# rcanut/nhwcodec

Measured on AMD Instinct MI355X. Metric: encode Mpixels/s (512x512 RGB batch), higher is better.
Workload: dtype int16

## Files before the change

include/nhw_hip_debug.h:

```cpp
#ifndef NHW_HIP_DEBUG_H
#define NHW_HIP_DEBUG_H

#include "nhw_hip.h"

#ifdef __cplusplus
extern "C" {
#endif

int nhw_debug_stop_after(nhw_enc *e, int stage);
int nhw_debug_front_fallback(nhw_enc *e, int on);
int nhw_debug_read(nhw_enc *e, int buf, int img, void *dst, size_t bytes);
int nhw_debug_hash(nhw_enc *e, int buf, size_t bytes, int n, void *d_out, void *stream);

int nhw_debug_fill(nhw_enc *e, int buf, int byte, size_t bytes, int n);

int nhw_debug_slice_order(nhw_enc *e, int mode);
int nhw_dec_debug_slice_order(nhw_dec *d, int mode);

int nhw_stage_chroma_loops(nhw_enc *e, int n, int comp, int form, void *stream);
int nhw_debug_write(nhw_enc *e, int buf, int img, const void *src, size_t bytes);
int nhw_stage_luma_loop(nhw_enc *e, int n, int form, void *stream);
int nhw_stage_ll2_walk(nhw_enc *e, int n, int form, void *stream);
int nhw_stage_quant(nhw_enc *e, int n, int form, void *stream);
int nhw_stage_residuals(nhw_enc *e, int n, int form, void *stream);
int nhw_stage_stream(nhw_enc *e, int n, int form, int32_t *status, uint32_t *sizes, void *stream);

void nhw_dec_debug_stop_after(nhw_dec *d, int stage);
int  nhw_dec_debug_read(nhw_dec *d, int what, int img, void *dst, size_t bytes);
int  nhw_dec_debug_colour(int quality, const void *d_yuv, void *d_rgb, int n);
void nhw_debug_warp_row_limit(int limit);

#ifdef __cplusplus
}
#endif
#endif
```

nhwcodec_amd/__init__.py:

```python
import ctypes
import math
import numbers
import os

HERE = os.path.dirname(os.path.abspath(__file__))
LIB_PATH = os.path.join(HERE, "libnhwhip.so")
IMG_BYTES = 786432
OUT_STRIDE = 512 << 10
QUALITY_DEFAULT = 20
NHW_OK, NHW_E_QUALITY, NHW_E_CODEBOOK, NHW_E_SPACE, NHW_E_ARG, NHW_E_HIP, NHW_E_FORMAT = 0, -1, -2, -3, -4, -5, -6
NHW_E_BUDGET = -7
PEAK_SSE_NUMERATOR = 65025 * IMG_BYTES

P = ctypes.c_void_p


class Timing(ctypes.Structure):
    _fields_ = [(n, ctypes.c_float) for n in ("total_ms", "front_ms", "color_dwt_ms", "luma_ms", "chroma_ms", "entropy_ms")] + [("parts", ctypes.c_int), ("front_images", ctypes.c_int), ("prefilter_ms", ctypes.c_float)]


class FitStats(ctypes.Structure):
    _fields_ = [("rungs", ctypes.c_int), ("quality", ctypes.c_int * 23), ("images", ctypes.c_int * 23), ("total_ms", ctypes.c_float)]


class NhwError(RuntimeError):
    pass


class CTensorFormat(ctypes.Structure):
    _fields_ = [(n, ctypes.c_int32) for n in ("dtype", "layout", "channels", "rows")] + [("scale", ctypes.c_float * 3), ("bias", ctypes.c_float * 3), ("reserved", ctypes.c_uint32)]


def load_library(path: str = LIB_PATH) -> ctypes.CDLL:
    if not os.path.exists(path):
        raise NhwError(f"{path} not built: run `python -c 'import __graft_entry__ as g; g.build()'` (needs hipcc); there is no CPU fallback")
    import torch
    L = ctypes.CDLL(path)
    L.nhw_last_error.restype = ctypes.c_char_p
    L.nhw_enc_create.argtypes = [ctypes.c_int, ctypes.c_int, ctypes.POINTER(P)]
    L.nhw_enc_create_ex.argtypes = [ctypes.c_int, ctypes.c_int, ctypes.c_uint, ctypes.POINTER(P)]
    L.nhw_enc_destroy.argtypes = [P]
    L.nhw_quality_supported.argtypes = [ctypes.c_int]
    L.nhw_enc_set_compat.argtypes = [P, ctypes.c_int]
    L.nhw_enc_batch_device.argtypes = [P, P, ctypes.c_int, ctypes.c_int, P, P, P, P]
    L.nhw_enc_batch.argtypes = [P, P, ctypes.c_int, ctypes.c_int, P, ctypes.c_size_t, P, P]
    L.nhw_synth_batch_device.argtypes = [P, P, ctypes.c_int, ctypes.c_uint32, P]
    L.nhw_enc_last_timing.argtypes = [P, ctypes.POINTER(Timing)]
    L.nhw_enc_synth_batch.argtypes = [P, ctypes.c_int, ctypes.c_uint32, ctypes.c_int, P, ctypes.c_size_t, P, P]
    L.nhw_host_alloc.restype = P
    L.nhw_host_alloc.argtypes = [ctypes.c_size_t]
    L.nhw_host_free.argtypes = [P]
    L.nhw_device_count.restype = ctypes.c_int
    L.nhw_enc_fit_batch_device.argtypes = [P, P, ctypes.c_int, P, P, ctypes.c_int, P, P, P, P, P]
    L.nhw_enc_fit_batch.argtypes = [P, P, ctypes.c_int, P, P, ctypes.c_int, P, ctypes.c_size_t, P, P, P]
    L.nhw_enc_last_fit_stats.argtypes = [P, ctypes.POINTER(FitStats)]
    L.nhw_sse_batch_device.argtypes = [P, P, ctypes.c_int, P, P]
    L.nhw_enc_fit_sse_batch_device.argtypes = [P, P, P, ctypes.c_int, P, P, ctypes.c_int, P, P, P, P, P, P]
    L.nhw_enc_fit_sse_batch.argtypes = [P, P, P, ctypes.c_int, P, P, ctypes.c_int, P, ctypes.c_size_t, P, P, P, P]
    L.nhw_stage_color.argtypes = [P, P, ctypes.c_int, ctypes.c_int, P, P, P, P]
    L.nhw_stage_prefilter.argtypes = [P, P, ctypes.c_int, ctypes.c_int, P]
    L.nhw_stage_chroma_l1.argtypes = [P, ctypes.c_int, P]
    L.nhw_stage_chroma_loops.argtypes = [P, ctypes.c_int, ctypes.c_int, ctypes.c_int, P]
    L.nhw_stage_luma_loop.argtypes = [P, ctypes.c_int, ctypes.c_int, P]
    L.nhw_stage_ll2_walk.argtypes = [P, ctypes.c_int, ctypes.c_int, P]
    L.nhw_stage_quant.argtypes = [P, ctypes.c_int, ctypes.c_int, P]
    L.nhw_stage_residuals.argtypes = [P, ctypes.c_int, ctypes.c_int, P]
    L.nhw_stage_stream.argtypes = [P, ctypes.c_int, ctypes.c_int, P, P, P]
    L.nhw_debug_write.argtypes = [P, ctypes.c_int, ctypes.c_int, P, ctypes.c_size_t]
    L.nhw_stage_analysis.argtypes = [P, P, P, ctypes.c_int, ctypes.c_size_t, ctypes.c_int, ctypes.c_int, ctypes.c_int, P]
    L.nhw_stage_synthesis.argtypes = [P, P, P, ctypes.c_int, ctypes.c_size_t, ctypes.c_int, ctypes.c_int, P]
    L.nhw_debug_slice_order.argtypes = [P, ctypes.c_int]
    L.nhw_dec_debug_slice_order.argtypes = [P, ctypes.c_int]
    L.nhw_picture_tiles.argtypes = [ctypes.c_uint32, ctypes.c_uint32]
    L.nhw_tile_pictures_device.argtypes = [P, ctypes.c_int, ctypes.c_int, ctypes.c_int, P, P]
    L.nhw_untile_pictures_device.argtypes = [P, P, ctypes.c_int, ctypes.c_int, ctypes.c_int, P]
    L.nhw_picture_info.argtypes = [P, ctypes.c_size_t, ctypes.POINTER(ctypes.c_uint32), ctypes.POINTER(ctypes.c_uint32)]
    L.nhw_enc_pictures.argtypes = [P, P, P, P, P, ctypes.c_int, ctypes.c_int, P, ctypes.c_size_t, P, P]
    L.nhw_dec_pictures.argtypes = [P, P, P, ctypes.c_int, P, P, P]
    L.nhw_sse_pictures_device.argtypes = [P, P, ctypes.c_int, ctypes.c_int, ctypes.c_int, P, P]
    L.nhw_enc_fit_pictures.argtypes = [P, P, P, P, P, ctypes.c_int, P, P, ctypes.c_int, P, ctypes.c_size_t, P, P, P]
    L.nhw_enc_fit_sse_pictures.argtypes = [P, P, P, P, P, P, ctypes.c_int, P, P, ctypes.c_int, P, ctypes.c_size_t, P, P, P, P]
    L.nhw_region_tiles.argtypes = [ctypes.c_uint32] * 6
    L.nhw_untile_regions_device.argtypes = [P, P, ctypes.c_int, ctypes.c_int, ctypes.c_int, P]
    L.nhw_dec_regions.argtypes = [P, P, P, ctypes.c_int, P, ctypes.c_int, P, P, P]
    L.nhw_dec_regions_to_device.argtypes = [P, P, P, ctypes.c_int, P, ctypes.c_int, P, P, P]
    L.nhw_dec_last_region_stats.argtypes = [P, ctypes.POINTER(ctypes.c_uint64), ctypes.POINTER(ctypes.c_uint64)]
    L.nhw_dec_batch_device_scaled.argtypes = [P, P, P, P, ctypes.c_int, ctypes.c_int, P, P, P, P]
    L.nhw_dec_batch_scaled.argtypes = [P, P, P, ctypes.c_int, ctypes.c_int, P, P, P]
    L.nhw_picture_scaled_size.argtypes = [ctypes.c_uint32, ctypes.c_uint32, ctypes.c_int, ctypes.POINTER(ctypes.c_uint32), ctypes.POINTER(ctypes.c_uint32)]
    L.nhw_untile_pictures_scaled_device.argtypes = [P, P, ctypes.c_int, ctypes.c_int, ctypes.c_int, ctypes.c_int, P]
    L.nhw_dec_pictures_scaled.argtypes = [P, P, P, ctypes.c_int, ctypes.c_int, P, P, P]
    L.nhw_window_tiles.argtypes = [ctypes.c_uint32, ctypes.c_uint32, ctypes.c_int] + [ctypes.c_uint32] * 4
    L.nhw_untile_windows_device.argtypes = [P, P, ctypes.c_int, P, ctypes.c_int, ctypes.c_int, ctypes.c_int, ctypes.c_int, P]
    L.nhw_dec_windows.argtypes = [P, P, P, ctypes.c_int, P, ctypes.c_int, ctypes.c_int, P, P, P]
    L.nhw_dec_windows_to_device.argtypes = [P, P, P, ctypes.c_int, P, ctypes.c_int, ctypes.c_int, P, P, P]
    L.nhw_dec_batch_device_tensor.argtypes = [P, P, P, P, ctypes.c_int, ctypes.c_int, ctypes.POINTER(CTensorFormat), P, P, P, P]
    L.nhw_bytes_to_tensor_device.argtypes = [P, ctypes.c_int, ctypes.POINTER(CTensorFormat), P, P]
    L.nhw_tensor_to_bytes_device.argtypes = [P, ctypes.c_int, ctypes.POINTER(CTensorFormat), P, P]
    L.nhw_crop_scale.argtypes = [ctypes.c_uint32] * 4
    L.nhw_resize_to_tensor_device.argtypes = [P, ctypes.c_int, ctypes.c_uint32, ctypes.c_uint32, ctypes.POINTER(CTensorFormat), P, P, P]
    L.nhw_dec_crops_to_device.argtypes = [P, P, P, ctypes.c_int, P, ctypes.c_int, ctypes.c_int, ctypes.c_uint32, ctypes.c_uint32, ctypes.POINTER(CTensorFormat), P, P, P]
    L.nhw_enc_batch_device_tensor.argtypes = [P, P, ctypes.c_int, ctypes.POINTER(CTensorFormat), ctypes.c_int, P, P, P, P]
    L.nhw_tile_tensors_device.argtypes = [P, ctypes.c_int, ctypes.c_int, ctypes.c_int, ctypes.POINTER(CTensorFormat), P, P]
    L.nhw_area_to_tensor_device.argtypes = L.nhw_resize_to_tensor_device.argtypes
    L.nhw_dec_crops_to_device_filter.argtypes = L.nhw_dec_crops_to_device.argtypes + [ctypes.c_int]
    a = L.nhw_resize_to_tensor_device.argtypes
    L.nhw_resample_to_tensor_device.argtypes = a[:4] + [ctypes.c_int] + a[4:]
    L.nhw_dec_crops_to_device_resample.argtypes = L.nhw_dec_crops_to_device_filter.argtypes
    L.nhw_enc_pictures_resized.argtypes = [P, P, P, P, P, ctypes.c_int, ctypes.c_uint32, ctypes.c_uint32, ctypes.c_int, P, ctypes.c_size_t, P, P]
    L.nhw_warp_to_tensor_device.argtypes = L.nhw_resize_to_tensor_device.argtypes
    L.nhw_dec_warps_to_device.argtypes = L.nhw_dec_crops_to_device.argtypes
    L.nhw_debug_warp_row_limit.argtypes, L.nhw_debug_warp_row_limit.restype = [ctypes.c_int], None
    L.nhw_grey_table.argtypes = [ctypes.c_int, P]
    L.nhw_dec_batch_device_grey.argtypes = L.nhw_dec_batch_device_tensor.argtypes
    L.nhw_dec_batch_grey.argtypes = L.nhw_dec_batch_scaled.argtypes
    L.nhw_untile_windows_grey_device.argtypes = L.nhw_untile_windows_device.argtypes
    L.nhw_resample_grey_to_tensor_device.argtypes = L.nhw_resample_to_tensor_device.argtypes
    L.nhw_warp_grey_to_tensor_device.argtypes = L.nhw_warp_to_tensor_device.argtypes
    L.nhw_dec_windows_grey.argtypes = L.nhw_dec_windows.argtypes
    L.nhw_dec_windows_grey_to_device.argtypes = L.nhw_dec_windows_to_device.argtypes
    L.nhw_dec_crops_grey_to_device.argtypes = L.nhw_dec_crops_to_device_resample.argtypes
    L.nhw_dec_warps_grey_to_device.argtypes = L.nhw_dec_warps_to_device.argtypes
    a = L.nhw_resample_to_tensor_device.argtypes
    L.nhw_resample_mapped_to_tensor_device.argtypes = a[:7] + [P] + a[7:]
    a = L.nhw_warp_to_tensor_device.argtypes
    L.nhw_warp_mapped_to_tensor_device.argtypes = a[:6] + [P] + a[6:]
    a = L.nhw_dec_crops_to_device_resample.argtypes
    L.nhw_dec_crops_mapped_to_device.argtypes = a[:11] + [P] + a[11:]
    a = L.nhw_dec_warps_to_device.argtypes
    L.nhw_dec_warps_mapped_to_device.argtypes = a[:11] + [P] + a[11:]
    a = L.nhw_resample_mapped_to_tensor_device.argtypes
    L.nhw_resample_toned_to_tensor_device.argtypes = a[:8] + [P] + a[8:]
    a = L.nhw_warp_mapped_to_tensor_device.argtypes
    L.nhw_warp_toned_to_tensor_device.argtypes = a[:7] + [P] + a[7:]
    a = L.nhw_dec_crops_mapped_to_device.argtypes
    L.nhw_dec_crops_toned_to_device.argtypes = a[:12] + [P] + a[12:]
    a = L.nhw_dec_warps_mapped_to_device.argtypes
    L.nhw_dec_warps_toned_to_device.argtypes = a[:12] + [P] + a[12:]
    L.nhw_hist_device.argtypes = [P, ctypes.c_int, ctypes.c_int, P, P]
    L.nhw_tone_from_hist_device.argtypes = [P, ctypes.c_int, ctypes.c_int, P, P, P]
    return L


_LIB = None


def _library():
    global _LIB
    if _LIB is None:
        _LIB = load_library()
    return _LIB


def psnr_to_max_sse(db):
    import numpy as np
    try:
        a = np.asarray(db, dtype=np.float64)
    except (TypeError, ValueError):
        raise NhwError(f"a PSNR target must be a finite number of dB above 0, got {db!r}") from None
    if a.size == 0 or not np.all(np.isfinite(a)) or not np.all(a > 0):
        raise NhwError(f"a PSNR target must be a finite number of dB above 0, got {db!r}")
    m = np.floor(float(PEAK_SSE_NUMERATOR) * np.power(10.0, -a / 10.0)).astype(np.int64)
    return int(m) if m.ndim == 0 else m


def sse_device(a, b):
    import torch
    for name, x in (("a", a), ("b", b)):
        if not (isinstance(x, torch.Tensor) and x.is_cuda and x.dtype == torch.uint8 and x.is_contiguous() and x.numel() > 0 and x.numel() % IMG_BYTES == 0):
            raise NhwError(f"sse_device: `{name}` must be a contiguous uint8 CUDA tensor of n * {IMG_BYTES} bytes")
    if a.numel() != b.numel() or a.device != b.device:
        raise NhwError("sse_device: `a` and `b` must hold as many pictures, on one device")
    n = a.numel() // IMG_BYTES
    L = _library()
    out = torch.empty(n, dtype=torch.int64, device=a.device)
    with torch.cuda.device(a.device):
        rc = L.nhw_sse_batch_device(a.data_ptr(), b.data_ptr(), n, out.data_ptr(), torch.cuda.current_stream(a.device).cuda_stream)
    if rc != 0:
        raise NhwError(f"libnhwhip rc={rc}: {L.nhw_last_error().decode()}")
    return out


PICTURE_DTYPE = [("addr", "<u8"), ("pitch", "<u8"), ("width", "<u4"), ("height", "<u4"), ("first_tile", "<u4"), ("reserved", "<u4")]


def picture_tiles(width: int, height: int) -> int:
    if not (1 <= width <= 65535 and 1 <= height <= 65535):
        raise NhwError(f"a picture side must be 1..65535, got {width} x {height}")
    return ((width + 511) // 512) * ((height + 511) // 512)


SCALES = (1, 2, 4)


def _scale(scale, what):
    if isinstance(scale, bool) or not isinstance(scale, numbers.Integral) or scale not in SCALES:
        raise NhwError(f"{what}: the scale must be 1, 2 or 4, got {scale!r}")
    return int(scale)


def scaled_size(width: int, height: int, scale: int) -> tuple:
    scale = _scale(scale, "scaled_size")
    if not (isinstance(width, numbers.Integral) and isinstance(height, numbers.Integral)):
        raise NhwError(f"a picture's sides must be integers, got {width!r} x {height!r}")
    picture_tiles(int(width), int(height))
    return -(-int(width) // scale), -(-int(height) // scale)


REGION_DTYPE = [("addr", "<u8"), ("pitch", "<u8"), ("x", "<u4"), ("y", "<u4"), ("width", "<u4"), ("height", "<u4"), ("pic_width", "<u4"),
                ("pic_height", "<u4"), ("first_tile", "<u4"), ("reserved", "<u4")]
RECT_DTYPE = [("container", "<u4"), ("x", "<u4"), ("y", "<u4"), ("width", "<u4"), ("height", "<u4")]


def region_tiles(pic_width: int, pic_height: int, x: int, y: int, width: int, height: int) -> int:
    picture_tiles(pic_width, pic_height)
# ... 1639 lines not shown
```

nhwcodec_amd/csrc/nhw_enc.h:

```cpp
#ifndef NHW_ENC_H
#define NHW_ENC_H

#include <stdio.h>
#include <stdlib.h>
#include <string.h>
#include <climits>

#include "nhw_host.h"
#include "nhw_ws.h"

extern thread_local std::string nhw_enc_err;
#define NHW_ERR nhw_enc_err

enum { EV_START, EV_FRONT, EV_LUMA, EV_CHROMA, EV_END, EV_COLOR, EV_PREFILTER, EV_COUNT };
enum { PE_LUMA_LIST, PE_CHROMA, PE_LISTS_FORK, PE_LISTS, PE_FRONT, PE_COUNT };
enum { LL_EV_FORK, LL_EV_DONE, LL_EV_Y5_FORK, LL_EV_Y5_DONE, LL_EV_PACK_FORK, LL_EV_PACK_DONE, LL_EV_COUNT };

struct nhw_enc {
	int device, max_batch;
	NhwWs ws;
	hipStream_t own_stream;
	hipStream_t part_stream[4];
	hipEvent_t part_ev[PE_COUNT];
	hipStream_t low_stream[4];
	hipEvent_t low_ev[LOW_EV_COUNT];
	int low_parts;
	int low_parts_used;
	int low_chroma;
	hipStream_t ll_stream;
	hipEvent_t ll_ev[LL_EV_COUNT];
	int ll_fork;
	int quant_join;
	int y5_fork;
	int ll2_once;
	int quant_marks;
	int pack_fork;
	int parts;
	hipEvent_t ev[EV_COUNT];
	bool timed;
	int timed_parts, timed_front_images;
	uint8_t *d_in, *d_out, *d_compact;
	uint32_t *d_sizes; int32_t *d_status; uint64_t *d_offs;
	int conv_cap;
	uint8_t *d_tensor_bytes;
	int chroma_fork;
	int lists_fork;
	int front_fallback;
	int stop_after;
	int slice_order;
	int last_n, last_q;
	struct {
		uint8_t *in, *out;
		uint32_t *sizes, *budget;
		int32_t *status, *quality;
		int *idx[2], *count;
		uint8_t *open;
	} fit;
	struct {
		uint8_t *px;
		uint64_t *doff;
		uint64_t *sse, *maxsse;
		uint64_t *sse_out;
		int32_t *dstatus;
	} fit_sse;
	int *h_fit_count;
	hipEvent_t fit_ev[2];
	nhw_fit_stats fit_stats;
	bool fit_done;
	GrowBuf pic_px, pic_desc, pfit_px, pfit_aux, pic_resized;
};

inline DevSet host_set(nhw_enc *e, size_t n)
{
	return { dev_buf(e->d_in, n * NHW_IMG_BYTES), dev_buf(e->d_out, n * NHW_OUT_STRIDE), dev_buf(e->d_compact, n * NHW_OUT_STRIDE), dev_buf(e->d_sizes, n),
	         dev_buf(e->d_status, n), dev_buf(e->d_offs, n + 1) };
}
inline DevSet fit_set(nhw_enc *e)
{
	const size_t mb = (size_t)e->max_batch;
	return { dev_buf(e->fit.in, mb * NHW_IMG_BYTES), dev_buf(e->fit.out, mb * NHW_OUT_STRIDE), dev_buf(e->fit.sizes, mb), dev_buf(e->fit.budget, mb),
	         dev_buf(e->fit.status, mb), dev_buf(e->fit.quality, mb), dev_buf(e->fit.idx[0], mb), dev_buf(e->fit.idx[1], mb), dev_buf(e->fit.count, 1),
	         dev_buf(e->fit.open, mb) };
}
inline DevSet fit_sse_set(nhw_enc *e)
{
	const size_t mb = (size_t)e->max_batch;
	return { dev_buf(e->fit_sse.px, mb * NHW_IMG_BYTES), dev_buf(e->fit_sse.doff, mb), dev_buf(e->fit_sse.sse, mb), dev_buf(e->fit_sse.maxsse, mb),
	         dev_buf(e->fit_sse.sse_out, mb), dev_buf(e->fit_sse.dstatus, mb) };
}

int host_buffers(nhw_enc *e, int n);
int host_download(nhw_enc *e, int n, uint8_t *out_arena, size_t arena_cap, uint64_t *out_off, int32_t *status);
int ladder_check(const int *ladder, int ladder_len, bool ascending, int *q, int *len);
int dec_check(const nhw_enc *e, nhw_dec *d, int need, const std::string &who, const char *need_name);
void fit_doff(uint64_t *d_off, int n, hipStream_t s);

#endif
```

nhwcodec_amd/csrc/nhw_enc.hip:

```cpp
#include "nhw_enc.h"

thread_local std::string nhw_enc_err;
extern "C" const char *nhw_last_error(void) { return nhw_enc_err.c_str(); }

static const size_t k_buf_bytes[B_COUNT] = {
	 8 * Q,  8 * Q,  Q,  Q,  2 * Q,  2 * Q,
	 2 * Q,  2 * Q,  Q / 2,  Q / 2,  4 * Q,  2 * Q,
	 2 * Q,  4 * Q + 256,  8 * Q,  16,  512,  6 * Q,
	 24832,  16384,  16384 + 256,  32768,  16384,  32768,
	 8192,  2 * Q + 1024,  2 * Q + 256,  2 * Q + 1024,  2 * Q + 1024,  Q / 2,
	 Q + 64, 8192 + 64, 16384 + 64,  Q + 64, 8192 + 64, 16384 + 64,  Q + 64, 8192 + 64, 16384 + 64,
	 2 * Q + 1024, 16384 + 64, 16384 + 64,  2048 + 64,  8 * Q + 64,
	 512,  512,  320000,  768,  768,  16384 + 64,  16384 + 64,
	 131072,  131072,  5632,  256,  512,  16,  16,  (8 + 9 * 512) * 2,
	 Q / 2 + 256,  Q / 2,  Q / 4,  4 * Q,
	 Q / 4 + 256,  2 * Q,
	 2 * Q,  2 * Q,  Q / 2,  Q / 2,  Q,
	 320 * 512,
	 sizeof(NhwChromaPack),  320000
};

static size_t round_up(size_t v, size_t a) { return (v + a - 1) / a * a; }

extern "C" int nhw_quality_supported(int quality) { return quality >= 1 && quality <= 23; }

extern "C" int nhw_enc_set_compat(nhw_enc *e, int mode)
{
	if (!e || (mode != NHW_COMPAT_CANONICAL && mode != NHW_COMPAT_GLIBC_ONESHOT)) return NHW_E_ARG;
	if (e->ws.compat != mode && mode == NHW_COMPAT_CANONICAL) {
		HIPCHK(hipSetDevice(e->device));
		HIPCHK(hipDeviceSynchronize());
		HIPCHK(hipMemset2D(e->ws.plane<uint8_t>(B_LL1).p + 2 * Q, e->ws.plane<uint8_t>(B_LL1).bytes(), 0, 1024, (size_t)e->max_batch));
		HIPCHK(hipMemset2D(e->ws.plane<uint8_t>(B_L2SAVE).p + 2 * Q, e->ws.plane<uint8_t>(B_L2SAVE).bytes(), 0, 256, (size_t)e->max_batch));
	}
	e->ws.compat = mode;
	return NHW_OK;
}

#define HOST_PATH_BYTES ((size_t)NHW_IMG_BYTES + 2 * (size_t)NHW_OUT_STRIDE + 24)
extern "C" int nhw_enc_create_ex(int device, int max_batch, unsigned flags, nhw_enc **out)
{
	if (!out || max_batch < 1 || max_batch > 65535 || (flags & ~(unsigned)NHW_CREATE_DEVICE_ONLY)) { nhw_enc_err = "bad argument"; return NHW_E_ARG; }
	const bool host_staging = !(flags & NHW_CREATE_DEVICE_ONLY);
	HIPCHK(hipSetDevice(device));
	nhw_enc *e = new nhw_enc();
	memset(e, 0, sizeof *e);
	e->device = device; e->max_batch = max_batch;
	size_t total = 0;
	for (int b = 0; b < B_COUNT; b++) {
		e->ws.stride[b] = round_up(k_buf_bytes[b] + GUARD, 256);
		e->ws.off[b] = total + GUARD;
		total += GUARD + e->ws.stride[b] * (size_t)max_batch;
	}
	const int rc = [&]() -> int {
		size_t free_b = 0, total_b = 0;
		HIPCHK(hipMemGetInfo(&free_b, &total_b));
		const size_t need = total + (host_staging ? HOST_PATH_BYTES * (size_t)max_batch : 0);
		if (need > free_b) {
			char b[200];
			snprintf(b, sizeof b, "encoder workspace for max_batch %d needs %zu MiB (%.1f MiB per image), %zu MiB of HBM are free", max_batch, need >> 20, (double)need / max_batch / 1048576.0, free_b >> 20);
			nhw_enc_err = b;
			return NHW_E_ARG;
		}
		{ const char *where = ""; int rc_ = nhw_front_set_attrs(&where); if (!rc_) rc_ = nhw_tail_set_attrs(&where);
		  if (rc_) { nhw_enc_err = std::string(where) + " -> " + hipGetErrorString((hipError_t)rc_); return NHW_E_HIP; } }
		HIPCHK(hipMalloc((void **)&e->ws.base, total));
		HIPCHK(hipMemset(e->ws.base, 0, total));
		HIPCHK(hipStreamCreate(&e->own_stream));
		for (int i = 0; i < EV_COUNT; i++) HIPCHK(hipEventCreate(&e->ev[i]));
		for (int i = 0; i < 4; i++) HIPCHK(hipStreamCreateWithFlags(&e->part_stream[i], hipStreamNonBlocking));
		for (int i = 0; i < PE_COUNT; i++) HIPCHK(hipEventCreateWithFlags(&e->part_ev[i], hipEventDisableTiming));
		for (int i = 0; i < 4; i++) HIPCHK(hipStreamCreateWithFlags(&e->low_stream[i], hipStreamNonBlocking));
		for (int i = 0; i < LOW_EV_COUNT; i++) HIPCHK(hipEventCreateWithFlags(&e->low_ev[i], hipEventDisableTiming));
		HIPCHK(hipStreamCreateWithFlags(&e->ll_stream, hipStreamNonBlocking));
		for (int i = 0; i < LL_EV_COUNT; i++) HIPCHK(hipEventCreateWithFlags(&e->ll_ev[i], hipEventDisableTiming));
		for (int i = 0; i < 2; i++) HIPCHK(hipEventCreate(&e->fit_ev[i]));
		HIPCHK(hipHostMalloc((void **)&e->h_fit_count, sizeof(int), hipHostMallocDefault));
		return host_staging ? host_buffers(e, max_batch) : NHW_OK;
	}();
	if (rc != NHW_OK) { nhw_enc_destroy(e); return rc; }
	auto env = [](const char *name, int dflt) { const char *p = getenv(name); return p ? atoi(p) : dflt; };
	auto within = [](int v, int lo, int hi, int other) { return v < lo || v > hi ? other : v; };
	e->parts = within(env("NHW_PARTS", 1), 1, 4, 1);
	e->low_parts = within(env("NHW_LOW_PARTS", 2), 1, 4, 1);
	e->low_chroma = within(env("NHW_LOW_CHROMA", 2), 0, 2, 2);
	e->chroma_fork = env("NHW_CHROMA_FORK", 1) != 0;
	e->lists_fork = env("NHW_LISTS_FORK", 1) != 0;
	e->ll_fork = env("NHW_LL_FORK", 1) != 0;
	e->quant_join = env("NHW_QUANT_JOIN", 1) != 0;
	e->y5_fork = env("NHW_Y5_FORK", 1) != 0;
	e->ll2_once = env("NHW_LL2_ONCE", 1) != 0;
	e->quant_marks = env("NHW_QUANT_MARKS", 1) != 0;
	e->pack_fork = within(env("NHW_PACK_FORK", 2), 0, 2, 2);
	*out = e;
	return NHW_OK;
}

extern "C" int nhw_enc_create(int device, int max_batch, nhw_enc **out) { return nhw_enc_create_ex(device, max_batch, 0u, out); }

extern "C" void nhw_enc_destroy(nhw_enc *e)
{
	if (!e) return;
	(void)hipSetDevice(e->device);
	(void)hipDeviceSynchronize();
	if (e->ws.base) (void)hipFree(e->ws.base);
	dev_free(host_set(e, 0));
	dev_free({ dev_buf(e->d_tensor_bytes, 0) });
	dev_free(fit_set(e));
	dev_free(fit_sse_set(e));
	for (GrowBuf *g : { &e->pic_px, &e->pic_desc, &e->pfit_px, &e->pfit_aux, &e->pic_resized }) nhw_grow_free(*g);
	if (e->h_fit_count) (void)hipHostFree(e->h_fit_count);
	for (int i = 0; i < 2; i++) if (e->fit_ev[i]) (void)hipEventDestroy(e->fit_ev[i]);
	for (int i = 0; i < EV_COUNT; i++) if (e->ev[i]) (void)hipEventDestroy(e->ev[i]);
	if (e->own_stream) (void)hipStreamDestroy(e->own_stream);
	for (int i = 0; i < 4; i++) if (e->part_stream[i]) (void)hipStreamDestroy(e->part_stream[i]);
	for (int i = 0; i < PE_COUNT; i++) if (e->part_ev[i]) (void)hipEventDestroy(e->part_ev[i]);
	for (int i = 0; i < 4; i++) if (e->low_stream[i]) (void)hipStreamDestroy(e->low_stream[i]);
	for (int i = 0; i < LOW_EV_COUNT; i++) if (e->low_ev[i]) (void)hipEventDestroy(e->low_ev[i]);
	if (e->ll_stream) (void)hipStreamDestroy(e->ll_stream);
	for (int i = 0; i < LL_EV_COUNT; i++) if (e->ll_ev[i]) (void)hipEventDestroy(e->ll_ev[i]);
	delete e;
}

int host_buffers(nhw_enc *e, int n)
{
	if (e->conv_cap >= n) return NHW_OK;
	dev_free(host_set(e, 0));
	e->conv_cap = 0;
	const int rc = dev_alloc(host_set(e, (size_t)n), nullptr, n, nhw_enc_err);
	if (rc == NHW_OK) e->conv_cap = n;
	return rc;
}

#define STAGE_DONE() do { if (e->stop_after && ++stage == e->stop_after) { HIPCHK(hipGetLastError()); return NHW_OK; } } while (0)
static int chroma_head_launches(nhw_enc *e, const NhwWs &ws, int comp, int n, hipStream_t cs, int &stage)
{
	const int q = ws.q;
	const bool low = q <= 16;
	const bool vp = comp && ws.split_chroma;
	const Plane<int16_t> cjpeg = ws.plane<int16_t>(vp ? B_CJPEG_V : B_CJPEG), cproc = ws.plane<int16_t>(vp ? B_CPROC_V : B_CPROC);
	const Plane<int16_t> cll1 = ws.plane<int16_t>(vp ? B_CLL1_V : B_CLL1), cl2save = ws.plane<int16_t>(vp ? B_CL2SAVE_V : B_CL2SAVE);
	const Plane<const uint8_t> bytes = ws.plane<const uint8_t>(comp ? B_PV : B_PU);
	const bool widen_in_analysis = q > 14 && !ws.dbg;
	if (q <= 14) nhw_launch_low_prefilter_chroma(bytes, cjpeg, q, n, cs);
	else if (!widen_in_analysis) nhw_launch_phase(PH_C0, ws, comp, cs);
	STAGE_DONE();
	NhwAnalysis l1 = NhwAnalysis{ cjpeg, cproc, n, H, H, 0 }.saving(cll1, H / 2, ANA_SAVE_LL);
	l1.store = ws.dbg ? ANA_STORE_ALL : ANA_STORE_NO_T_LL_SAVED;
	if (widen_in_analysis) l1.src8 = bytes;
	nhw_launch_analysis(l1, cs);
	if (low) nhw_launch_low_chroma_thin(cproc, n, cs);
	STAGE_DONE();
	STAGE_DONE();
	if (!ws.dbg) {
		nhw_launch_chroma_loops(cproc, cll1, cl2save, ws.plane<const uint8_t>(B_PU), q, comp, ws.compat, n, cs);
		return 1;
	}
	const NhwAnalysis l2{ cjpeg, cproc, n, H, H / 2, 1 };
	nhw_launch_analysis(l2, cs);
	STAGE_DONE();
	nhw_launch_phase(PH_C2, ws, comp, cs);
	STAGE_DONE();
	nhw_launch_synthesis(cjpeg, cproc, n, H, H / 2, 0, cs);
	STAGE_DONE();
	nhw_launch_phase(PH_C3, ws, comp, cs);
	STAGE_DONE();
	nhw_launch_analysis(l2.saving(cl2save, H / 2, ANA_SAVE_BLOCK), cs);
	STAGE_DONE();
	STAGE_DONE();
	nhw_launch_phase(PH_C4, ws, comp, cs);
	STAGE_DONE();
	nhw_launch_synthesis(cjpeg, cproc, n, H, H / 2, 0, cs);
	STAGE_DONE();
	return 1;
}

static int luma_loop_launches(nhw_enc *e, const NhwWs &ws, int n, hipStream_t s, int &stage, bool y5_beside = false ,
                              bool lean = false )
{
	const int q = ws.q;
	const Plane<int16_t> jpeg = ws.plane<int16_t>(B_JPEG), proc = ws.plane<int16_t>(B_PROC), ll1 = ws.plane<int16_t>(B_LL1), l2save = ws.plane<int16_t>(B_L2SAVE);
	const NhwAnalysis l2{ jpeg, proc, n, W, H, 1 };
	assert(!lean || (!ws.dbg && !ws.compat));
	NhwAnalysis first = l2.from(ll1, H);
	if (lean && q > 6) first.store = ANA_STORE_NO_T;
	nhw_launch_analysis(first, s);
	STAGE_DONE();
	if (q > 6) {
	if (y5_beside) {
		assert(!ws.dbg);
		HIPCHK(hipEventRecord(e->ll_ev[LL_EV_Y5_FORK], s));
		HIPCHK(hipStreamWaitEvent(e->ll_stream, e->ll_ev[LL_EV_Y5_FORK], 0));
		nhw_launch_phase(PH_L1, ws, 0, e->ll_stream);
		HIPCHK(hipEventRecord(e->ll_ev[LL_EV_Y5_DONE], e->ll_stream));
	} else
	nhw_launch_phase(PH_L1, ws, 0, s);
	nhw_launch_wave(WV_DQ1, ws, s);
	if (y5_beside) HIPCHK(hipStreamWaitEvent(s, e->ll_ev[LL_EV_Y5_DONE], 0));
	STAGE_DONE();
	if (ws.dbg) {
	nhw_launch_synthesis(jpeg, proc, n, W, H, 0, s);
	STAGE_DONE();
	nhw_launch_phase(PH_L2, ws, 0, s);
	STAGE_DONE();
	} else nhw_launch_l2_recon(jpeg, proc, ll1, q > 12 ? l2save : Plane<int16_t>{}, n, s, lean && q > 12);
	if (q <= 12) nhw_launch_analysis(l2, s);
	else if (ws.dbg) nhw_launch_analysis(l2.saving(l2save, H, ANA_SAVE_BLOCK), s);
	STAGE_DONE();
	}
	return 1;
}

static int run_batch(nhw_enc *e, const NhwWs &ws_in, const void *d_bgr, int n, int quality, void *d_out, uint32_t *d_sizes, int32_t *d_status, hipStream_t s,
                     int timed ,
                     int what = 3 )
{
	NhwWs ws = ws_in;
	const int q = quality;
	const bool low = q <= 16;
	const Plane<int16_t> jpeg = ws.plane<int16_t>(B_JPEG), proc = ws.plane<int16_t>(B_PROC);
	const Plane<uint8_t> pu = ws.plane<uint8_t>(B_PU), pv = ws.plane<uint8_t>(B_PV);

	e->low_parts_used = 1;
	int stage = 0;
	if (what & 1) {
	if (timed == 1) HIPCHK(hipEventRecord(e->ev[EV_START], s));
	const Plane<int16_t> yin = ws.plane<int16_t>(B_KMAP);
	NhwFront f;
	f.q = q; f.n = n; f.y = yin ; f.st = ws.plane<uint8_t>(B_ROWSTATE);
	f.proc = proc; f.jpeg = jpeg; f.ll1 = ws.plane<int16_t>(B_LL1); f.switches = ws.dbg ? 2 : 0;
	if (low) {
		nhw_launch_color((const uint8_t *)d_bgr, n, q, jpeg, pu, pv, s);
		HIPCHK(hipEventRecord(e->ev[EV_COLOR], s));
		STAGE_DONE();
		{ const int lparts = (timed == 1 && what == 3 && !e->stop_after && n >= 1024) ? e->low_parts : 1;
		  e->low_parts_used = lparts;
		  HIPCHK((hipError_t)nhw_launch_low_prefilter(jpeg, yin, proc, ws.plane<uint8_t>(B_SCAN), ws.plane<uint8_t>(B_KEEP), ws.plane<uint8_t>(B_LOWTAB), q, n, s, (e->front_fallback & 1) ? 32 : 0,
		                                              lparts, e->low_stream, e->low_ev)); }
		HIPCHK(hipEventRecord(e->ev[EV_PREFILTER], s));
		STAGE_DONE();
		if (ws.compat) nhw_launch_low_stale(proc, ws.plane<uint8_t>(B_STALE), n, s);
	} else {
		HIPCHK(hipEventRecord(e->ev[EV_COLOR], s)); HIPCHK(hipEventRecord(e->ev[EV_PREFILTER], s));
		STAGE_DONE();
		if (q < 22) STAGE_DONE();
		f.bgr = (const uint8_t *)d_bgr; f.pu = pu; f.pv = pv; f.with_prefilter = q < 22; f.switches |= e->front_fallback & 1;
		if (q > 21) f.keep = ws.plane<int16_t>(B_KEEP);
	}
	nhw_launch_front_fused(f, s);
	if (!low && ws.compat && q < 22) {
		nhw_launch_color((const uint8_t *)d_bgr, n, q, yin, pu, pv, s);
		nhw_launch_front_stale(yin, f.st, ws.plane<uint8_t>(B_STALE), n, s);
	}
	STAGE_DONE();
	STAGE_DONE();
	if (timed == 1) HIPCHK(hipEventRecord(e->ev[EV_FRONT], s));
	if (!(what & 2)) { HIPCHK(hipGetLastError()); return NHW_OK; }
	}
	const bool fork = timed == 1 && what == 3 && !e->stop_after && e->chroma_fork;
	const bool fork_ll = fork && q > 13 && !ws.compat && e->ll_fork;
	ws.defer_verbatim = fork_ll;
	hipStream_t cs = fork ? e->part_stream[0] : s;
	ws.split_chroma = fork;
	auto chroma_head = [&](int comp) -> int { return chroma_head_launches(e, ws, comp, n, cs, stage); };
	auto chroma_tail = [&](int comp) -> int {
		nhw_launch_phase(PH_C5, ws, comp, cs);
		STAGE_DONE();
		return 1;
	};
#define CHROMA(call) do { const int rc_ = (call); if (rc_ != 1) return rc_; } while (0)
	if (fork) {
		HIPCHK(hipStreamWaitEvent(cs, !low || e->low_chroma == 0 ? e->ev[EV_FRONT] : (e->low_chroma == 2 && e->low_parts_used > 1) ? e->low_ev[low_ev_pass_a(e->low_parts_used - 1)] : e->ev[EV_COLOR], 0));
		CHROMA(chroma_head(0));
		CHROMA(chroma_head(1));
	}
	{ const int rc_ = luma_loop_launches(e, ws, n, s, stage, fork && e->y5_fork, !ws.dbg && !ws.compat); if (rc_ != 1) return rc_; }
	if (q <= 12) {
		nhw_launch_low_ll2(proc, q, n, s);
		nhw_launch_copy_block(proc, W, ws.plane<int16_t>(B_L2SAVE), H, H, H, n, s);
	}
	STAGE_DONE();
	const bool one_walk = fork && q > 12 && e->ll2_once;
	const bool marks = q > 16 && !e->stop_after && !ws.dbg && e->quant_marks;
	nhw_launch_wave(WV_EMIT, ws, s, one_walk);
	if (fork_ll) {
		HIPCHK(hipEventRecord(e->ll_ev[LL_EV_FORK], s));
		HIPCHK(hipStreamWaitEvent(e->ll_stream, e->ll_ev[LL_EV_FORK], 0));
		nhw_launch_phase(PH_L3, ws, 0, e->ll_stream);
		HIPCHK(hipEventRecord(e->ll_ev[LL_EV_DONE], e->ll_stream));
		HIPCHK(hipEventRecord(e->part_ev[PE_LUMA_LIST], e->ll_stream));
	} else {
	nhw_launch_phase(PH_L3, ws, 0, s);
	if (fork) HIPCHK(hipEventRecord(e->part_ev[PE_LUMA_LIST], s));
	}
	if (q > 12) {
	nhw_launch_wave(WV_DQ0, ws, s, one_walk, marks);
	STAGE_DONE();
	if (fork_ll) {
		HIPCHK(hipStreamWaitEvent(s, e->ll_ev[LL_EV_DONE], 0));
		const Plane<const uint8_t> meta = ws.plane<const uint8_t>(B_META), len{ meta.p + offsetof(NhwMeta, ll_mem_len), meta.pitch };
		nhw_launch_synthesis(jpeg, proc, n, W, H, q <= 21 && !ws.dbg, ws.plane<const uint8_t>(B_LLMEM), len, s);
	} else
	nhw_launch_synthesis(jpeg, proc, n, W, H, q <= 21 && !ws.dbg, s);
	STAGE_DONE();
	}
	nhw_launch_phase(PH_L4A, ws, 0, s);
	const bool fork_lists = fork && q <= 20 && q > 12 && e->lists_fork;
	if (fork_lists) {
		HIPCHK(hipEventRecord(e->part_ev[PE_LISTS_FORK], s));
		HIPCHK(hipStreamWaitEvent(e->part_stream[1], e->part_ev[PE_LISTS_FORK], 0));
		nhw_launch_phase(PH_L4B, ws, 0, e->part_stream[1]);
		HIPCHK(hipEventRecord(e->part_ev[PE_LISTS], e->part_stream[1]));
	} else if (q > 12)
		nhw_launch_phase(PH_L4B, ws, 0, s);
	nhw_launch_phase(PH_L4C, ws, 0, s);
	const bool early_join = fork && e->quant_join;
	const int pack_fork = fork ? e->pack_fork : 0;
	auto chroma_rest = [&]() -> int {
		HIPCHK(hipStreamWaitEvent(cs, e->part_ev[PE_LUMA_LIST], 0));
		CHROMA(chroma_tail(0));
		CHROMA(chroma_tail(1));
		if (pack_fork == 2) {
			HIPCHK(hipEventRecord(e->ll_ev[LL_EV_PACK_FORK], cs));
			HIPCHK(hipStreamWaitEvent(e->ll_stream, e->ll_ev[LL_EV_PACK_FORK], 0));
			nhw_launch_pack_chroma(ws, e->ll_stream);
			HIPCHK(hipEventRecord(e->ll_ev[LL_EV_PACK_DONE], e->ll_stream));
		}
		nhw_launch_phase(PH_LLC, ws, 0, cs);
		if (pack_fork == 1) nhw_launch_pack_chroma(ws, cs);
		if (pack_fork == 2) HIPCHK(hipStreamWaitEvent(cs, e->ll_ev[LL_EV_PACK_DONE], 0));
		HIPCHK(hipEventRecord(e->part_ev[PE_CHROMA], cs));
		return 1;
	};
	if (early_join) {
		CHROMA(chroma_rest());
		if (fork_lists) HIPCHK(hipStreamWaitEvent(s, e->part_ev[PE_LISTS], 0));
		HIPCHK(hipStreamWaitEvent(s, e->part_ev[PE_CHROMA], 0));
	}
	nhw_launch_wave(WV_QUANT, ws, s, false, marks);
	if (q > 21) nhw_launch_phase(PH_L4C2, ws, 0, s);
	if (fork && !early_join) CHROMA(chroma_rest());
	nhw_launch_phase(PH_L4D, ws, 0, s);
	STAGE_DONE();
	if (timed) HIPCHK(hipEventRecord(e->ev[EV_LUMA], s));

	if (fork_lists && !early_join) HIPCHK(hipStreamWaitEvent(s, e->part_ev[PE_LISTS], 0));
	if (fork) { if (!early_join) HIPCHK(hipStreamWaitEvent(s, e->part_ev[PE_CHROMA], 0)); }
	else
		for (int comp = 0; comp < 2; comp++) {
			CHROMA(chroma_head(comp));
			CHROMA(chroma_tail(comp));
		}
#undef CHROMA
	if (timed) HIPCHK(hipEventRecord(e->ev[EV_CHROMA], s));
	if (!fork) nhw_launch_phase(PH_LLC, ws, 0, s);
	nhw_launch_final(ws, (uint8_t *)d_out, d_sizes, d_status, s, pack_fork != 0);
	if (timed == 1) HIPCHK(hipEventRecord(e->ev[EV_END], s));
	HIPCHK(hipGetLastError());
	return NHW_OK;
}

extern "C" int nhw_enc_batch_device(nhw_enc *e, const void *d_bgr, int n, int quality, void *d_out, uint32_t *d_sizes,
                                    int32_t *d_status, void *stream)
{
	if (!e || !d_bgr || !d_out || !d_sizes || !d_status || n < 1 || n > e->max_batch) { nhw_enc_err = "bad argument"; return NHW_E_ARG; }
	if (!nhw_quality_supported(quality)) { nhw_enc_err = "quality outside 1..23"; return NHW_E_QUALITY; }
	HIPCHK(hipSetDevice(e->device));
	hipStream_t s = stream ? (hipStream_t)stream : e->own_stream;
	const NhwSliceScope slices(e->slice_order);
	NhwWs ws = e->ws;
	ws.n = n; ws.q = quality; ws.dbg = e->stop_after != 0;
	e->timed = false;
	const int parts = (e->stop_after || n < 512) ? 1 : e->parts;
	if (parts == 1) {
		const int rc = run_batch(e, ws, d_bgr, n, quality, d_out, d_sizes, d_status, s, 1);
		if (rc == NHW_OK && !e->stop_after) { e->timed = true; e->timed_parts = 1; e->timed_front_images = n; e->last_n = n; e->last_q = quality; }
		return rc;
	}
	HIPCHK(hipEventRecord(e->ev[EV_START], s));
	{ const int rc = run_batch(e, ws, d_bgr, n, quality, d_out, d_sizes, d_status, s, 0, 1); if (rc != NHW_OK) return rc; }
	HIPCHK(hipEventRecord(e->ev[EV_FRONT], s));
	HIPCHK(hipEventRecord(e->part_ev[PE_FRONT], s));
	e->timed_front_images = n;
	for (int k = 0; k < parts; k++) {
		const int i0 = (int)((long long)n * k / parts), i1 = (int)((long long)n * (k + 1) / parts);
		NhwWs view = ws;
		view.n = i1 - i0;
		for (int b = 0; b < B_COUNT; b++) view.off[b] += (size_t)i0 * ws.stride[b];
		hipStream_t ps_ = e->part_stream[k];
		HIPCHK(hipStreamWaitEvent(ps_, e->part_ev[PE_FRONT], 0));
		const int rc = run_batch(e, view, (const uint8_t *)d_bgr + (size_t)i0 * (W * W * 3), i1 - i0, quality, (uint8_t *)d_out + (size_t)i0 * NHW_OUT_STRIDE,
		                         d_sizes + i0, d_status + i0, ps_, k == 0 ? 2 : 0, 2);
		if (rc != NHW_OK) return rc;
		HIPCHK(hipEventRecord(e->part_ev[k], ps_));
		HIPCHK(hipStreamWaitEvent(s, e->part_ev[k], 0));
	}
	HIPCHK(hipEventRecord(e->ev[EV_END], s));
	e->timed = true; e->timed_parts = parts; e->last_n = n; e->last_q = quality;
	return NHW_OK;
}

extern "C" int nhw_enc_last_timing(nhw_enc *e, nhw_timing *t)
{
	if (!e || !t || !e->timed) { nhw_enc_err = "no timed batch"; return NHW_E_ARG; }
	HIPCHK(hipEventSynchronize(e->ev[EV_END]));
	memset(t, 0, sizeof *t);
	HIPCHK(hipEventElapsedTime(&t->total_ms, e->ev[EV_START], e->ev[EV_END]));
	HIPCHK(hipEventElapsedTime(&t->front_ms, e->ev[EV_START], e->ev[EV_FRONT]));
	HIPCHK(hipEventElapsedTime(&t->luma_ms, e->ev[EV_FRONT], e->ev[EV_LUMA]));
	HIPCHK(hipEventElapsedTime(&t->chroma_ms, e->ev[EV_LUMA], e->ev[EV_CHROMA]));
	HIPCHK(hipEventElapsedTime(&t->entropy_ms, e->ev[EV_CHROMA], e->ev[EV_END]));
	HIPCHK(hipEventElapsedTime(&t->color_dwt_ms, e->ev[EV_START], e->ev[EV_COLOR]));
	HIPCHK(hipEventElapsedTime(&t->prefilter_ms, e->ev[EV_COLOR], e->ev[EV_PREFILTER]));
	t->parts = e->timed_parts; t->front_images = e->timed_front_images;
	return NHW_OK;
}

extern "C" int nhw_synth_batch_device(nhw_enc *e, void *d_bgr, int n, uint32_t seed_base, void *stream)
{
	if (!e || !d_bgr || n < 1) { nhw_enc_err = "bad argument"; return NHW_E_ARG; }
	HIPCHK(hipSetDevice(e->device));
	nhw_launch_synth((uint8_t *)d_bgr, n, seed_base, stream ? (hipStream_t)stream : e->own_stream);
	HIPCHK(hipGetLastError());
	return NHW_OK;
}

extern "C" int nhw_stage_color(nhw_enc *e, const void *d_bgr, int n, int quality, void *d_y, void *d_u, void *d_v, void *stream)
{
	if (!e || n < 1) return NHW_E_ARG;
	if (quality < 1 || quality > 23) return NHW_E_QUALITY;
	HIPCHK(hipSetDevice(e->device));
	nhw_launch_color((const uint8_t *)d_bgr, n, quality, Plane<int16_t>{ (int16_t *)d_y, 4 * Q }, Plane<uint8_t>{ (uint8_t *)d_u, Q }, Plane<uint8_t>{ (uint8_t *)d_v, Q }, stream ? (hipStream_t)stream : e->own_stream);
	HIPCHK(hipGetLastError());
	return NHW_OK;
}

extern "C" int nhw_stage_prefilter(nhw_enc *e, void *d_y, int n, int quality, void *stream)
{
	if (!e || !d_y || n < 1 || n > e->max_batch) { nhw_enc_err = "bad argument"; return NHW_E_ARG; }
	if (quality < 1 || quality > 16) { nhw_enc_err = "the pre-filter is a stage of its own only for quality 1..16"; return NHW_E_QUALITY; }
	HIPCHK(hipSetDevice(e->device));
	const NhwWs &ws = e->ws;
	hipStream_t s = stream ? (hipStream_t)stream : e->own_stream;
	const Plane<int16_t> filtered = ws.plane<int16_t>(B_KMAP);
	HIPCHK((hipError_t)nhw_launch_low_prefilter(Plane<const int16_t>{ (const int16_t *)d_y, 4 * Q }, filtered, ws.plane<int16_t>(B_PROC), ws.plane<uint8_t>(B_SCAN), ws.plane<uint8_t>(B_KEEP), ws.plane<uint8_t>(B_LOWTAB), quality, n, s, 0, 1 , e->low_stream, e->low_ev));
	HIPCHK(hipMemcpy2DAsync(d_y, 8 * Q, filtered.p, filtered.bytes(), 8 * Q, (size_t)n, hipMemcpyDeviceToDevice, s));
	HIPCHK(hipGetLastError());
	return NHW_OK;
}

__global__ __launch_bounds__(256) void k_plane_range(const int16_t *__restrict__ base, size_t plane_stride, int *__restrict__ mnmx)
{
	const uint4 *p = reinterpret_cast<const uint4 *>(base + (size_t)blockIdx.y * plane_stride);
	int mn = 32767, mx = -32768;
	for (int i = blockIdx.x * 256 + threadIdx.x; i < W * W / 8; i += gridDim.x * 256) {
		const uint4 v = p[i];
		const uint32_t w[4] = { v.x, v.y, v.z, v.w };
		for (int k = 0; k < 4; k++) {
			const int a = (int16_t)(w[k] & 0xFFFF), b = (int16_t)(w[k] >> 16);
			mn = a < mn ? a : mn; mn = b < mn ? b : mn; mx = a > mx ? a : mx; mx = b > mx ? b : mx;
		}
	}
	for (int o = 32; o; o >>= 1) { const int a = __shfl_xor(mn, o), b = __shfl_xor(mx, o); mn = a < mn ? a : mn; mx = b > mx ? b : mx; }
	if ((threadIdx.x & 63) == 0) { atomicMin(&mnmx[0], mn); atomicMax(&mnmx[1], mx); }
}

extern "C" int nhw_stage_analysis(nhw_enc *e, void *d_jpeg, void *d_proc, int n_img, size_t plane_stride, int stride, int size,
                                  int final_level, void *stream)
{
	if (!e || n_img < 1) { nhw_enc_err = "bad argument"; return NHW_E_ARG; }
	HIPCHK(hipSetDevice(e->device));
	hipStream_t s = stream ? (hipStream_t)stream : e->own_stream;
	if (size == 512) {
		if (stride != W || final_level || n_img > e->max_batch) { nhw_enc_err = "size 512: stride 512, not the final level, n <= max_batch"; return NHW_E_ARG; }
		if (((uintptr_t)d_jpeg & 15) || ((uintptr_t)d_proc & 15) || (plane_stride & 7) || plane_stride < (size_t)W * W) {
			nhw_enc_err = "size 512: planes must be 16-byte aligned and plane_stride (in samples) a multiple of 8, at least 512 x 512"; return NHW_E_ARG;
		}
		const NhwWs &ws = e->ws;
		{
			int *d_mm = reinterpret_cast<int *>(ws.plane<uint8_t>(B_ROWSTATE).p), mm[2] = { 32767, -32768 };
			HIPCHK(hipMemcpyAsync(d_mm, mm, sizeof mm, hipMemcpyHostToDevice, s));
			k_plane_range<<<dim3(32, n_img), 256, 0, s>>>((const int16_t *)d_jpeg, plane_stride, d_mm);
			HIPCHK(hipMemcpyAsync(mm, d_mm, sizeof mm, hipMemcpyDeviceToHost, s));
			HIPCHK(hipStreamSynchronize(s));
			const long U = mm[1] > 0 ? mm[1] : 0, L = mm[0] < 0 ? -(long)mm[0] : 0;
			if (104 * U + 40 * L > NHW_ANA512_BOUND || 104 * L + 40 * U > NHW_ANA512_BOUND) {
				nhw_enc_err = "size 512: samples outside the level-1 kernel's 16-bit domain (104 U + 40 L <= 32720, see nhw_hip.h)";
				return NHW_E_ARG;
			}
		}
		const Plane<int16_t> in = ws.plane<int16_t>(B_KMAP);
		HIPCHK(hipMemcpy2DAsync(in.p, in.bytes(), d_jpeg, plane_stride * 2, 8 * Q, (size_t)n_img, hipMemcpyDeviceToDevice, s));
		NhwFront f;
		f.q = 20; f.n = n_img; f.y = in; f.st = ws.plane<uint8_t>(B_ROWSTATE);
		f.proc = { (int16_t *)d_proc, plane_stride }; f.jpeg = { (int16_t *)d_jpeg, plane_stride }; f.ll1 = ws.plane<int16_t>(B_LL1); f.switches = 2;
		nhw_launch_front_fused(f, s);
	} else if (size == 256 || size == 128)
		nhw_launch_analysis(NhwAnalysis{ { (int16_t *)d_jpeg, plane_stride }, { (int16_t *)d_proc, plane_stride }, n_img, stride, size, final_level }, s);
	else { nhw_enc_err = "transform size must be 512, 256 or 128"; return NHW_E_ARG; }
	HIPCHK(hipGetLastError());
	return NHW_OK;
}

extern "C" int nhw_stage_chroma_l1(nhw_enc *e, int n, void *stream)
{
	if (!e || n < 1 || n > e->max_batch) { nhw_enc_err = "bad argument"; return NHW_E_ARG; }
	if (!e->timed || n > e->last_n || e->last_q < 15) {
		nhw_enc_err = "nhw_stage_chroma_l1: the handle's last batch does not cover the request (needs a completed batch of >= n images at quality >= 15)";
		return NHW_E_ARG;
	}
	HIPCHK(hipSetDevice(e->device));
	const NhwWs &ws = e->ws;
	hipStream_t s = stream ? (hipStream_t)stream : e->own_stream;
	HIPCHK(hipStreamWaitEvent(s, e->ev[EV_END], 0));
	NhwAnalysis l1 = NhwAnalysis{ ws.plane<int16_t>(B_CJPEG), ws.plane<int16_t>(B_CPROC), n, H, H, 0 }.saving(ws.plane<int16_t>(B_CLL1), H / 2, ANA_SAVE_LL);
	l1.store = ANA_STORE_NO_T_LL_SAVED;
	for (int comp = 0; comp < 2; comp++) { l1.src8 = ws.plane<const uint8_t>(comp ? B_PV : B_PU); nhw_launch_analysis(l1, s); }
	HIPCHK(hipGetLastError());
	return NHW_OK;
}

extern "C" int nhw_stage_chroma_loops(nhw_enc *e, int n, int comp, int form, void *stream)
{
	if (!e || n < 1 || n > e->max_batch || comp < 0 || comp > 1 || form < 0 || form > 8) { nhw_enc_err = "bad argument"; return NHW_E_ARG; }
	if (!e->timed || n > e->last_n || e->stop_after) {
		nhw_enc_err = "nhw_stage_chroma_loops: needs a completed whole batch of >= n images and no debug stop";
		return NHW_E_ARG;
	}
	HIPCHK(hipSetDevice(e->device));
	NhwWs ws = e->ws;
	ws.n = n; ws.q = e->last_q; ws.dbg = 0; ws.split_chroma = false;
	hipStream_t s = stream ? (hipStream_t)stream : e->own_stream;
	HIPCHK(hipStreamWaitEvent(s, e->ev[EV_END], 0));
	const Plane<int16_t> cjpeg = ws.plane<int16_t>(B_CJPEG), cproc = ws.plane<int16_t>(B_CPROC), cll1 = ws.plane<int16_t>(B_CLL1), cl2save = ws.plane<int16_t>(B_CL2SAVE);
	if (form == 0) {
		int stage = 0;
		const int rc = chroma_head_launches(e, ws, comp, n, s, stage);
		if (rc != 1) return rc;
	} else if (form == 1)
		nhw_launch_chroma_loops(cproc, cll1, cl2save, ws.plane<const uint8_t>(B_PU), ws.q, comp, ws.compat, n, s);
	else {
		const int k = form - 1;
		const NhwAnalysis l2{ cjpeg, cproc, n, H, H / 2, 1 };
		nhw_launch_analysis(l2.from(cll1, H / 2), s);
		if (k > 1) nhw_launch_phase(PH_C2, ws, comp, s);
		if (k > 2) nhw_launch_synthesis(cjpeg, cproc, n, H, H / 2, 0, s);
		if (k > 3) nhw_launch_phase(PH_C3, ws, comp, s);
		if (k > 4) nhw_launch_analysis(l2.saving(cl2save, H / 2, ANA_SAVE_BLOCK), s);
		if (k > 5) nhw_launch_phase(PH_C4, ws, comp, s);
		if (k > 6) nhw_launch_synthesis(cjpeg, cproc, n, H, H / 2, 0, s);
	}
	HIPCHK(hipGetLastError());
	return NHW_OK;
}

extern "C" int nhw_stage_luma_loop(nhw_enc *e, int n, int form, void *stream)
{
	if (!e || n < 1 || n > e->max_batch || form < 0 || form > 7) { nhw_enc_err = "bad argument"; return NHW_E_ARG; }
	if (!e->timed || n > e->last_n || e->stop_after || e->last_q < 7) {
		nhw_enc_err = "nhw_stage_luma_loop: needs a completed whole batch of >= n images at quality >= 7 and no debug stop";
		return NHW_E_ARG;
	}
	HIPCHK(hipSetDevice(e->device));
	NhwWs ws = e->ws;
	ws.n = n; ws.q = e->last_q; ws.dbg = 0;
	hipStream_t s = stream ? (hipStream_t)stream : e->own_stream;
	HIPCHK(hipStreamWaitEvent(s, e->ev[EV_END], 0));
	const Plane<int16_t> jpeg = ws.plane<int16_t>(B_JPEG), proc = ws.plane<int16_t>(B_PROC), ll1 = ws.plane<int16_t>(B_LL1), l2save = ws.plane<int16_t>(B_L2SAVE);
	const NhwAnalysis l2{ jpeg, proc, n, W, H, 1 };
	const bool save = ws.q > 12;
	const bool lean = form >= 6;
	if (lean && ws.compat) { nhw_enc_err = "nhw_stage_luma_loop: forms 6 and 7 are not launched in the compatibility mode"; return NHW_E_ARG; }
	if (form == 0 || form == 6) {
		int stage = 0;
		const int rc = luma_loop_launches(e, ws, n, s, stage, false, lean);
		if (rc != 1) return rc;
	} else if (form == 1 || form == 7) {
		nhw_launch_l2_recon(jpeg, proc, ll1, save ? l2save : Plane<int16_t>{}, n, s, lean && save);
		if (!save) nhw_launch_analysis(l2, s);
	} else {
		if (form == 3 || form == 4) {
			nhw_launch_analysis(l2.from(ll1, H), s);
			nhw_launch_phase(PH_L1, ws, 0, s);
			nhw_launch_wave(WV_DQ1, ws, s);
		}
		nhw_launch_synthesis(jpeg, proc, n, W, H, 0, s);
		if (form < 4) {
			nhw_launch_phase(PH_L2, ws, 0, s);
			nhw_launch_analysis(save ? l2.saving(l2save, H, ANA_SAVE_BLOCK) : l2, s);
		}
	}
	HIPCHK(hipGetLastError());
	return NHW_OK;
}

extern "C" int nhw_stage_ll2_walk(nhw_enc *e, int n, int form, void *stream)
{
	if (!e || n < 1 || n > e->max_batch || form < 0 || form > 3) { nhw_enc_err = "bad argument"; return NHW_E_ARG; }
	if (!e->timed || n > e->last_n || e->stop_after || e->last_q < 13) {
		nhw_enc_err = "nhw_stage_ll2_walk: needs a completed whole batch of >= n images at quality >= 13 and no debug stop";
		return NHW_E_ARG;
	}
	HIPCHK(hipSetDevice(e->device));
	NhwWs ws = e->ws;
	ws.n = n; ws.q = e->last_q; ws.dbg = 0; ws.defer_verbatim = form >= 2;
	hipStream_t s = stream ? (hipStream_t)stream : e->own_stream;
	HIPCHK(hipStreamWaitEvent(s, e->ev[EV_END], 0));
	const bool one_walk = !(form & 1);
	nhw_launch_wave(WV_EMIT, ws, s, one_walk);
	nhw_launch_phase(PH_L3, ws, 0, s);
	nhw_launch_wave(WV_DQ0, ws, s, one_walk);
	if (ws.defer_verbatim) {
		const Plane<const uint8_t> meta = ws.plane<const uint8_t>(B_META), len{ meta.p + offsetof(NhwMeta, ll_mem_len), meta.pitch };
		nhw_launch_synthesis(ws.plane<int16_t>(B_JPEG), ws.plane<int16_t>(B_PROC), n, W, H, ws.q <= 21, ws.plane<const uint8_t>(B_LLMEM), len, s);
	}
	HIPCHK(hipGetLastError());
	return NHW_OK;
}

extern "C" int nhw_stage_quant(nhw_enc *e, int n, int form, void *stream)
{
	if (!e || n < 1 || n > e->max_batch || form < 0 || form > 1) { nhw_enc_err = "bad argument"; return NHW_E_ARG; }
	if (!e->timed || n > e->last_n || e->stop_after || e->last_q < 17) {
		nhw_enc_err = "nhw_stage_quant: needs a completed whole batch of >= n images at quality >= 17 and no debug stop";
		return NHW_E_ARG;
	}
	HIPCHK(hipSetDevice(e->device));
	NhwWs ws = e->ws;
	ws.n = n; ws.q = e->last_q; ws.dbg = 0; ws.defer_verbatim = 1;
	hipStream_t s = stream ? (hipStream_t)stream : e->own_stream;
	HIPCHK(hipStreamWaitEvent(s, e->ev[EV_END], 0));
	if (form == 0) nhw_launch_wave(WV_DQ0, ws, s, true, true);
	nhw_launch_wave(WV_QUANT, ws, s, false, form == 0);
	HIPCHK(hipGetLastError());
	return NHW_OK;
}

extern "C" int nhw_stage_residuals(nhw_enc *e, int n, int form, void *stream)
{
	if (!e || n < 1 || n > e->max_batch || form < 0 || form > 3) { nhw_enc_err = "bad argument"; return NHW_E_ARG; }
	if (!e->timed || n > e->last_n || e->stop_after || (form == 2 && e->last_q <= 12)) {
		nhw_enc_err = "nhw_stage_residuals: needs a completed whole batch of >= n images (form 2: at quality >= 13) and no debug stop";
		return NHW_E_ARG;
	}
	HIPCHK(hipSetDevice(e->device));
	NhwWs ws = e->ws;
	ws.n = n; ws.q = e->last_q; ws.dbg = form == 1;
	hipStream_t s = stream ? (hipStream_t)stream : e->own_stream;
	HIPCHK(hipStreamWaitEvent(s, e->ev[EV_END], 0));
	if (form < 2) nhw_launch_phase(PH_L4A, ws, 0, s);
	if (form < 3 && ws.q > 12) nhw_launch_phase(PH_L4B, ws, 0, s);
	if (form != 2) nhw_launch_phase(PH_L4C, ws, 0, s);
	HIPCHK(hipGetLastError());
	return NHW_OK;
}

extern "C" int nhw_stage_stream(nhw_enc *e, int n, int form, int32_t *status, uint32_t *sizes, void *stream)
{
	if (!e || (!status && form != 2) || n < 1 || n > e->max_batch || form < 0 || form > 2) { nhw_enc_err = "bad argument"; return NHW_E_ARG; }
	if (!e->timed || n > e->last_n || e->stop_after) {
		nhw_enc_err = "nhw_stage_stream: needs a completed whole batch of >= n images and no debug stop";
		return NHW_E_ARG;
	}
	HIPCHK(hipSetDevice(e->device));
	{ const int rc = host_buffers(e, n); if (rc != NHW_OK) return rc; }
	NhwWs ws = e->ws;
	ws.n = n; ws.q = e->last_q; ws.dbg = 0;
	hipStream_t s = stream ? (hipStream_t)stream : e->own_stream;
	HIPCHK(hipStreamWaitEvent(s, e->ev[EV_END], 0));
	if (form != 1) nhw_launch_phase(PH_L4D, ws, 0, s);
	if (form == 2) { HIPCHK(hipGetLastError()); HIPCHK(hipStreamSynchronize(s)); return NHW_OK; }
	nhw_launch_final(ws, e->d_out, e->d_sizes, e->d_status, s);
	HIPCHK(hipGetLastError());
	HIPCHK(hipMemcpyAsync(status, e->d_status, sizeof(int32_t) * (size_t)n, hipMemcpyDeviceToHost, s));
	if (sizes) HIPCHK(hipMemcpyAsync(sizes, e->d_sizes, sizeof(uint32_t) * (size_t)n, hipMemcpyDeviceToHost, s));
	HIPCHK(hipStreamSynchronize(s));
	return NHW_OK;
}

extern "C" int nhw_stage_synthesis(nhw_enc *e, void *d_jpeg, void *d_proc, int n_img, size_t plane_stride, int stride, int size, void *stream)
{
	if (!e || n_img < 1) return NHW_E_ARG;
	if (size != 256 && size != 128) { nhw_enc_err = "synthesis: transform size must be 256 or 128 (the encoder has no synthesis of size 512)"; return NHW_E_ARG; }
	HIPCHK(hipSetDevice(e->device));
	nhw_launch_synthesis({ (int16_t *)d_jpeg, plane_stride }, { (int16_t *)d_proc, plane_stride }, n_img, stride, size, 0, stream ? (hipStream_t)stream : e->own_stream);
	HIPCHK(hipGetLastError());
	return NHW_OK;
}

extern "C" int nhw_debug_front_fallback(nhw_enc *e, int on) { if (!e) return NHW_E_ARG; e->front_fallback = on; return NHW_OK; }
extern "C" int nhw_debug_stop_after(nhw_enc *e, int stage) { if (!e) return NHW_E_ARG; e->stop_after = stage; return NHW_OK; }
extern "C" int nhw_debug_slice_order(nhw_enc *e, int mode) { if (!e || mode < 0 || mode > 2) return NHW_E_ARG; e->slice_order = mode; return NHW_OK; }
__global__ __launch_bounds__(256) void k_debug_hash(const uint8_t *base, size_t stride, size_t words, unsigned long long *out)
{
	const uint32_t *p = reinterpret_cast<const uint32_t *>(base + (size_t)blockIdx.x * stride);
	unsigned long long h = 0;
	for (size_t i = threadIdx.x; i < words; i += 256) {
		unsigned long long x = ((unsigned long long)p[i] + 0x9E3779B97F4A7C15ull) * (2 * i + 1);
		x ^= x >> 29; x *= 0xBF58476D1CE4E5B9ull; x ^= x >> 32;
		h += x;
	}
	if (threadIdx.x == 0) out[blockIdx.x] = 0;
	__syncthreads();
	atomicAdd(&out[blockIdx.x], h);
}
extern "C" int nhw_debug_hash(nhw_enc *e, int buf, size_t bytes, int n, void *d_out, void *stream)
{
	if (!e || buf < 0 || buf >= B_COUNT || n < 1 || n > e->max_batch || bytes > e->ws.stride[buf]) return NHW_E_ARG;
// ... 31 lines not shown
```

nhwcodec_amd/csrc/nhw_host.h:

```cpp
#ifndef NHW_HOST_H
#define NHW_HOST_H

#include <hip/hip_runtime.h>
#include <stdint.h>
#include <string>
#include <vector>

#include "../../include/nhw_hip.h"
#include "nhw_container.h"

struct NhwWs;

template <class T> struct Plane {
	T *p = nullptr; size_t pitch = 0;
	Plane at(size_t i) const { return { p + i * pitch, pitch }; }
	size_t bytes() const { return pitch * sizeof(T); }
	operator Plane<const T>() const { return { p, pitch }; }
};

extern thread_local int nhw_slice_mode;

struct NhwSliceScope {
	int saved;
	explicit NhwSliceScope(int mode) : saved(nhw_slice_mode) { nhw_slice_mode = mode; }
	~NhwSliceScope() { nhw_slice_mode = saved; }
};

template <typename F> inline void nhw_slices(int nslices, F &&launch)
{
	if (nhw_slice_mode == 1) for (int i = 0; i < nslices; i++) launch(i);
	else if (nhw_slice_mode == 2) for (int i = nslices - 1; i >= 0; i--) launch(i);
	else launch(-1);
}

void nhw_launch_color(const uint8_t *bgr, int n, int q, Plane<int16_t> y, Plane<uint8_t> u, Plane<uint8_t> v, hipStream_t s);
enum NhwAnaSave { ANA_SAVE_NONE, ANA_SAVE_BLOCK , ANA_SAVE_LL  };
enum NhwAnaStore { ANA_STORE_ALL, ANA_STORE_NO_T, ANA_STORE_NO_T_LL_SAVED };
struct NhwAnalysis {
	Plane<int16_t> jpeg, proc; int n, stride, size, final_level;
	Plane<int16_t> save = {}; int save_row = 0; NhwAnaSave save_kind = ANA_SAVE_NONE; NhwAnaStore store = ANA_STORE_ALL;
	Plane<const uint8_t> src8 = {}; Plane<const int16_t> alt = {}; int alt_stride = 0;
	NhwAnalysis from(Plane<const int16_t> p, int row) const { NhwAnalysis a = *this; a.alt = p; a.alt_stride = row; return a; }
	NhwAnalysis saving(Plane<int16_t> p, int row, NhwAnaSave kind) const { NhwAnalysis a = *this; a.save = p; a.save_row = row; a.save_kind = kind; return a; }
};
void nhw_launch_analysis(const NhwAnalysis &a, hipStream_t s);
void nhw_launch_synthesis(Plane<int16_t> jpeg, Plane<int16_t> proc, int n, int stride, int size, int drop_nat, Plane<const uint8_t> verb_list, Plane<const uint8_t> verb_len, hipStream_t s);
inline void nhw_launch_synthesis(Plane<int16_t> jpeg, Plane<int16_t> proc, int n, int stride, int size, int drop_nat, hipStream_t s) { nhw_launch_synthesis(jpeg, proc, n, stride, size, drop_nat, {}, {}, s); }
void nhw_launch_synth(uint8_t *bgr, int n, uint32_t seed_base, hipStream_t s);
struct NhwFront {
	const uint8_t *bgr = nullptr; Plane<uint8_t> pu = {}, pv = {}, st = {}; Plane<const int16_t> y = {};
	Plane<int16_t> proc = {}, jpeg = {}, ll1 = {}, keep = {}; int q = 0, with_prefilter = 0, n = 0, switches = 0;
};
void nhw_launch_front_fused(const NhwFront &f, hipStream_t s);
void nhw_launch_front_stale(Plane<const int16_t> y, Plane<const uint8_t> st, Plane<uint8_t> stale, int n, hipStream_t s);
int nhw_front_set_attrs(const char **where);
enum { PH_L1, PH_L2, PH_L3, PH_L4A, PH_C0, PH_C2, PH_C3, PH_C4, PH_C5, PH_L4B = 10, PH_L4C, PH_L4D, PH_LLC, PH_L4C2 };
enum { WV_DQ1, WV_DQ0, WV_EMIT, WV_QUANT };
void nhw_launch_phase(int ph, const NhwWs &ws, int comp, hipStream_t s);
void nhw_launch_pack_chroma(const NhwWs &ws, hipStream_t s);
void nhw_launch_final(const NhwWs &ws, uint8_t *out, uint32_t *sizes, int32_t *status, hipStream_t s, bool chroma_packed = false);
void nhw_launch_wave(int ph, const NhwWs &ws, hipStream_t s, bool one_walk = false ,
                     bool marks = false );
void nhw_launch_l2_recon(Plane<int16_t> jpeg, Plane<int16_t> proc, Plane<int16_t> ll1, Plane<int16_t> l2save , int n, hipStream_t s, bool lean = false );
void nhw_launch_chroma_loops(Plane<int16_t> cproc, Plane<int16_t> cll1, Plane<int16_t> cl2save, Plane<const uint8_t> pu, int q, int comp, int compat, int n, hipStream_t s);
void nhw_launch_copy_block(Plane<const int16_t> src, int src_row, Plane<int16_t> dst, int dst_row, int rows, int cols, int n, hipStream_t s);
int nhw_tail_set_attrs(const char **where);
enum { LOW_EV_START = 0, LOW_EV_COUNT = 13 };
inline int low_ev_pass_a(int p) { return 1 + p; }
inline int low_ev_done(int parts, int p) { return 1 + parts + p; }
int nhw_launch_low_prefilter(Plane<const int16_t> src, Plane<int16_t> y, Plane<int16_t> km, Plane<uint8_t> so, Plane<uint8_t> chain, Plane<uint8_t> tab,
                             int q, int n, hipStream_t s, int force, int parts, hipStream_t *aux, hipEvent_t *ev);
void nhw_launch_low_prefilter_chroma(Plane<const uint8_t> src, Plane<int16_t> dst, int q, int n, hipStream_t s);
void nhw_launch_low_chroma_thin(Plane<int16_t> plane, int n, hipStream_t s);
void nhw_launch_low_ll2(Plane<int16_t> proc, int q, int n, hipStream_t s);
void nhw_launch_low_stale(Plane<const int16_t> km, Plane<uint8_t> stale, int n, hipStream_t s);
void nhw_launch_fit_gather(const uint8_t *d_bgr, const int *idx, int m, uint8_t *staging, hipStream_t s);
void nhw_launch_fit_select(const int *idx, int m, const uint8_t *st_out, const uint32_t *st_sizes, const int32_t *st_status, const void *limit,
                           const int32_t *dec_status, const uint64_t *sse, int quality, int last, uint8_t *out, uint32_t *sizes, int32_t *status,
                           int32_t *qual, uint64_t *sse_out, uint8_t *open, hipStream_t s);
void nhw_launch_fit_compact(const uint8_t *open, const int *idx, int m, int *next, int *count, hipStream_t s);
hipError_t nhw_launch_sse(const uint8_t *a, const uint8_t *b, int n, uint64_t *sse, hipStream_t s);
hipError_t nhw_launch_tile_pad(const nhw_picture *d_pics, int n_pics, int tile0, int m, uint8_t *d_tiles, hipStream_t s);
hipError_t nhw_launch_untile_crop(const uint8_t *d_tiles, const nhw_picture *d_pics, int n_pics, int tile0, int m, int scale , hipStream_t s);
hipError_t nhw_launch_untile_region(const uint8_t *d_tiles, const nhw_region *d_regs, int n_regs, int tile0, int m, hipStream_t s);
hipError_t nhw_launch_untile_window(const uint8_t *d_tiles, const nhw_region *d_regs, int n_regs, const nhw_window_use *d_uses , int n_uses, int tile0, int m, int scale, hipStream_t s);
hipError_t nhw_launch_untile_window_grey(const uint8_t *d_tiles , const nhw_region *d_regs, int n_regs, const nhw_window_use *d_uses, int n_uses, int tile0, int m, int scale, hipStream_t s);
hipError_t nhw_launch_sse_crop(const uint8_t *d_tiles, const nhw_picture *d_pics, int n_pics, int tile0, int m, uint64_t *d_sse, hipStream_t s);
void nhw_dec_props(const nhw_dec *d, int *device, int *max_batch, int *stop_after);

int nhw_hip_error(std::string &err, hipError_t e, const char *file, int line, const char *call);
#define HIPCHK(x) do { hipError_t e_ = (x); if (e_ != hipSuccess) return nhw_hip_error(NHW_ERR, e_, __FILE__, __LINE__, #x); } while (0)

struct DevBuf { void **p; size_t bytes; };
using DevSet = std::vector<DevBuf>;
template <class T> inline DevBuf dev_buf(T *&p, size_t count) { return { (void **)&p, count * sizeof(T) }; }
void dev_free(const DevSet &set);
int dev_alloc(const DevSet &set, const char *what, int images, std::string &err);

struct GrowBuf {
	void *p; size_t cap;
	template <class T> T *as() const { return (T *)p; }
};
hipError_t nhw_grow(GrowBuf &b, size_t bytes);
void nhw_grow_free(GrowBuf &b);

#endif
```

nhwcodec_amd/csrc/nhw_tail.hip:

```cpp
#include "nhw_host.h"
#include "nhw_tail_par.h"
#include "nhw_dwt.h"

using namespace nhw;

#ifndef NHW_DENSE_STREAM
#define NHW_DENSE_STREAM 0
#endif

template <int PH>
__global__ __launch_bounds__(256) void k_phase(NhwWs ws, int comp)
{
	__shared__ int sh_counts[2];
	__shared__ int sh_pos[2 * NT + 2];
	__shared__ uint32_t sh_z[4 * Q / 16 / 32 + 4];
	extern __shared__ __attribute__((aligned(16))) int16_t dyn_lds[];
	const int img = blockIdx.x, tid = threadIdx.x;
	Ctx c;
	ctx_load(&c, ws, img, comp);
	if (PH == PH_L1) luma_p1_par(&c, tid, sh_pos);
	else if (PH == PH_L2) luma_p2_par(&c, tid, dyn_lds);
	else if (PH == PH_L3) luma_p3_par(&c, tid, sh_pos, sh_counts, dyn_lds, ws.q <= 12 || ws.dbg != 0);
	else if (PH == PH_L4A) luma_p4a_par(&c, tid, dyn_lds);
	else if (PH == PH_L4B) luma_p4b_par(&c, tid, sh_pos, dyn_lds);
	else if (PH == PH_L4C) luma_p4c_par(&c, tid, sh_pos, dyn_lds, ws.q > 21 || ws.dbg);
	else if (PH == PH_L4D) luma_p4d_par(&c, tid, sh_counts, sh_z, dyn_lds, NHW_DENSE_STREAM || ws.dbg);
	else if (PH == PH_L4C2) luma_p4c2_par(&c, tid, reinterpret_cast<unsigned *>(sh_z), sh_pos);
	else if (PH == PH_LLC) { PROF_BEGIN(); ll_code_chroma_par(&c, tid, reinterpret_cast<uint8_t *>(dyn_lds)); if (!tid) PROF(&c, 18); }
	else if (PH == PH_C0) chroma_p0_par(&c, comp, tid);
	else if (PH == PH_C2) { chroma_ll1_neighbour(&c, tid); dequant_sim_chroma_par(&c, 1, tid); }
	else if (PH == PH_C3) chroma_p3_par(&c, comp, tid);
	else if (PH == PH_C4) dequant_sim_chroma_par(&c, 0, tid);
	else if (PH == PH_C5) chroma_p5_par(&c, comp, tid, dyn_lds, sh_counts, ws.dbg != 0);
}

#ifndef NHW_FINAL_WAVES
#define NHW_FINAL_WAVES 6
#endif
__global__ __launch_bounds__(256) __attribute__((amdgpu_waves_per_eu(NHW_FINAL_WAVES, NHW_FINAL_WAVES))) void k_final(NhwWs ws, uint8_t *out, uint32_t *sizes, int32_t *status)
{
	extern __shared__ __attribute__((aligned(16))) int16_t dyn_lds[];
	__shared__ PackShared sh_pack;
	const int img = blockIdx.x, tid = threadIdx.x;
	Ctx c;
	ctx_load(&c, ws, img);
	final_phase_par(&c, ws.buf<NhwChromaPack>(B_CPACK, img), ws.buf<uint32_t>(B_CPACKET, img), out + (size_t)img * (512u << 10), 512u << 10, &sizes[img], &status[img], &sh_pack, tid,
	                reinterpret_cast<uint32_t *>(dyn_lds));
}

#ifndef NHW_PACKC_WAVES
#define NHW_PACKC_WAVES 6
#endif
__global__ __launch_bounds__(256) __attribute__((amdgpu_waves_per_eu(NHW_PACKC_WAVES, NHW_PACKC_WAVES))) void k_pack_chroma(NhwWs ws)
{
	extern __shared__ __attribute__((aligned(16))) int16_t dyn_lds[];
	__shared__ PackShared sh_pack;
	const int img = blockIdx.x;
	Ctx c;
	ctx_load(&c, ws, img);
	pack_chroma_par(&c, ws.buf<NhwChromaPack>(B_CPACK, img), ws.buf<uint32_t>(B_CPACKET, img), &sh_pack, threadIdx.x, reinterpret_cast<uint32_t *>(dyn_lds));
}

__global__ __launch_bounds__(512) void k_y31(NhwWs ws)
{
	extern __shared__ __attribute__((aligned(16))) int16_t dyn_lds[];
	__shared__ int sh_counts[2];
	Ctx c;
	ctx_load(&c, ws, blockIdx.x);
	PROF_BEGIN();
	scan_rewrite_list_par<512>(&c, threadIdx.x, reinterpret_cast<uint8_t *>(dyn_lds), sh_counts);
	if (!threadIdx.x) PROF(&c, 17);
}

#ifndef NHW_L4A_WAVES
#define NHW_L4A_WAVES 8
#endif
__global__ __launch_bounds__(256) __attribute__((amdgpu_waves_per_eu(NHW_L4A_WAVES, NHW_L4A_WAVES))) void k_l4a(NhwWs ws)
{
	extern __shared__ __attribute__((aligned(16))) int16_t dyn_lds[];
	Ctx c;
	ctx_load(&c, ws, blockIdx.x);
	luma_p4a_par(&c, threadIdx.x, dyn_lds);
}

template <int PH>
__global__ __launch_bounds__(256) void k_wave(NhwWs ws, int flags )
{
	const int one_walk = flags & 1, marks = flags & 2;
	const int img = blockIdx.x * 4 + (threadIdx.x >> 6), lane = threadIdx.x & 63;
	__shared__ uint32_t dq_lut[(PH == WV_DQ1 || PH == WV_DQ0) ? DQ_WORDS : 1];
	if (PH == WV_DQ1 || PH == WV_DQ0) {
		for (int i = threadIdx.x; i < DQ_WORDS; i += 256) dq_lut[i] = dq_entry(i);
		__syncthreads();
	}
	if (img >= ws.n) return;
	Ctx c;
	ctx_load(&c, ws, img);
	if (PH == WV_DQ1) wave_dequant_sim_luma(&c, 1, lane, dq_lut, false, ws.dbg != 0);
	else if (PH == WV_DQ0) wave_dequant_sim_luma(&c, 0, lane, dq_lut, !ws.dbg, ws.dbg != 0, one_walk != 0, marks ? ws.buf<int16_t>(B_KMAP, img) : nullptr);
	else if (PH == WV_QUANT) {
		__shared__ __attribute__((aligned(16))) uint8_t park[4][16 * QROW];
		__shared__ uint32_t lut[4][QLUT + 3];
		PROF_BEGIN(); wave_quantise_luma(&c, lane, park[threadIdx.x >> 6], lut[threadIdx.x >> 6], ws.q > 21 || ws.dbg, NHW_DENSE_STREAM || ws.dbg, !(ws.q > 21 || ws.dbg), marks ? ws.buf<int16_t>(B_KMAP, img) : nullptr); if (!lane) PROF(&c, 15);
	}
	else if (PH == WV_EMIT) { PROF_BEGIN(); wave_emit_ll2(&c, lane, one_walk != 0); if (!lane) PROF(&c, 4); }
}
void nhw_launch_wave(int ph, const NhwWs &ws, hipStream_t s, bool one_walk, bool marks)
{
	const dim3 g((ws.n + 3) / 4), b(256);
	assert(!one_walk || ((ph == WV_EMIT || ph == WV_DQ0) && ws.q > 12 && !ws.dbg));
	assert(!marks || ((ph == WV_DQ0 || ph == WV_QUANT) && ws.q > 16 && !ws.dbg));
	(ph == WV_DQ1 ? k_wave<WV_DQ1> : ph == WV_DQ0 ? k_wave<WV_DQ0> : ph == WV_EMIT ? k_wave<WV_EMIT> : k_wave<WV_QUANT>)<<<g, b, 0, s>>>(ws, (one_walk ? 1 : 0) | (marks ? 2 : 0));
}

template <bool ANA, bool LEAN = false>
__global__ __launch_bounds__(1024) void k_l2_recon(int16_t *__restrict__ jpegb, int16_t *__restrict__ procb, size_t plane_stride, int16_t *__restrict__ ll1b, size_t ll1_stride, int n,
                                                   int16_t *__restrict__ saveb, size_t save_stride)
{
	extern __shared__ __attribute__((aligned(16))) int16_t smem[];
	constexpr int S = H, LS = S + 2, HLF = S / 2, PPL = HLF / 64, NT_ = 1024, NPRE = S * (S / 8) / NT_;
	const int t = threadIdx.x, lane = t & 63, wv = t >> 6;
	int16_t *A = smem;
	int8_t *ytab = reinterpret_cast<int8_t *>(A + S * LS);
	if (t < PRECOMP_TAB) ytab[t] = (int8_t)precomp_pick(t / 11 - 12, t % 11 - 5);
	uint4 pre[NPRE];
	if ((int)blockIdx.x < n) {
		const int16_t *src = jpegb + (size_t)blockIdx.x * plane_stride;
#pragma unroll
		for (int u = 0; u < NPRE; u++) { const int v = t + u * NT_; pre[u] = *reinterpret_cast<const uint4 *>(src + (size_t)(v / (S / 8)) * W + 8 * (v % (S / 8))); }
	}
	for (int img = blockIdx.x; img < n; img += gridDim.x) {
		int16_t *jp = jpegb + (size_t)img * plane_stride, *o = ll1b + (size_t)img * ll1_stride;
		int16_t *p = procb + (size_t)img * plane_stride;
#pragma unroll
		for (int u = 0; u < NPRE; u++) {
			const int v = t + u * NT_, row = v / (S / 8), c8 = v % (S / 8);
			uint32_t *d = reinterpret_cast<uint32_t *>(A + row * LS + 8 * c8);
			d[0] = pre[u].x; d[1] = pre[u].y; d[2] = pre[u].z; d[3] = pre[u].w;
		}
		lds_barrier();
		if (img + (int)gridDim.x < n) {
			const int16_t *src = jpegb + (size_t)(img + gridDim.x) * plane_stride;
#pragma unroll
			for (int u = 0; u < NPRE; u++) { const int v = t + u * NT_; pre[u] = *reinterpret_cast<const uint4 *>(src + (size_t)(v / (S / 8)) * W + 8 * (v % (S / 8))); }
		}
		const int r0 = wv * 16, c0 = 4 * lane;
		int side = 0;
		if (lane < 16) side = p[(size_t)(r0 + lane) * W - 1];
		else if (lane < 32) side = p[(size_t)(r0 + lane - 16) * W + H];
		else if (lane == 32) { side = o[(size_t)r0 * H - 1]; if (wv > 0) side = side > 14000 ? side - 16000 : side > 10000 ? side - 12000 : side; }
		else if (lane == 33) { side = o[(size_t)(r0 + 16) * H]; if (wv < 15) side = side > 14000 ? side - 16000 : side > 10000 ? side - 12000 : side; }
		for (int i = 0; i < 16; i++) {
			int16_t *x = A + (wv * 16 + i) * LS;
			int e[PPL], od[PPL];
#pragma unroll
			for (int u = 0; u < PPL; u++) syn_pair<S>(x, 1, lane + 64 * u, false, &e[u], &od[u]);
#pragma unroll
			for (int u = 0; u < PPL; u++) reinterpret_cast<uint32_t *>(x)[lane + 64 * u] = (uint32_t)(uint16_t)e[u] | ((uint32_t)(uint16_t)od[u] << 16);
		}
		lds_barrier();
#pragma unroll 4
		for (int i = 0; i < 16; i++) {
			int16_t *x = A + wv * 16 + i;
			int e[PPL], od[PPL];
#pragma unroll
			for (int u = 0; u < PPL; u++) syn_pair<S>(x, LS, lane + 64 * u, true, &e[u], &od[u]);
#pragma unroll
			for (int u = 0; u < PPL; u++) { const int k = lane + 64 * u; x[(2 * k) * LS] = (int16_t)e[u]; x[(2 * k + 1) * LS] = (int16_t)od[u]; }
		}
		lds_barrier();
		auto ll1_row = [&](int i) { return *reinterpret_cast<const uint2 *>(o + (size_t)(r0 + (i < 16 ? i : 15)) * H + c0); };
		auto untag = [](int v) { return v > 14000 ? v - 16000 : v > 10000 ? v - 12000 : v; };
		uint2 w0 = ll1_row(0), w1 = ll1_row(1), w2 = ll1_row(2), w3 = ll1_row(3);
#pragma unroll 1
		for (int i = 0; i < 16; i++) {
			const int r = r0 + i;
			int v[4];
			unpack4(w0, v);
			w0 = w1; w1 = w2; w2 = w3; w3 = ll1_row(i + 4);
			bool any = false;
#pragma unroll
			for (int k = 0; k < 4; k++) {
				const int step = v[k] > 14000 ? 1 : v[k] > 10000 ? -1 : 0;
				if (!step) continue;
				v[k] = untag(v[k]);
				any = true;
				const int j = c0 + k;
				if (r < HLF && j >= HLF) A[(2 * r) * LS + 2 * (j - HLF) + 1] += (int16_t)step;
				else if (r >= HLF && j < HLF) A[(2 * (r - HLF) + 1) * LS + 2 * j] += (int16_t)step;
				else if (r >= HLF && j >= HLF) A[(2 * (r - HLF) + 1) * LS + 2 * (j - HLF) + 1] += (int16_t)step;
			}
			if (any) {
				uint2 w;
				w.x = (uint32_t)(uint16_t)v[0] | ((uint32_t)(uint16_t)v[1] << 16); w.y = (uint32_t)(uint16_t)v[2] | ((uint32_t)(uint16_t)v[3] << 16);
				*reinterpret_cast<uint2 *>(o + (size_t)r * H + c0) = w;
			}
		}
		w0 = ll1_row(0); w1 = ll1_row(1); w2 = ll1_row(2); w3 = ll1_row(3);
		lds_barrier();
		int o_left = __builtin_amdgcn_readlane(side, 32);
#pragma unroll 1
		for (int i = 0; i < 16; i++) {
			const int r = r0 + i;
			int pv[4], ov[4], d[4], st[4];
			unpack4(w0, ov);
			const int o_right = i == 15 ? __builtin_amdgcn_readlane(side, 33) : untag((int)(int16_t)(__builtin_amdgcn_readlane((int)w1.x, 0) & 0xFFFF));
			w0 = w1; w1 = w2; w2 = w3; w3 = ll1_row(i + 4);
#pragma unroll
			for (int k = 0; k < 4; k++) { ov[k] = untag(ov[k]); pv[k] = A[(c0 + k) * LS + r]; d[k] = (int16_t)(pv[k] - ov[k]); }
			const int p_left = __shfl(side, i), p_right = __shfl(side, 16 + i);
			const int my_edge = lane ? p_right - o_right : p_left - o_left;
			o_left = __builtin_amdgcn_readlane(ov[3], 63);
			const int sd = __shfl_down(d[0], 1), su = __shfl_up(d[3], 1);
			const int dn4 = lane < 63 ? sd : my_edge;
			const int first = lane ? su : my_edge;
			const int nb[4] = { precomp_right(d[1]), precomp_right(d[2]), precomp_right(d[3]), precomp_right(dn4) };
			int prev_in = first;
			for (;;) {
				int prev = prev_in;
#pragma unroll
				for (int k = 0; k < 4; k++) { st[k] = ytab[precomp_index(d[k], nb[k] + prev)]; prev = d[k] + st[k]; }
				int np = __shfl_up(prev, 1);
				if (!lane) np = first;
				if (!__any(np != prev_in)) break;
				prev_in = np;
			}
			uint2 w;
			w.x = (uint32_t)(uint16_t)(ov[0] + st[0]) | ((uint32_t)(uint16_t)(ov[1] + st[1]) << 16); w.y = (uint32_t)(uint16_t)(ov[2] + st[2]) | ((uint32_t)(uint16_t)(ov[3] + st[3]) << 16);
			if (!ANA) *reinterpret_cast<uint2 *>(jp + (size_t)r * W + c0) = w;
			else {
				int lo[2], hi[2];
				ana_row_quad(w.x, w.y, lane, lo, hi);
				int16_t *x = A + (2 * lane) * LS + r;
				x[0] = (int16_t)lo[0]; x[LS] = (int16_t)lo[1]; x[HLF * LS] = (int16_t)hi[0]; x[(HLF + 1) * LS] = (int16_t)hi[1];
			}
// ... 40 lines not shown

__global__ __launch_bounds__(512) __attribute__((amdgpu_waves_per_eu(8, 8))) void k_chroma_loops(int16_t *__restrict__ cprocb, size_t plane_stride, int16_t *__restrict__ cll1b, size_t ll1_stride,
                                                      int16_t *__restrict__ saveb, size_t save_stride, const uint8_t *__restrict__ pub, size_t pu_stride,
                                                      int q, int comp, int compat)
{
	constexpr int S = H / 2, LS = S + 2, HLF = S / 2;
	__shared__ __attribute__((aligned(16))) int16_t A[S * LS];
	const int t = threadIdx.x, lane = t & 63, wv = t >> 6, img = blockIdx.x, r0 = wv * 16;
	int16_t *p = cprocb + (size_t)img * plane_stride, *o = cll1b + (size_t)img * ll1_stride, *save = saveb + (size_t)img * save_stride;
	const uint8_t *pu = pub + (size_t)img * pu_stride;
	const int behind = compat ? (int16_t)(pu[32768] | (pu[32769] << 8)) : 0;
	auto ll1_row = [&](int i) { return reinterpret_cast<const uint32_t *>(o + (size_t)(r0 + (i < 16 ? i : 15)) * S)[lane]; };
	uint32_t w0 = ll1_row(0), w1 = ll1_row(1), w2 = ll1_row(2), w3 = ll1_row(3);
	int side = 0;
	if (lane < 16) side = p[(size_t)(r0 + lane) * H + S];
	else if (lane == 16) side = wv < 7 ? o[(size_t)(r0 + 16) * S] : behind;
	if (t == 0) o[Q >> 2] = (int16_t)behind;
	auto ana_row = [&](int16_t *x, uint32_t w) {
		const uint32_t Dw[1] = { w };
		int lo[1], hi[1];
		ana_row_pair<1>(Dw, lane, lo, hi);
		x[lane] = (int16_t)lo[0]; x[HLF + lane] = (int16_t)hi[0];
	};
	auto columns = [&](const int loop , int16_t *out) {
		for (int i = 0; i < 8; i++) {
			const int c = r0 + 2 * i;
			uint32_t Ew[1], Ow[1];
			int lo[1][2], hi[1][2];
			Ew[0] = *reinterpret_cast<const uint32_t *>(A + (2 * lane) * LS + c); Ow[0] = *reinterpret_cast<const uint32_t *>(A + (2 * lane + 1) * LS + c);
			ana_col_pair<1, HLF>(Ew, Ow, c < HLF, lane, lo, hi);
			*reinterpret_cast<uint32_t *>(A + lane * LS + c) = (uint32_t)(uint16_t)lo[0][0] | ((uint32_t)(uint16_t)lo[0][1] << 16);
			*reinterpret_cast<uint32_t *>(A + (HLF + lane) * LS + c) = (uint32_t)(uint16_t)hi[0][0] | ((uint32_t)(uint16_t)hi[0][1] << 16);
			if (out)
#pragma unroll
				for (int h = 0; h < 2; h++) { int16_t *d = out + (size_t)(c + h) * S; d[lane] = (int16_t)lo[0][h]; d[HLF + lane] = (int16_t)hi[0][h]; }
		}
		for (int i = 0; i < 16; i++) {
			const int r = r0 + i, col0 = r < HLF ? HLF : 0;
			int16_t *x = A + r;
			int v[3] = { x[lane * LS], x[(HLF + lane) * LS], __builtin_amdgcn_readlane(side, i) };
			int ll = v[0];
			if (loop) {
				if (q <= 15) ll = (int16_t)((ll & 0xFFFC) + 1);
				else if ((r == 0) == (bool)(lane & 1)) ll = clear_bit0(ll);
			} else if (ll > 0 && ll < 256) ll = clear_bit0(ll);
			if (col0) v[0] = 0;
			uint64_t pair[2] = { 0, 0 };
			if (!loop) {
				const uint64_t m0 = __ballot(v[0] == -7 || v[0] == -8), m1 = __ballot(v[1] == -7 || v[1] == -8);
				const M4 m = M4{ { col0 ? 0 : m0, m1, 0, 0 } };
				const M4 fired = alt_runs(m & dn1(m) & col_range(col0, S - 2));
				const M4 both = fired | up1(fired);
				pair[0] = both.w[0]; pair[1] = both.w[1];
			}
			int dv[2] = { ll, 0 };
			for (int k = col0 ? 1 : 0; k < 2; k++) {
				int a = v[k];
				const int nx = right_of(v, k, 3, 1, lane);
				if (a < 0) {
					a = -a;
					if (nx < 0 && nx > -8) { if ((a & 7) < 6) a &= 0xFFF8; }
					else { if ((a & 7) < 7) a &= 0xFFF8; }
					a = -a;
				}
				dv[k] = ((pair[k] >> lane) & 1) ? -11 : dequant_value(a);
			}
			x[lane * LS] = (int16_t)dv[0]; x[(HLF + lane) * LS] = (int16_t)dv[1];
			int e, od;
			syn_pair<S>(x, LS, lane, false, &e, &od);
			x[(2 * lane) * LS] = (int16_t)e; x[(2 * lane + 1) * LS] = (int16_t)od;
		}
	};
	auto p3_step = [&](int d, int nx) {
		int step = 0;
		if (d > 10) step = -6; else if (d > 7) step = -3; else if (d > 4) step = -2; else if (d > 3) step = -1;
		else if (d > 2 && (comp ? nx > 0 : nx >= 0)) step = -1;
		else if (d < -10) step = 6; else if (d < -7) step = 3; else if (d < -4) step = 2; else if (d < -3) step = 1;
		else if (d < -2 && (comp ? nx < 0 : nx <= 0)) step = 1;
		return step;
	};
#pragma unroll 1
	for (int i = 0; i < 16; i++) { ana_row(A + (r0 + i) * LS, w0); w0 = w1; w1 = w2; w2 = w3; w3 = ll1_row(i + 4); }
	lds_barrier();
	columns(1, nullptr);
	w0 = ll1_row(0); w1 = ll1_row(1); w2 = ll1_row(2); w3 = ll1_row(3);
	lds_barrier();
#pragma unroll 1
	for (int i = 0; i < 16; i++) {
		int16_t *x = A + (r0 + i) * LS;
		int e, od;
		syn_pair<S>(x, 1, lane, true, &e, &od);
		const uint32_t ow = w0, ow_next = w1;
		w0 = w1; w1 = w2; w2 = w3; w3 = ll1_row(i + 4);
		const int oc0 = (int16_t)(ow & 0xFFFF), oc1 = (int)ow >> 16;
		int pn = __builtin_amdgcn_update_dpp(0, e, 0x130 , 0xF, 0xF, false);
		int on = (int16_t)(__builtin_amdgcn_update_dpp(0, (int)ow, 0x130, 0xF, 0xF, false) & 0xFFFF);
		if (lane == 63) {
			pn = __builtin_amdgcn_readlane(side, i);
			on = i < 15 ? (int16_t)(__builtin_amdgcn_readlane((int)ow_next, 0) & 0xFFFF) : __builtin_amdgcn_readlane(side, 16);
		}
		const int d0 = e - oc0, d1 = od - oc1, d2 = pn - on;
		ana_row(x, (uint32_t)(uint16_t)(oc0 + p3_step(d0, d1)) | ((uint32_t)(uint16_t)(oc1 + p3_step(d1, d2)) << 16));
	}
	lds_barrier();
	columns(0, save);
	lds_barrier();
#pragma unroll 1
	for (int i = 0; i < 16; i++) {
		int e, od;
		syn_pair<S>(A + (r0 + i) * LS, 1, lane, true, &e, &od);
		reinterpret_cast<uint32_t *>(p + (size_t)(r0 + i) * H)[lane] = (uint32_t)(uint16_t)e | ((uint32_t)(uint16_t)od << 16);
	}
}
void nhw_launch_chroma_loops(Plane<int16_t> cproc, Plane<int16_t> cll1, Plane<int16_t> cl2save, Plane<const uint8_t> pu, int q, int comp, int compat, int n, hipStream_t s)
{
	k_chroma_loops<<<n, 512, 0, s>>>(cproc.p, cproc.pitch, cll1.p, cll1.pitch, cl2save.p, cl2save.pitch, pu.p, pu.pitch, q, comp, compat);
}

__global__ __launch_bounds__(256) void k_copy_block(const int16_t *__restrict__ src, size_t src_plane, int src_row,
                                                    int16_t *__restrict__ dst, size_t dst_plane, int dst_row, int rows, int cols)
{
	const int16_t *sp = src + (size_t)blockIdx.x * src_plane;
	int16_t *dp = dst + (size_t)blockIdx.x * dst_plane;
	const int per = cols >> 3, n = rows * per;
	for (int i0 = threadIdx.x; i0 < n; i0 += 4 * 256) {
		uint4 v[4];
#pragma unroll
		for (int u = 0; u < 4; u++) { const int i = i0 + u * 256; if (i < n) v[u] = reinterpret_cast<const uint4 *>(sp + (size_t)(i / per) * src_row)[i % per]; }
#pragma unroll
		for (int u = 0; u < 4; u++) { const int i = i0 + u * 256; if (i < n) reinterpret_cast<uint4 *>(dp + (size_t)(i / per) * dst_row)[i % per] = v[u]; }
	}
}

static size_t phase_lds(int ph)
{
	const size_t tile = (size_t)NT * TLS * sizeof(int16_t);
	switch (ph) {
	case PH_L2: return 3 * 32 * 33 + 32;
	case PH_L3: return LL_LDS_BYTES;
	case PH_LLC: return LLC_LDS_BYTES;
	case PH_L4A: return RF_LDS_BYTES > (NT + 2) * TLS * sizeof(int16_t) ? RF_LDS_BYTES : (size_t)(NT + 2) * TLS * sizeof(int16_t);
	case PH_L4B: return (size_t)(NT + 2) * TLS * sizeof(int16_t);
	case PH_L4C: return 0;
	case PH_L4D: return SL_LDS_BYTES;
	case PH_C5: return CQ_LDS_BYTES > 32 * 130 * 2 + (32 * 128 + 258) * 2 ? CQ_LDS_BYTES : 32 * 130 * 2 + (32 * 128 + 258) * 2;
	default: return 0;
	}
}

int nhw_tail_set_attrs(const char **where)
{
#define SETATTR(fn) do { const hipError_t e_ = hipFuncSetAttribute(reinterpret_cast<const void *>(&fn), hipFuncAttributeMaxDynamicSharedMemorySize, 100 << 10); \
                         if (e_ != hipSuccess) { *where = "hipFuncSetAttribute(" #fn ", MaxDynamicSharedMemorySize)"; return (int)e_; } } while (0)
	SETATTR(k_phase<PH_L1>); SETATTR(k_phase<PH_L2>); SETATTR(k_phase<PH_L3>); SETATTR(k_phase<PH_C5>);
	for (const void *fn : { reinterpret_cast<const void *>(&k_l2_recon<false>), reinterpret_cast<const void *>(&k_l2_recon<true>), reinterpret_cast<const void *>(&k_l2_recon<true, true>) }) {
		const hipError_t e_ = hipFuncSetAttribute(fn, hipFuncAttributeMaxDynamicSharedMemorySize, (int)(H * (H + 2) * sizeof(int16_t) + 288));
		if (e_ != hipSuccess) { *where = "hipFuncSetAttribute(k_l2_recon, MaxDynamicSharedMemorySize)"; return (int)e_; }
	}
#undef SETATTR
	return 0;
}

void nhw_launch_phase(int ph, const NhwWs &ws, int comp, hipStream_t s)
{
	const dim3 g(ws.n), b(256);
	const size_t lds = phase_lds(ph);
#define PHASE(P) case P: k_phase<P><<<g, b, lds, s>>>(ws, comp); break
	switch (ph) {
	PHASE(PH_L1); PHASE(PH_L2); PHASE(PH_L3);
	case PH_L4A: if (ws.q >= 17) k_l4a<<<g, b, lds, s>>>(ws); else k_phase<PH_L4A><<<g, b, lds, s>>>(ws, comp); break;
	PHASE(PH_L4B); PHASE(PH_L4C);
	case PH_L4D: if (NHW_DENSE_STREAM || ws.dbg) k_phase<PH_L4D><<<g, b, lds, s>>>(ws, comp); else k_y31<<<g, 512, lds, s>>>(ws); break;
	PHASE(PH_LLC); PHASE(PH_L4C2); PHASE(PH_C0); PHASE(PH_C2); PHASE(PH_C3); PHASE(PH_C4); PHASE(PH_C5);
	}
#undef PHASE
}
void nhw_launch_pack_chroma(const NhwWs &ws, hipStream_t s)
{
	k_pack_chroma<<<ws.n, 256, PK_LDS_BYTES, s>>>(ws);
}
void nhw_launch_final(const NhwWs &ws, uint8_t *out, uint32_t *sizes, int32_t *status, hipStream_t s, bool chroma_packed)
{
	if (!chroma_packed) nhw_launch_pack_chroma(ws, s);
	k_final<<<ws.n, 256, PK_LDS_BYTES, s>>>(ws, out, sizes, status);
}

void nhw_launch_copy_block(Plane<const int16_t> src, int src_row, Plane<int16_t> dst, int dst_row, int rows, int cols, int n, hipStream_t s)
{
	if ((cols | src_row | dst_row) & 7 || (src.pitch | dst.pitch) & 7 || ((uintptr_t)src.p | (uintptr_t)dst.p) & 15) { fprintf(stderr, "nhw_launch_copy_block: block not 16-byte aligned\n"); abort(); }
	k_copy_block<<<n, 256, 0, s>>>(src.p, src.pitch, src_row, dst.p, dst.pitch, dst_row, rows, cols);
}
```

nhwcodec_amd/csrc/nhw_tail_par.h:

```cpp
#ifndef NHW_TAIL_PAR_H
#define NHW_TAIL_PAR_H

#include "nhw_tail_dev.h"
#include "nhw_tail_wave.h"

namespace nhw {

#define NT 256
#define BARRIER() __syncthreads()
#include "nhw_residual_rules.h"


DEV void tag_l2_details_par(Ctx *c, int tid)
{
	const int16_t *p = c->proc;
	for (int g = tid; g < Q / 8; g += NT) {
		const int r = g >> 5, j0 = (g & 31) * 8;
		if (r < H / 2 && j0 < H / 2) continue;
		const int at0 = r * W + j0;
		const uint4 pv = *reinterpret_cast<const uint4 *>(p + at0);
		uint4 cv = *reinterpret_cast<const uint4 *>(c->ll1 + r * H + j0);
		uint4 uv = make_uint4(0, 0, 0, 0), dv = uv;
		int u0 = 0, d7 = 0;
		if (r > 0) { uv = *reinterpret_cast<const uint4 *>(p + at0 - W); u0 = p[at0 - W - 1]; }
// ... 529 lines not shown
		BARRIER();
		if (tid < 2) carry[tid] = T[63 * FO_TP + 2 + H - 2 + tid];
		for (int jl = wv; jl < 64; jl += NT / 64) {
			const uint32_t *w = reinterpret_cast<const uint32_t *>(T + jl * FO_TP + 4 * lane);
			const uint32_t w0 = w[0], w1 = w[1] & 0xFFFFu;
			if (!(w0 | w1)) continue;
			const unsigned by[6] = { w0 & 255u, (w0 >> 8) & 255u, (w0 >> 16) & 255u, w0 >> 24, w1 & 255u, w1 >> 8 };
			uint2 *cell = reinterpret_cast<uint2 *>(f + (size_t)(64 * b + jl) * H + 4 * lane);
			uint2 v = *cell;
			int x[4] = { (int16_t)(v.x & 0xFFFF), (int16_t)(v.x >> 16), (int16_t)(v.y & 0xFFFF), (int16_t)(v.y >> 16) };
#pragma unroll
			for (int k = 0; k < 4; k++) x[k] += add[by[k + 2]] + add[32 + by[k + 1]] + add[64 + by[k]];
			v.x = (uint32_t)(uint16_t)x[0] | ((uint32_t)(uint16_t)x[1] << 16); v.y = (uint32_t)(uint16_t)x[2] | ((uint32_t)(uint16_t)x[3] << 16);
			*cell = v;
		}
	}
	BARRIER();
}

struct CleanP { int thresh, lim, lim2, last_look; };
template <int MODE>
DEV int clean_cell(const CleanP &f, int x, int n, int v1, int v2, bool look2, int &dout)
{
	const int ax = iabs(x);
	const bool keep = ax >= f.thresh, small = keep && ax < f.lim2, in_lim = x < f.lim && x > -f.lim;
	bool to7;
	if (MODE == 0) to7 = small && n < 3 && in_lim && ax > 6;
	else if (MODE == 1) to7 = small && ((n < 3 && in_lim) || !n);
	else to7 = small && n < 3;
	int e = keep ? x : 0;
	e = to7 ? (x < 0 ? -7 : 7) : e;
	const int nv1 = -v1;
	const bool big_p = e >= 8 && (e & 7) < 2, big_n = e < -7 && ((-e) & 7) < 2;
	const bool up1 = big_n && v1 < -14 && ((nv1 & 7) == 7 || ((nv1 & 7) < 2 && look2 && v2 <= 0));
	dout = (big_p && v1 > 7 && v1 < 10000) ? -1 : up1 ? 1 : 0;
	e = (e == -7 && v1 == 8) ? -8 : e;
	return e;
}
template <int MODE>
DEV int clean_row(const CleanP &f, const int o[4], uint2 up, uint2 dn, int my_far, int upt, int c0, int jb, int je, int lane, int e[4])
{
	typedef short s16x2_ __attribute__((ext_vector_type(2)));
	typedef unsigned short u16x2_ __attribute__((ext_vector_type(2)));
	const int left = __shfl_up(o[3], 1), sd0 = __shfl_down(o[0], 1), r2 = __shfl_down(o[1], 1);
	const int r1 = lane < 63 ? sd0 : my_far;
	auto loud2 = [](uint32_t w, uint32_t bias) {
		const s16x2_ v = __builtin_bit_cast(s16x2_, w);
		const u16x2_ a = __builtin_bit_cast(u16x2_, __builtin_elementwise_max(v, -v));
		return __builtin_bit_cast(uint32_t, (u16x2_)((a + __builtin_bit_cast(u16x2_, bias)) >> (u16x2_)(15)));
	};
	const uint32_t bu = 0x80008000u - 0x00010001u * (uint32_t)upt, b6 = 0x7FFA7FFAu;
	const uint32_t s01 = loud2(up.x, bu) + loud2(dn.x, b6), s23 = loud2(up.y, bu) + loud2(dn.y, b6);
	int n[4]; bool proc[4];
#pragma unroll
	for (int k = 0; k < 4; k++) {
		const int j = c0 + k;
		proc[k] = j >= jb && j < je;
		const int lv = k ? o[k ? k - 1 : 0] : left, rv = k < 3 ? o[k < 3 ? k + 1 : k] : r1;
		const int lt = (MODE == 2 && j - 1 >= jb) ? 7 : 6;
		n[k] = (iabs(lv) >= lt) + (iabs(rv) >= 6) + (int)(((k < 2 ? s01 : s23) >> (16 * (k & 1))) & 3u);
	}
	int din = 0, dd = 0, d0out = 0;
#pragma unroll
	for (int k = 0; k < 4; k++) {
		const int x = o[k] + dd;
		if (proc[k]) {
			const int v1 = k < 3 ? o[k < 3 ? k + 1 : k] : r1, v2 = k < 2 ? o[k < 2 ? k + 2 : k] : (k == 2 ? r1 : r2);
			e[k] = clean_cell<MODE>(f, x, n[k], v1, v2, c0 + k < f.last_look, dd);
		} else { e[k] = x; dd = 0; }
		if (k == 0) d0out = dd;
	}
	int dout = dd;
	for (;;) {
		int nd = __shfl_up(dout, 1);
		if (!lane) nd = 0;
		if (!__any(nd != din)) break;
		din = nd;
		int d0 = 0;
		{
			const int x = o[0] + din;
			if (proc[0]) e[0] = clean_cell<MODE>(f, x, n[0], o[1], o[2], c0 < f.last_look, d0);
			else e[0] = x;
		}
		if (__any(d0 != d0out)) {
			d0out = d0; dd = d0;
#pragma unroll
			for (int k = 1; k < 4; k++) {
				const int x = o[k] + dd;
				if (proc[k]) {
					const int v1 = k < 3 ? o[k < 3 ? k + 1 : k] : r1, v2 = k < 2 ? o[k < 2 ? k + 2 : k] : (k == 2 ? r1 : r2);
					e[k] = clean_cell<MODE>(f, x, n[k], v1, v2, c0 + k < f.last_look, dd);
				} else { e[k] = x; dd = 0; }
			}
			dout = dd;
		}
	}
	return dout;
}
DEV void clean_details_seq(Ctx *c, int tid, bool ll_in_plane )
{
	int16_t *p = c->proc;
	const int q = c->q, lane = tid & 63, wv = tid >> 6;
	const CleanP fa = { DEADZONE - 2, q > 22 ? 8 : 9, q > 22 ? 4 : 9, W - 2 };
	const CleanP fb = { DEADZONE - 2, q > 17 ? 8 : 9, q > 22 ? 4 : 9, H - 2 };
	const int lim = q > 22 ? 8 : 11;
	const CleanP fc = { DEADZONE - 1, lim, lim, W - 2 };
	auto ld = [&](int r, int c0) { return *reinterpret_cast<const uint2 *>(p + (size_t)r * W + c0); };
	auto st = [&](int r, int c0, const int e[4]) {
		uint2 w;
		w.x = (uint32_t)(uint16_t)e[0] | ((uint32_t)(uint16_t)e[1] << 16); w.y = (uint32_t)(uint16_t)e[2] | ((uint32_t)(uint16_t)e[3] << 16);
		*reinterpret_cast<uint2 *>(p + (size_t)r * W + c0) = w;
	};
	const int cl = 4 * lane, ch = H + 4 * lane;
	const int lo0 = H + 64 * wv, lo1 = lo0 + 63 < W - 2 ? lo0 + 63 : W - 2;
	const uint2 hh_below = ld(lo1 + 1, ch);
	BARRIER();
	{
		const int r0 = 1 + 64 * wv, r1 = r0 + 63 < H - 2 ? r0 + 63 : H - 2;
		uint2 up = ld(r0 - 1, ch), cur = ld(r0, ch), dn = ld(r0 + 1, ch);
		for (int r = r0; r <= r1; r++) {
			const uint2 nx = ld(r + 2 < W ? r + 2 : r + 1, ch);
			int o[4], e[4];
			unpack4(cur, o);
			clean_row<0>(fa, o, up, dn, 0, 6, ch, H + 1, W - 1, lane, e);
			st(r, ch, e);
			up = cur; cur = dn; dn = nx;
		}
	}
	{
		uint2 upl = (wv == 0 && !ll_in_plane) ? *reinterpret_cast<const uint2 *>(c->l2save + (size_t)(H - 1) * H + cl) : ld(lo0 - 1, cl), curl = ld(lo0, cl), dnl = ld(lo0 + 1, cl);
		uint2 uph = ld(lo0 - 1, ch), curh = ld(lo0, ch), dnh = lo0 + 1 > lo1 ? hh_below : ld(lo0 + 1, ch);
		for (int r = lo0; r <= lo1; r++) {
			const int rn = r + 2 < W ? r + 2 : W - 1;
			const uint2 nxl = ld(rn, cl);
			const uint2 nxh = r + 2 > lo1 ? (r + 2 == lo1 + 1 ? hh_below : make_uint2(0, 0)) : ld(rn, ch);
			int o[4], e[4];
			unpack4(curl, o);
			const int my_far = (int16_t)((uint32_t)__builtin_amdgcn_readfirstlane((int)curh.x) & 0xFFFFu);
			const int dout = clean_row<1>(fb, o, upl, dnl, my_far, 6, cl, 1, H, lane, e);
			st(r, cl, e);
			const int moved = __builtin_amdgcn_readlane(dout, 63);
			unpack4(curh, o);
			if (lane == 0) o[0] += moved;
			clean_row<2>(fc, o, uph, dnh, 0, r > H ? 7 : 6, ch, H + 1, W - 1, lane, e);
			st(r, ch, e);
			upl = curl; curl = dnl; dnl = nxl;
			uph = curh; curh = dnh; dnh = nxh;
		}
	}
}

#define CQROW 264
#define CQ_LDS_BYTES (4 * 16 * CQROW + 2 * (H + 2))
DEV void quantise_chroma_par(Ctx *c, int comp, int tid, int16_t *lds, bool write_plane, bool dense )
{
	unsigned vtotal = 0;
	int16_t *p = c->cproc;
	uint8_t *ubytes = c->ubytes;
	uint8_t *scan = c->scan + 4 * Q;
	const int lane = tid & 63, wv = tid >> 6;
	uint8_t *park = reinterpret_cast<uint8_t *>(lds) + wv * 16 * CQROW;
	int16_t *nf = lds + 4 * 16 * CQROW / 2;
	nf[tid + 1] = p[(tid + 1) * H];
	BARRIER();
	int cur[4], nxt[4] = { 0, 0, 0, 0 };
	const int r0 = 64 * wv;
	for (int k = 0; k < 4; k++) cur[k] = p[r0 * H + lane + 64 * k];
	for (int i = 0; i < 64; i++) {
		const int r = r0 + i;
		if (i + 1 < 64) for (int k = 0; k < 4; k++) nxt[k] = p[(r + 1) * H + lane + 64 * k];
		const int first_next = nf[r + 1];
		unsigned P, S, T;
		BS_PRED(P, cur, 4, (unsigned)(x + 8) < 2u); BS_PRED(S, cur, 4, x > 6 && x <= 127 && (x & 7) >= 6); BS_PRED(T, cur, 4, x == 7);
		const unsigned inrow = lane == 63 ? 0x7u : 0xFu;
		const unsigned pc = P & bs_dn(P, lane) & inrow, bc = S & bs_dn(T, lane) & inrow;
		const unsigned pf = __any(pc != 0) ? bs_from4(alt_runs(bs_ballot4(pc))) : 0u;
		const unsigned bf = __any(bc != 0) ? bs_from4(alt_runs(bs_ballot4(bc))) : 0u;
		const unsigned pair = pf | bs_up<4>(pf, lane), raised = bs_up<4>(bf, lane);
		for (int k = 0; k < 4; k++) {
			const int x = cur[k], nx = right_of_dpp(cur, k, 4, lane, first_next);
			int a = (raised >> k) & 1 ? 8 : x;
			const bool neg = a < 0;
			int m = neg ? -a : a;
			const bool keep = (nx < 0 && nx > -8) ? (m & 7) >= 6 : (m & 7) == 7;
			m = (neg && !keep) ? (m & 504) : m;
			a = neg ? -m : m;
			int sym = (unsigned)(a + DEADZONE - 1) < (unsigned)(2 * DEADZONE - 1) ? 128 : ((a + 128) & 248);
			sym = (pair >> k) & 1 ? 120 : sym;
			if (__ballot(x > 127 || x < -127)) {
				if (x == 12400) sym = 124; else if (x == 12600) sym = 126; else if (x == 12900) sym = 122; else if (x == 13000) sym = 130;
				else if (x > 127) sym = big_code(x, k_big_pos);
				else if (x < -127) sym = big_code(-x, k_big_neg);
			}
			if (write_plane) p[r * H + lane + 64 * k] = (int16_t)sym;
			park[(i & 15) * CQROW + lane + 64 * k] = (uint8_t)sym;
		}
		if ((i & 15) == 15) {
			__threadfence_block();
			const int strip = lane >> 1, rb = r - 15 + 8 * (lane & 1);
			uint32_t w[16];
			for (int j = 0; j < 8; j++) {
				const uint2 x = *reinterpret_cast<const uint2 *>(park + (8 * (lane & 1) + j) * CQROW + 8 * strip);
				if ((rb + j) & 1) { w[2 * j] = __builtin_bswap32(x.y); w[2 * j + 1] = __builtin_bswap32(x.x); } else { w[2 * j] = x.x; w[2 * j + 1] = x.y; }
			}
			const int pos = strip * (8 * H) + 8 * rb;
			if (!comp) { for (int j = 0; j < 4; j++) reinterpret_cast<uint4 *>(ubytes + pos)[j] = make_uint4(w[4 * j], w[4 * j + 1], w[4 * j + 2], w[4 * j + 3]); }
			else {
				uint32_t o[32];
				for (int j = 0; j < 4; j++) {
					const uint4 u4 = reinterpret_cast<const uint4 *>(ubytes + pos)[j];
					const uint32_t uu[4] = { u4.x, u4.y, u4.z, u4.w };
					for (int e = 0; e < 4; e++) {
						const uint32_t u = uu[e], v = w[4 * j + e];
						o[8 * j + 2 * e] = (u & 0xFF) | ((v & 0xFF) << 8) | ((u & 0xFF00) << 8) | ((v & 0xFF00) << 16);
						o[8 * j + 2 * e + 1] = ((u >> 16) & 0xFF) | (((v >> 16) & 0xFF) << 8) | ((u >> 24) << 16) | ((v >> 24) << 24);
					}
				}
				if (dense) for (int j = 0; j < 8; j++) reinterpret_cast<uint4 *>(scan + 2 * pos)[j] = make_uint4(o[4 * j], o[4 * j + 1], o[4 * j + 2], o[4 * j + 3]);
				const int F = 4 * wv + (i >> 4);
				const uint64_t M0 = (uint64_t)ne_mask32(o, 0x80808080u) | (uint64_t)ne_mask32(o + 8, 0x80808080u) << 32;
				const uint64_t M1 = (uint64_t)ne_mask32(o + 16, 0x80808080u) | (uint64_t)ne_mask32(o + 24, 0x80808080u) << 32;
				*reinterpret_cast<uint4 *>(c->cnzq + (F * 64 + lane) * 2) = make_uint4((uint32_t)M0, (uint32_t)(M0 >> 32), (uint32_t)M1, (uint32_t)(M1 >> 32));
				const unsigned cnt = (unsigned)(__builtin_popcountll(M0) + __builtin_popcountll(M1));
				unsigned incl = cnt;
				for (int o_ = 1; o_ < 64; o_ <<= 1) { const unsigned t_ = (unsigned)__shfl_up((int)incl, o_); if (lane >= o_) incl += t_; }
				if (lane == 0) { c->cfbase[F] = 32768u * wv + vtotal; c->cfbase[16 + wv] = vtotal + (unsigned)__builtin_amdgcn_readlane((int)incl, 63); }
				uint8_t *vp = c->cvals + 32768u * wv + vtotal + incl - cnt;
				vtotal += (unsigned)__builtin_amdgcn_readlane((int)incl, 63);
				uint32_t *sw = reinterpret_cast<uint32_t *>(park);
				static_assert(16 * CQROW >= 16 * 64 * 4, "a slice of every lane fits the parked rows");
#pragma unroll
				for (int hs = 0; hs < 2; hs++) {
					__builtin_amdgcn_fence(__ATOMIC_SEQ_CST, "wavefront"); __builtin_amdgcn_wave_barrier();
#pragma unroll
					for (int k = 0; k < 16; k++) sw[64 * k + lane] = o[16 * hs + k];
					__builtin_amdgcn_fence(__ATOMIC_SEQ_CST, "wavefront"); __builtin_amdgcn_wave_barrier();
					const uint8_t *sb = reinterpret_cast<const uint8_t *>(sw) + 4 * lane;
					for (uint64_t m = hs ? M1 : M0; m; m &= m - 1) {
						const int bit = __builtin_ctzll(m);
						*vp++ = sb[256 * (bit >> 2) + (bit & 3)];
					}
				}
			}
			__threadfence_block();
		}
		for (int k = 0; k < 4; k++) cur[k] = nxt[k];
	}
}

DEV bool is_pm8(int v) { return v == 136 || v == 120; }
DEV bool pair_cand(const uint8_t *s, int c, int n)
{
	return c >= 0 && c <= n - 5 && is_pm8(s[c]) && s[c + 1] == 128 && s[c + 2] == 128 && s[c + 3] == 128 && is_pm8(s[c + 4]);
}
DEV void fix_sign_code(uint8_t *s, int at) { if (s[at] == 153) s[at] = 124; else if (s[at] == 155) s[at] = 123; }

DEV void scan_and_rewrite_par(Ctx *c, int tid, int *sh_counts, uint32_t *sh_z , int16_t *lds )
{
	const int16_t *p = c->proc;
	uint8_t *s = c->scan;
	const int n = 4 * Q;
	PROF_BEGIN();
	uint32_t *bits = reinterpret_cast<uint32_t *>(c->half);

	if (tid == 0) { sh_counts[0] = 0; sh_counts[1] = 0; }
	BARRIER();

#define WIN_LOAD(dst_, base) do { const uint4 a_ = *reinterpret_cast<const uint4 *>(s + (base) - 16), b_ = *reinterpret_cast<const uint4 *>(s + (base)), \
		c_ = (base) + 16 < n ? *reinterpret_cast<const uint4 *>(s + (base) + 16) : make_uint4(0, 0, 0, 0);    \
		dst_[0] = a_.x; dst_[1] = a_.y; dst_[2] = a_.z; dst_[3] = a_.w; dst_[4] = b_.x; dst_[5] = b_.y; dst_[6] = b_.z; dst_[7] = b_.w; dst_[8] = c_.x; dst_[9] = c_.y; dst_[10] = c_.z; dst_[11] = c_.w; } while (0)
#define WB(w, k) ((int)(((w)[((k) + 16) >> 2] >> (8 * (((k) + 16) & 3))) & 0xFF))
#define PM8(v) ((v) == 136 || (v) == 120)
#define WIN_MASK(w, pat) ((unsigned long long)(~ne_mask32((w) + 2, pat)) << 8)
#define Z4(x) ((((~((((x) ^ 0x80808080u) & 0x7F7F7F7Fu) + 0x7F7F7F7Fu | ((x) ^ 0x80808080u) | 0x7F7F7F7Fu)) >> 7) * 0x00204081u) >> 21 & 15u)
#define HASZ(x) ((((x) - 0x01010101u) & ~(x)) & 0x80808080u)
#define ANY_PM8(w) ((HASZ((w)[4] ^ 0x88888888u) | HASZ((w)[5] ^ 0x88888888u) | HASZ((w)[6] ^ 0x88888888u) | HASZ((w)[7] ^ 0x88888888u) | \
                     HASZ((w)[4] ^ 0x78787878u) | HASZ((w)[5] ^ 0x78787878u) | HASZ((w)[6] ^ 0x78787878u) | HASZ((w)[7] ^ 0x78787878u)) != 0)
	for (int w = tid; w < n / 32; w += NT) bits[w] = 0;
	if (tid < 4) sh_z[n / 16 / 32 + tid] = 0;
	BARRIER();
	if (!tid) PROF(c, 40);
	for (int base = 16 * tid; base < n; base += 16 * NT) {
		uint32_t w[12];
		WIN_LOAD(w, base);
		{
			const unsigned long long mask = __ballot(w[4] == 0x80808080u && w[5] == 0x80808080u && w[6] == 0x80808080u && w[7] == 0x80808080u);
			if ((tid & 63) == 0) { sh_z[base >> 9] = (uint32_t)mask; sh_z[(base >> 9) + 1] = (uint32_t)(mask >> 32); }
		}
		if (!ANY_PM8(w)) continue;
		const unsigned long long Zm = WIN_MASK(w, 0x80808080u), P = WIN_MASK(w, 0x88888888u) | WIN_MASK(w, 0x78787878u);
		unsigned long long hit = P & (Zm >> 1) & (Zm >> 2) & (Zm >> 3) & (P >> 4) & 0xFFFF0000ull;
		if (base > n - 5 - 15) hit &= (1ull << (n - 4 - base + 16)) - 1;
		const unsigned long long prev = (P << 4) & (Zm << 3) & (Zm << 2) & (Zm << 1);
		while (hit) {
			const int j = __ffsll((long long)hit) - 1, cpos = base + j - 16;
			hit &= hit - 1;
			int m = 1, back = cpos - 4;
			if (back >= 0 && ((prev >> j) & 1)) {
				m++; back -= 4;
				while (pair_cand(s, back, n)) { m++; back -= 4; }
			}
			if (m & 1) atomicOr(&bits[cpos >> 5], 1u << (cpos & 31));
		}
	}
	BARRIER();
	if (!tid) PROF(c, 41);
	for (int w = tid; w < n / 32; w += NT) {
		uint32_t word = bits[w];
		while (word) {
			const int cpos = (w << 5) + __ffs((int)word) - 1;
			word &= word - 1;
			const int x = s[cpos], y = s[cpos + 4];
			s[cpos] = (uint8_t)(x == 136 ? (y == 136 ? 132 : 133) : (y == 136 ? 134 : 135));
			s[cpos + 4] = 201;
		}
	}
	BARRIER();
	if (tid < 4) { s[tid] = 128; s[n - 4 + tid] = 128; }
	BARRIER();

	if (!tid) PROF(c, 42);
	{
		int n1 = 0, n2 = 0;
		for (int base = 16 * tid; base < n; base += 16 * NT) {
			uint32_t w[12];
			WIN_LOAD(w, base);
			if (!ANY_PM8(w)) continue;
			const unsigned long long Zm = WIN_MASK(w, 0x80808080u), P6 = WIN_MASK(w, 0x88888888u), P0 = WIN_MASK(w, 0x78787878u), P = P6 | P0;
			unsigned long long act = P & 0xFFFF0000ull;
			unsigned long long left = P << 1;
			if (base == 0) { act &= ~0xFull << 16; left &= ~0x1Full << 16; }
			if (base == n - 16) act &= (1ull << 28) - 1;
			const unsigned long long before4 = (Zm << 1) & (Zm << 2) & (Zm << 3) & (Zm << 4);
			const unsigned long long after3 = (Zm >> 2) & (Zm >> 3) & (Zm >> 4);
			const unsigned long long taken = left & (Zm >> 1) & (((Zm << 2) & (Zm << 3) & (Zm << 4) & (Zm << 5)) | ((Zm << 2) & after3));
			act &= ~taken;
			const unsigned long long pairA = act & (P >> 1) & (Zm >> 2) & (before4 | ((Zm << 1) & (Zm >> 3) & (Zm >> 4) & (Zm >> 5)));
			const unsigned long long lone = act & ~pairA & (Zm >> 1) & (before4 | ((Zm << 1) & after3));
			for (unsigned long long h = pairA; h; h &= h - 1) {
				const int j = __ffsll((long long)h) - 1;
				s[base + j - 15] = (uint8_t)(((P0 >> (j + 1)) & 1) ? 157 : 159);
			}
			for (unsigned long long h = lone; h; h &= h - 1) {
				const int j = __ffsll((long long)h) - 1;
				s[base + j - 16] = (uint8_t)(((P6 >> j) & 1) ? 153 : 155);
			}
			n2 += __popcll(pairA); n1 += __popcll(lone);
		}
		if (n1) atomicAdd(&sh_counts[0], n1);
		if (n2) atomicAdd(&sh_counts[1], n2);
	}
	BARRIER();
	if (tid == 0) { c->m->select1 = sh_counts[0]; c->m->select2 = sh_counts[1]; }

	if (!tid) PROF(c, 43);
	int *cand = reinterpret_cast<int *>(lds);
	if (!tid) cand[0] = 0;
	BARRIER();
	for (int base = 16 * tid; base < n; base += 16 * NT) {
		const int gi = base >> 4;
		unsigned long long zz;
		if (gi) { const int g = gi - 1; zz = ((unsigned long long)sh_z[(g >> 5) + 1] << 32 | sh_z[g >> 5]) >> (g & 31); }
		else zz = ((unsigned long long)sh_z[1] << 32 | sh_z[0]) << 1;
		if (((zz >> 2) & 0x3FFF) != 0x3FFF) continue;
		int i;
		if ((zz >> 1) & 1) {
			if (zz & 1) continue;
			if (base > 0 && s[base - 1] == 128) continue;
			i = base;
		} else {
			const uint4 o = *reinterpret_cast<const uint4 *>(s + base);
			const unsigned own = Z4(o.x) | (Z4(o.y) << 4) | (Z4(o.z) << 8) | (Z4(o.w) << 12);
			const int tz = __clz((int)~(own << 16));
			if (tz == 0) continue;
			i = base + 16 - tz;
		}
		cand[1 + atomicAdd(&cand[0], 1)] = i;
	}
	BARRIER();
	const int ncand = cand[0];
	for (int ci = tid; ci < ncand; ci += NT) {
		const int i = cand[1 + ci];
		{
			int b;
			{
				int g2 = (i >> 4) + 1;
				for (;;) {
					const uint32_t inv = ~(sh_z[g2 >> 5] >> (g2 & 31));
					const int room = 32 - (g2 & 31);
					const int z = inv ? __ffs((int)inv) - 1 : 32;
					if (z >= room) { g2 += room; if (g2 >= n / 16) break; continue; }
					g2 += z; break;
				}
				b = 16 * g2 - 1;
				if (b + 1 < n) {
					const uint4 e = *reinterpret_cast<const uint4 *>(s + b + 1);
// ... 1076 lines not shown
		const int16_t *lo = c->first_order + rr * H, *hi = b + rr * H;
		HqIn in;
		in.lw = *reinterpret_cast<const uint2 *>(lo + k0); in.hw = *reinterpret_cast<const uint2 *>(hi + k0);
		in.l4 = k0 + 4 < H ? (int)lo[k0 + 4] : 0x7fffffff; in.h0 = k0 > 0 ? (int)hi[k0 - 1] : 0x7fffffff; in.h5 = k0 + 4 < H ? (int)hi[k0 + 4] : 0x7fffffff;
		in.kw = *reinterpret_cast<const uint4 *>(c->keep + rr * W + 2 * k0);
		return in;
	};
	HqIn nin = hq_fetch(tid);
	for (int idx = tid; idx < Q / 4; idx += NT) {
		const int rr = idx >> 6, k0 = (idx & 63) * 4;
		int n_q3 = 0, n_e = 0, n_c = 0;
		const HqIn in = nin;
		if (idx + NT < Q / 4) nin = hq_fetch(idx + NT);
		int l[5], h[6];
		{
			const uint2 lw = in.lw, hw = in.hw;
			l[0] = (int16_t)(lw.x & 0xFFFF); l[1] = (int16_t)(lw.x >> 16); l[2] = (int16_t)(lw.y & 0xFFFF); l[3] = (int16_t)(lw.y >> 16);
			h[1] = (int16_t)(hw.x & 0xFFFF); h[2] = (int16_t)(hw.x >> 16); h[3] = (int16_t)(hw.y & 0xFFFF); h[4] = (int16_t)(hw.y >> 16);
			l[4] = in.l4 != 0x7fffffff ? in.l4 : l[3];
			h[0] = in.h0 != 0x7fffffff ? in.h0 : h[1];
			h[5] = in.h5 != 0x7fffffff ? in.h5 : h[4];
		}
		const uint4 kw = in.kw;
		const uint32_t kk[4] = { kw.x, kw.y, kw.z, kw.w };
		uint32_t out[4];
#pragma unroll
		for (int t = 0; t < 4; t++) {
			int16_t o[2];
			o[0] = (int16_t)((int16_t)(l[t] << 3) - ((h[t + 1] + h[t]) << 1));
			o[1] = (int16_t)((int16_t)((l[t] + l[t + 1]) << 2) + (6 * h[t + 1] - h[t] - h[t + 2]));
			for (int e = 0; e < 2; e++) {
				const int d = (int16_t)(kk[t] >> (16 * e)) - o[e];
				if (iabs(d) > thr) o[e] = (int16_t)((q > 22 && iabs(d) > 56) ? (d > 0 ? 32000 : 32500) : (d > 0 ? 30000 : 31000));
			}
			out[t] = (uint32_t)(uint16_t)o[0] | ((uint32_t)(uint16_t)o[1] << 16);
			for (int e = 0; e < 2; e++) {
				n_q3 += o[e] == 32000 || o[e] == 32500;
				const bool hit = o[e] == 30000 || o[e] == 31000;
				if ((lane == 31 || lane == 63) && t == 3) { if (lane == 31) n_c += hit; } else n_e += hit;
			}
		}
		*reinterpret_cast<uint4 *>(hs + rr * W + 2 * k0) = make_uint4(out[0], out[1], out[2], out[3]);
		int t_q3 = 0, t_e = 0;
		for (int bit = 0; bit < 4; bit++) { t_q3 += __popcll(__ballot((n_q3 >> bit) & 1)) << bit; t_e += __popcll(__ballot((n_e >> bit) & 1)) << bit; }
		const int t_c = __builtin_amdgcn_readlane(n_c, 31);
		if (!lane) { sh[rr] = t_q3; sh[H + rr] = t_e | (t_c << 16); }
	}
	BARRIER();
	if (!tid) PROF(c, 51);
	auto load8 = [&](const int16_t *rowp, int v[8]) {
		const uint4 w = reinterpret_cast<const uint4 *>(rowp)[lane];
		const uint32_t ww[4] = { w.x, w.y, w.z, w.w };
		for (int e = 0; e < 4; e++) { v[2 * e] = (int16_t)(ww[e] & 0xFFFF); v[2 * e + 1] = (int16_t)(ww[e] >> 16); }
	};
	const unsigned q3_r = (unsigned)sh[r], e_r = (unsigned)sh[H + r] & 0xFFFFu, nc_r = (unsigned)sh[H + r] >> 16;
	BARRIER();
	unsigned te, tc;
	const unsigned aq_r = block_exscan(q3_r, tid, shm, &tot);
	const unsigned ae_r = block_exscan(e_r, tid, shm, &te);
	const unsigned ac_r = block_exscan(nc_r, tid, shm, &tc);
	sh[r] = (int)aq_r; sh[H + r] = (int)(ae_r | (ac_r << 20));
	BARRIER();
	if (!tid) PROF(c, 52);
	uint8_t *raw = c->raw, *pay = c->pay;
	for (int row = wv; row < H; row += NT / 64) {
		int v[8], cnt = 0, nq = 0, total, tq;
		load8(hs + (size_t)row * W, v);
		const bool special = lane == 31 || lane == 63;
		for (int e = 0; e < 8; e++) { nq += v[e] == 32000 || v[e] == 32500; if (e < (special ? 6 : 8)) cnt += v[e] == 30000 || v[e] == 31000; }
		if (tot) {
			int at = sh[row] + wave_exscan(nq, tq);
			for (int e = 0; e < 8; e++) {
				const int i = row * W + 8 * lane + e;
				if (v[e] == 32000) c->qsetting3[at++] = (uint32_t)(i << 1);
				else if (v[e] == 32500) c->qsetting3[at++] = (uint32_t)(i << 1) + 1;
			}
		}
		const int off = wave_exscan(cnt, total);
		const int first_half = __shfl(off, 32);
		const int base_e = sh[H + row] & 0xFFFFF;
		int ae = base_e + off;
		int an = ae + 2 * row + (lane >= 32);
		for (int e = 0; e < (special ? 6 : 8); e++) {
			if (v[e] == 30000) { raw[an++] = (uint8_t)((8 * lane + e) & 255); pay[ae++] = 0; }
			else if (v[e] == 31000) { raw[an++] = (uint8_t)((8 * lane + e) & 255); pay[ae++] = 1; }
		}
		if (lane == 31) {
			raw[base_e + 2 * row + first_half] = H - 2;
			int ac = sh[H + row] >> 20;
			if (v[6] == 30000) c->char_res1[ac++] = (uint16_t)(row * H); else if (v[6] == 31000) c->char_res1[ac++] = (uint16_t)(row * H + 1);
			if (v[7] == 30000) c->char_res1[ac++] = (uint16_t)(row * H + 2); else if (v[7] == 31000) c->char_res1[ac++] = (uint16_t)(row * H + 3);
		}
		if (lane == 63) raw[base_e + 2 * row + total + 1] = H - 2;
	}
	BARRIER();
	if (tid == 0) { c->m->qsetting3_len = (int)tot; c->m->char_res1_len = (int)tc; sh[0] = (int)(te + 2 * H); sh[1] = (int)te; }
	BARRIER();
	poslist_finish_par(c, &c->res6, raw, sh[0], pay, sh[1], 1, tid, shm);
	BARRIER();
	if (!tid) PROF(c, 16);
}
DEV void luma_p4d_par(Ctx *c, int tid, int *sh_counts, uint32_t *sh_z, int16_t *lds, bool dense)
{
	PROF_BEGIN();
	scan_rewrite_list_par<NT>(c, tid, reinterpret_cast<uint8_t *>(lds), sh_counts);
	if (dense) {
		BARRIER();
		scan_and_rewrite_par(c, tid, sh_counts, sh_z, lds);
	}
	if (!tid) PROF(c, 17);
}

DEV void chroma_p0_par(Ctx *c, int comp, int tid)
{
	const uint8_t *src = comp ? c->pv : c->pu;
	for (int idx = tid; idx < Q / 4; idx += NT) {
		const uint32_t v = reinterpret_cast<const uint32_t *>(src)[idx];
		uint2 o;
		o.x = (v & 0xFF) | (((v >> 8) & 0xFF) << 16);
		o.y = ((v >> 16) & 0xFF) | ((v >> 24) << 16);
		reinterpret_cast<uint2 *>(c->cjpeg)[idx] = o;
	}
}
DEV void chroma_ll1_neighbour(Ctx *c, int tid)
{
	if (!tid) c->cll1[Q >> 2] = (int16_t)(c->compat ? (c->pu[32768] | (c->pu[32769] << 8)) : 0);
}
DEV void chroma_p3_par(Ctx *c, int comp, int tid)
{
	int16_t *jp = c->cjpeg, *p = c->cproc, *o = c->cll1;
	for (int g = tid; g < Q / 32; g += NT) {
		const int r = g >> 4, j0 = (g & 15) * 8, e0 = r * H + j0, k0 = r * (H / 2) + j0;
		const uint4 pv = *reinterpret_cast<const uint4 *>(p + e0), ov = *reinterpret_cast<const uint4 *>(o + k0);
		const int p8 = p[e0 + 8], o8 = o[k0 + 8];
		const uint32_t pw[4] = { pv.x, pv.y, pv.z, pv.w }, ow[4] = { ov.x, ov.y, ov.z, ov.w };
		int pc[9], oc[9];
#pragma unroll
		for (int t = 0; t < 8; t++) { pc[t] = (int16_t)(pw[t >> 1] >> (16 * (t & 1))); oc[t] = (int16_t)(ow[t >> 1] >> (16 * (t & 1))); }
		pc[8] = p8; oc[8] = o8;
		uint32_t out[4] = { 0, 0, 0, 0 };
#pragma unroll
		for (int t = 0; t < 8; t++) {
			const int d = pc[t] - oc[t], nx = pc[t + 1] - oc[t + 1];
			int step = 0;
			if (d > 10) step = -6; else if (d > 7) step = -3; else if (d > 4) step = -2; else if (d > 3) step = -1;
			else if (d > 2 && (comp ? nx > 0 : nx >= 0)) step = -1;
			else if (d < -10) step = 6; else if (d < -7) step = 3; else if (d < -4) step = 2; else if (d < -3) step = 1;
			else if (d < -2 && (comp ? nx < 0 : nx <= 0)) step = 1;
			out[t >> 1] |= (uint32_t)(uint16_t)(oc[t] + step) << (16 * (t & 1));
		}
		*reinterpret_cast<uint4 *>(jp + e0) = make_uint4(out[0], out[1], out[2], out[3]);
	}
}
DEV void chroma_p5_par(Ctx *c, int comp, int tid, int16_t *lds, int *sh_misc, bool write_plane)
{
	int16_t *p = c->cproc, *o = c->cll1;
	const int q = c->q;
	PROF_BEGIN();
	if (q >= 18) {
		const int res_uv = q > 17 ? 4 : 5;
		const int lane = tid & 63, wv = tid >> 6;
		int *shift = reinterpret_cast<int *>(lds), *haz = shift + H / 2;
		bool last_cand = false;
		if (tid < H / 2) {
			shift[tid] = 0; haz[tid] = 0;
			const int at = tid * H + H / 2 - 1, ko = tid * (H / 2) + H / 2 - 1;
			const int d = p[at] - o[ko], d1 = p[tid * H + H / 2] - o[ko + 1];
			const bool pair = (d > 3 && d < 7 && d1 > 2 && d1 < 7) || (d < -3 && d > -7 && d1 < -2 && d1 > -8);
			last_cand = pair && (iabs(p[at + H / 2]) < 8 || iabs(p[at + Q / 2]) < 8 || iabs(p[at + Q / 2 + H / 2]) < 8);
		}
		const int first_pass = __syncthreads_or(last_cand) ? 0 : 1;
		for (int pass = first_pass;; pass++) {
			bool mark = false;
			if (pass > 0) {
				int ns = 0;
				if (tid < H / 2) for (int r = 0; r < tid; r++) ns += haz[r];
				const int changed = __syncthreads_or(tid < H / 2 && ns != shift[tid]);
				if (tid < H / 2) shift[tid] = ns;
				BARRIER();
				mark = !changed;
			}
			int16_t nx[12];
			auto fetch = [&](int r) {
				const int sh = shift[r];
#pragma unroll
				for (int k = 0; k < 2; k++) {
					const int at = r * H + lane + 64 * k, ko = r * (H / 2) + sh + lane + 64 * k;
					nx[6 * k] = p[at]; nx[6 * k + 1] = p[at + H / 2]; nx[6 * k + 2] = p[at + Q / 2]; nx[6 * k + 3] = p[at + Q / 2 + H / 2];
					nx[6 * k + 4] = o[ko]; nx[6 * k + 5] = o[ko + 1];
				}
			};
			fetch(wv);
			for (int r = wv; r < H / 2; r += 4) {
				int pl[2], hl[2], lh[2], hh[2], d[2], d1[2];
#pragma unroll
				for (int k = 0; k < 2; k++) {
					pl[k] = nx[6 * k]; hl[k] = nx[6 * k + 1]; lh[k] = nx[6 * k + 2]; hh[k] = nx[6 * k + 3];
					d[k] = pl[k] - nx[6 * k + 4];
					d1[k] = nx[6 * k + 5];
				}
				if (r + 4 < H / 2) fetch(r + 4);
				const int hl_first = __shfl(hl[0], 0);
				for (int k = 0; k < 2; k++) {
					int pn = right_of(pl, k, 2, 1, lane);
					if (k == 1 && lane == 63) pn = hl_first;
					d1[k] = pn - d1[k];
				}
				uint64_t pp[2], pn_[2], fr[2], sg[2], fhl[2], flh[2], m5[2];
				for (int k = 0; k < 2; k++) {
					pp[k] = __ballot(d[k] > 3 && d[k] < 7 && d1[k] > 2 && d1[k] < 7);
					pn_[k] = __ballot(d[k] < -3 && d[k] > -7 && d1[k] < -2 && d1[k] > -8);
					fhl[k] = __ballot(iabs(hl[k]) < 8); flh[k] = __ballot(iabs(lh[k]) < 8);
					fr[k] = fhl[k] | flh[k] | __ballot(iabs(hh[k]) < 8);
					sg[k] = __ballot(iabs(d[k]) > res_uv && (d[k] > 0 || d[k] != -5 || d1[k] < 0));
					m5[k] = __ballot(d[k] == -5);
				}
				uint64_t f[2] = { (pp[0] | pn_[0]) & fr[0], (pp[1] | pn_[1]) & fr[1] };
				if ((fhl[0] & 1) && ((f[0] | sg[0]) & 1)) {
					f[1] &= ~(1ull << 63);
					if (m5[1] >> 63) sg[1] &= ~(1ull << 63);
				}
				const M4 fired = alt_runs(M4{ { f[0], f[1], 0, 0 } });
				if (!mark) { if (lane == 0) haz[r] = (int)(fired.w[1] >> 63); continue; }
				const M4 vis = ~up1(fired);
				for (int k = 0; k < 2; k++) {
					const bool pair = (fired.w[k] >> lane) & 1;
					const bool single = !pair && ((vis.w[k] >> lane) & 1) && ((sg[k] >> lane) & 1);
					if (!pair && !single) continue;
					const int16_t code = pair ? (((pp[k] >> lane) & 1) ? 12400 : 12600) : (d[k] > 0 ? 12900 : 13000);
					const int at = r * H + lane + 64 * k;
					if (iabs(hl[k]) < 8) p[at + H / 2] = code;
					else if (iabs(lh[k]) < 8) p[at + Q / 2] = code;
					else if (iabs(hh[k]) < 8) p[at + Q / 2 + H / 2] = code;
				}
			}
			BARRIER();
			if (mark) break;
		}
		if (tid == 0) { int ev = 0; for (int r = 0; r < H / 2; r++) ev += haz[r]; c->m->pad = comp ? c->m->pad + (ev << 8) : ev; }
	}
	BARRIER();
	if (!tid) PROF(c, 27);
	copy_block_par(c->cl2save, H / 2, p, H, H / 2, H / 2, tid);
	for (int idx = tid; idx < (H / 4) * (H / 4); idx += NT) lds[idx] = c->cl2save[(idx >> 6) * (H / 2) + (idx & 63)];
	BARRIER();
	if (q <= 11 && tid < 64) {
		const int L = H / 4, lane = tid;
		for (int pass = 0; pass < 2; pass++)
			for (int t = 0; t < (L - 2) + 2 * (L - 3); t++) {
				const int r = lane, j = t - 2 * lane;
				if (r < L - 2 && j >= 0 && j < L - 2) {
					int16_t *v = lds + r * L + j;
					if (!pass) {
						if (iabs(v[1] - v[2 * L + 1]) < 5 && iabs(v[L] - v[L + 2]) < 5 && iabs(v[L + 1] - v[L]) < 7 && iabs(v[1] - v[L + 1]) < 8)
							v[L + 1] = (int16_t)((v[1] + v[2 * L + 1] + v[L] + v[L + 2] + 2) >> 2);
					} else {
						if (iabs(v[2] - v[1]) < 5 && iabs(v[1] - v[0]) < 5 && iabs(v[0] - v[L]) < 5 && iabs(v[2] - v[L + 2]) < 5 &&
						    iabs(v[2 * L + 1] - v[L]) < 5 && iabs(v[L] - v[L + 1]) < 8)
							v[L + 1] = (int16_t)((v[1] + v[2 * L + 1] + v[L] + v[L + 2] + 1) >> 2);
					}
				}
			}
	}
	BARRIER();
	if (!tid) PROF(c, 28);
	{
		unsigned *shm = reinterpret_cast<unsigned *>(lds + 4096);
		const int e0 = c->m->exw_len, base = comp ? (Q >> 2) + (Q >> 4) : (Q >> 2);
		int nexc = 0, lastgood = -1;
		for (int u = 0; u < 16; u++) {
			const int idx = tid * 16 + u, s = lds[idx];
			if ((s > 255 || s < 0) && idx > 0) nexc++; else lastgood = idx;
		}
		unsigned total;
		const unsigned eoff = block_exscan((unsigned)nexc, tid, shm, &total);
		int lg = (int)block_exscan_max((unsigned)(lastgood + 1), tid, shm) - 1;
		uint32_t w[4] = { 0, 0, 0, 0 };
		uint8_t *ex = c->exw + e0 + 2 + 3 * eoff;
		for (int u = 0; u < 16; u++) {
			const int idx = tid * 16 + u, s = lds[idx];
			if ((s > 255 || s < 0) && idx > 0) {
				const int mag = s > 255 ? s - 255 : -s;
				*ex++ = (uint8_t)(idx >> 6);
				*ex++ = (uint8_t)((idx & 63) + (s > 255 ? 128 : 0));
				*ex++ = (uint8_t)(mag > 255 ? 255 : mag);
			} else lg = idx;
			int v = lds[lg];
			v = v > 255 ? 255 : (v < 0 ? 0 : v);
			w[u >> 2] |= (uint32_t)(v & 254) << (8 * (u & 3));
		}
		*reinterpret_cast<uint4 *>(c->ll_bytes + base + tid * 16) = make_uint4(w[0], w[1], w[2], w[3]);
		BARRIER();
		if (tid == 0) { c->exw[e0] = 0; c->exw[e0 + 1] = 0; c->m->exw_len = e0 + 2 + 3 * (int)total; }
	}
	for (int idx = tid; idx < (H / 4) * (H / 4); idx += NT) p[(idx >> 6) * H + (idx & 63)] = 0;
	BARRIER();
	{
		uint8_t *dst = comp ? c->res_v64 : c->res_u64;
		const uint8_t *sb = c->ll_bytes + (comp ? 20480 : 16384);
		for (int i = tid; i < 16 * H / 8; i += NT) {
			int v = 0;
			for (int b = 0; b < 8; b++) v = (v << 1) | ((sb[8 * i + b] >> 1) & 1);
			dst[i] = (uint8_t)v;
		}
	}
	if (!tid) PROF(c, 21);
	BARRIER();
	quantise_chroma_par(c, comp, tid, lds, write_plane, write_plane);
	if (!tid) PROF(c, 22);
}


#define PK_SLICE 64
#define PK_SCAN(sh) ((sh)->n2 + 150)
#define PK_CHUNK (PK_SLICE * NT)
struct PackShared {
	union { struct { int hist[256], runs[256]; }; struct { uint32_t code_sym[256], code_run[256]; }; };
	union { struct { unsigned bits[NT], n1[NT], n2[160]; }; struct { unsigned weight[360]; uint16_t entry[600]; }; };
	uint16_t sorted[360];
	int k, select, zone, top_is_zero, rc;
	unsigned total_bits, total_n1, total_n2;
	int stale_len;
};

DEV bool book_ok(int v) { return v < 109 ? !(v & 1) : (v == 112 || (v >= 120 && v < 141) || (v >= 144 && !(v & 3))); }

struct SliceBits { uint32_t b[4]; uint64_t s1m, s2m; };

#define PK_LDS_BYTES ((17 * NT + 1) * 4)
struct PackPreL { uint64_t M; uint32_t off; uint4 v[4]; int prev_nz, next_nz; };
DEV void pack_fetch_list(const Ctx *c, const uint8_t *vals, int ch, int tid, PackPreL *pre, const int *prevnz, const int *nextnz)
{
	const int g = ch * NT + tid;
	pre->prev_nz = prevnz[g]; pre->next_nz = nextnz[g + 1];
	pre->M = c->nzs[g]; pre->off = c->voff[g];
	const int cnt = __builtin_popcountll(pre->M);
	const uint8_t *v = vals + (pre->off & 0x1FFFFFFFu);
#pragma unroll
	for (int k = 0; k < 4; k++) if (cnt > 16 * k) __builtin_memcpy(&pre->v[k], v + 16 * k, 16);
}
DEV const uint8_t *pack_stage_list(const PackPreL *pre, int tid, uint32_t *lw)
{
	uint32_t *w = lw + 17 * tid;
	const int cnt = __builtin_popcountll(pre->M);
#pragma unroll
	for (int k = 0; k < 4; k++) if (cnt > 16 * k) { w[4 * k] = pre->v[k].x; w[4 * k + 1] = pre->v[k].y; w[4 * k + 2] = pre->v[k].z; w[4 * k + 3] = pre->v[k].w; }
	return reinterpret_cast<const uint8_t *>(w);
}
template <int MODE>
DEV void pack_walk_list(uint64_t nz, int skip, const uint8_t *vb, int N, int lo, int hi, PackShared *sh, uint32_t *words, unsigned bit0, uint8_t *s1, unsigned i1, uint8_t *s2, unsigned i2,
                        unsigned *out_bits, unsigned *out_n1, unsigned *out_n2, int prev_nz, int next_nz, SliceBits *rec = nullptr)
{
	unsigned bits = 0, n1 = 0, n2 = 0;
	uint32_t cur = 0; int w = (int)(bit0 >> 5), fill = (int)(bit0 & 31);
	uint32_t r0 = 0, r1 = 0, r2 = 0, r3 = 0; uint64_t s1m = 0, s2m = 0;
	const int select = sh->select;
#define EMIT(entry) do { const uint32_t e_ = (entry), code_ = e_ & 0xFFFFFF; const int len_ = (int)(e_ >> 24); \
		if (MODE == 1) { \
			r0 = (r0 << len_) | (r1 >> (32 - len_)); r1 = (r1 << len_) | (r2 >> (32 - len_)); r2 = (r2 << len_) | (r3 >> (32 - len_)); r3 = (r3 << len_) | code_; \
			bits += (unsigned)len_; \
		} \
		else { fill += len_; if (fill <= 32) cur |= code_ << (32 - fill); \
			else { const int sp_ = fill - 32; atomicOr(&words[w], cur | (code_ >> sp_)); w++; cur = (code_ & ((1u << sp_) - 1)) << (32 - sp_); fill = sp_; } } } while (0)
	const int send = lo + PK_SLICE < N ? lo + PK_SLICE : N;
	int i = lo, vi = 0;
	if (MODE != 0 && skip) { i = lo + skip; vi = __builtin_popcountll(nz & ((1ull << skip) - 1)); }
	uint64_t rest = nz >> (i - lo);
	while (i < hi) {
		if (rest & 1) {
			const int px = vb[vi++];
			if (MODE == 0) { atomicAdd(&sh->hist[px], 1); i++; rest >>= 1; continue; }
			if (px == 153 || px == 155) { if (MODE == 2 && s1 && i1 + n1 < S_CAP) s1[i1 + n1] = (uint8_t)(px == 155); if (MODE == 1 && px == 155) s1m |= 1ull << n1; n1++; i++; rest >>= 1; continue; }
			if (px == 157 || px == 159) { if (MODE == 2 && s2 && i2 + n2 < S_CAP) s2[i2 + n2] = (uint8_t)(px == 159); if (MODE == 1 && px == 159) s2m |= 1ull << n2; n2++; i++; rest >>= 1; continue; }
			EMIT(sh->code_sym[px]);
			if (px > 131 && px < 136) { vi += __builtin_popcount((unsigned)rest & 0x1Eu); i += 5; rest >>= 5; } else { i++; rest >>= 1; }
			continue;
		}
		int a = i, b;
		if (i == lo && i > 0 && prev_nz != lo - 1) a = prev_nz + 1;
		if (rest) b = i + __builtin_ctzll(rest) - 1;
		else b = send < N ? next_nz - 1 : send - 1;
		const int L = b - a + 1;
		if (L == 1) {
			if (MODE == 0) atomicAdd(&sh->hist[128], 1); else EMIT(sh->code_sym[128]);
		} else if (a == i && L < 255) {
			if (MODE == 0) atomicAdd(&sh->runs[L], 1);
			else if (L < select) { for (int z = 0; z < L; z++) EMIT(sh->code_sym[128]); }
			else EMIT(sh->code_run[L]);
		} else {
			const int m = L > 255 ? (L - 255 + 253) / 254 : 0;
			int k1 = (hi - 1 - a) / 254;
			if (k1 > m) k1 = m;
			for (int k = (i - a + 253) / 254; k <= k1; k++) {
				const int len = k < m ? 254 : L - 254 * m;
				if (MODE == 0) atomicAdd(&sh->runs[len], 1);
				else if (len < select) { for (int z = 0; z < len; z++) EMIT(sh->code_sym[128]); }
				else EMIT(sh->code_run[len]);
			}
		}
		rest = (b + 1 - i) < 64 ? rest >> (b + 1 - i) : 0;
		i = b + 1;
	}
	if (MODE == 2 && fill > 0) atomicOr(&words[w], cur);
	if (MODE == 1) {
		*out_bits = bits; *out_n1 = n1; *out_n2 = n2;
		if (bits <= 128u) {
			const unsigned sh_ = 128u - bits, ws_ = sh_ >> 5, bs_ = sh_ & 31;
			const uint32_t w_[7] = { r0, r1, r2, r3, 0u, 0u, 0u };
			uint32_t x_[5];
#pragma unroll
			for (int k_ = 0; k_ < 5; k_++) x_[k_] = ws_ == 0 ? w_[k_] : ws_ == 1 ? w_[k_ + 1] : ws_ == 2 ? w_[k_ + 2] : ws_ == 3 ? w_[(k_ + 3) < 7 ? k_ + 3 : 6] : 0u;
#pragma unroll
			for (int k_ = 0; k_ < 4; k_++) rec->b[k_] = bs_ ? (x_[k_] << bs_) | (x_[k_ + 1] >> (32 - bs_)) : x_[k_];
		}
		rec->s1m = s1m; rec->s2m = s2m;
	}
#undef EMIT
}
DEV void pack_chroma_order(Ctx *c, int tid)
{
	const int F = tid >> 4, e0 = 8 * (tid & 15);
	uint64_t m[8];
	unsigned tot = 0;
	for (int k = 0; k < 8; k++) { m[k] = c->cnzq[F * 128 + e0 + k]; tot += (unsigned)__builtin_popcountll(m[k]); }
	unsigned incl = tot;
	for (int o = 1; o < 16; o <<= 1) { const unsigned t_ = (unsigned)__shfl_up((int)incl, o, 16); if ((tid & 15) >= o) incl += t_; }
	unsigned at = c->cfbase[F] + incl - tot;
	const int wv = F >> 2, turn = F & 3;
	for (int k = 0; k < 8; k++) {
		const int e = e0 + k, lane = e >> 1, half = e & 1;
		const int S = 64 * (lane >> 1) + 16 * wv + 4 * turn + 2 * (lane & 1) + half;
		uint64_t M = m[k];
		if (S == 2 * Q / 64 - 1) M = (M & ~(1ull << 63)) | ((M >> 62) & 1ull) << 63;
		c->nzs[S] = M; c->voff[S] = at;
		at += (unsigned)__builtin_popcountll(m[k]);
	}
}

template <int PART>
DEV void pack_words_par(Ctx *c, PackShared *sh, int tid, uint32_t *lw )
{
	constexpr int part = PART;
	const uint8_t *vals = part ? c->cvals : c->vals;
	const int N = part ? 2 * Q : 4 * Q;
	if (part) { pack_chroma_order(c, tid); __threadfence_block(); BARRIER(); }
	const int S = N - 1, nchunks = (S + PK_CHUNK - 1) / PK_CHUNK;
	const int nsl = nchunks * NT;

	int *prevnz = reinterpret_cast<int *>(c->raw), *nextnz = prevnz + nsl + 8;

	PROF_BEGIN();
	sh->hist[tid] = 0; sh->runs[tid] = 0;
	if (tid == 0) { sh->select = part ? 3 : 4; sh->zone = 0; sh->rc = NHW_OK; }
	for (int ch = 0; ch < nchunks; ch++) {
		const int g = ch * NT + tid, lo = g * PK_SLICE;
		const uint64_t nz = c->nzs[g];
		prevnz[g] = nz ? lo + 63 - __builtin_clzll(nz) : -1;
		nextnz[g] = nz ? lo + __builtin_ctzll(nz) : N;
	}
	BARRIER();
	{
// ... 330 lines not shown
```

profiles/make_design_table.py:

```python
import json, os, re, sys
ROOT = os.path.dirname(os.path.dirname(os.path.abspath(__file__)))
STATS = os.path.join(ROOT, "profiles", "l2_dead_stores_kernel_stats_1stream_after.txt")
PMC = os.path.join(ROOT, "profiles", "l2_dead_stores_pmc_after.json")
BATCHES = 7.0
PH = ["L1", "L2", "L3", "L4A", "C0", "C2", "C3", "C4", "C5", "FINAL", "L4B", "L4C", "L4D", "LLC", "L4C2"]
WV = ["DQ1", "DQ0", "EMIT", "QUANT"]
WHAT = {
    "k_front_image": "a1 + a2 + Y2 + Y3 fused: BGR24 -> Y, 4:2:0 chroma planes out, pre-filter (carry chained in the kernel), both directions of the level-1 analysis, LL copy; a workgroup walks an image (32 rows a band, 512 threads, 78 KB LDS)",
    "k_front_plain": "the same without the pre-filter (q >= 22; q <= 16 and the analysis stage from a luma plane): horizontal pass from registers, 64 rows a band",
    "k_dwt_ana<256>": "level-2 luma analysis of the first closed loop, from ll1, without its transposed plane (whole block in LDS, persistent workgroups); the second loop's only for q <= 12 and the stage checks, level-1 chroma analysis only for q <= 14 and the stage checks",
    "k_chroma_l1q": "level-1 chroma analysis from the 4:2:0 byte plane, a quarter of the 256 x 256 block to a workgroup (four a CU); its coefficients are part of SURVEY's 6 B/pixel",
    "k_dwt_ana<128>": "level-2 chroma analysis (only the tests' stage checks run it)",
    "k_chroma_loops": "both chroma closed loops of a component on one LDS residency of its level-2 block: analysis, simulation 1, synthesis, pre-compensation, analysis (+ cl2save), simulation 2, synthesis (four workgroups a CU)",
    "k_dwt_syn<256>": "level-2 luma synthesis of the second closed loop",
    "k_dwt_syn<128>": "level-2 chroma synthesis (only the tests' stage checks run it)",
    "k_l2_recon": "first closed loop: level-2 synthesis + Y8 (tags -> reconstruction) + Y9 (LL1 pre-compensation) + the second level-2 analysis with Y13's copy on one LDS residency of the block; a batch's form stores l2save and rows 0 .. 127 of the work plane's block",
    "L1": "Y5 tag level-2 details", "L2": "Y8, Y9 as a kernel of their own (only the tests' stage checks run it)", "L3": "Y16 LL2 coder (parse), on a stream of its own beside the second dequantiser simulation",
    "L4A": "Y19-Y23: small runs (wavefront per row), residual classification (one table-driven step for every kind) and coding (column walks on LDS tiles)",
    "L4B": "Y24, Y25 position lists + list packing", "L4C": "Y27 detail clean-up (a wavefront takes 64 consecutive rows, neighbours in registers; Y26 only for q >= 22)", "L4D": "Y31 rewrites, on the symbol LIST (non-zero map + values); leaves map and offsets in stream order",
    "L4C2": "Y29 (q >= 22): band reconstruction, half synthesis, res6 / char_res1 / qsetting3 lists",
    "C0": "chroma: copy", "C2": "chroma: dequantiser simulation 1", "C3": "chroma: tags", "C4": "chroma: dequantiser simulation 2",
    "C5": "chroma: marks (running-index fixed point), LL2 emission, quantiser (wavefront per row); V leaves the merged chroma stream as a list", "LLC": "Z1 chroma LL2 coder", "FINAL": "Z2 packetiser + container",
    "k_l4a": "Y19-Y23 of q >= 17: Y21 small runs (wavefront per row, rows in which nothing fires skipped), Y22 + Y23 as ONE column sweep on registers and class tables (eight workgroups a CU)",
    "k_y31": "Y31 rewrites on the symbol LIST (non-zero map + values), 512 threads an image; leaves map and offsets in stream order",
    "k_final": "Z2 packetiser (the luma part from its symbol list, both books) + container; a kernel of its own at six wavefronts a SIMD",
    "k_pack_chroma": "Z2's chroma part: words and ranked book entries from the chroma symbol list (on the chroma stream in the forked order)",
    "DQ1": "a8 dequantiser simulation, first closed loop (wavefront per image)", "DQ0": "a8 dequantiser simulation, second closed loop",
    "EMIT": "Y14/Y15 LL2 emission", "QUANT": "Y28 luma quantiser + Y30: the symbols leave as a list in stream order (wavefront per image); reads the level-2 block from l2save (Y26)",
}


def label(name):
    m = re.match(r"void k_phase<(\d+)>", name)
    if m:
        return f"`k_phase<{PH[int(m.group(1))]}>`", WHAT.get(PH[int(m.group(1))], "")
    m = re.match(r"void k_wave<(\d+)>", name)
    if m:
        return f"`k_wave<{WV[int(m.group(1))]}>`", WHAT.get(WV[int(m.group(1))], "")
    short = name.replace("void ", "").replace("nhw::", "").split("(")[0]
    base = re.sub(r"<.*", "", short)
    return f"`{short}`", WHAT.get(short, WHAT.get(base, ""))


def table():
    pmc = json.load(open(PMC))
    rows, tot_ms, tot_gb = [], 0.0, 0.0
    for ln in open(STATS):
        m = re.match(r"(.{78})\s+(\d+)\s+([\d.]+)\s+([\d.]+)", ln)
        if not m or "at::" in ln or "rocclr" in ln or "k_synth" in ln:
            continue
        name = m.group(1).strip().split("(")[0]
        calls, total = int(m.group(2)), float(m.group(3))
        key = max((k for k in pmc if len(k.strip()) >= 5 and name.startswith(k.strip())), key=len, default=None)
        rd = wr = None
        if key and "FETCH_SIZE" in pmc[key] and "WRITE_SIZE" in pmc[key]:
            rd = 2 * pmc[key]["FETCH_SIZE"]["per_launch"] * 1024 / 1e9 * calls / BATCHES
            wr = pmc[key]["WRITE_SIZE"]["per_launch"] * 1024 / 1e9 * calls / BATCHES
        rows.append((total / BATCHES, name, calls / BATCHES, rd, wr))
        tot_ms += total / BATCHES; tot_gb += (rd or 0) + (wr or 0)
    out = ["| kernel | passes | launches | ms | HBM read + written, GB | TB/s |", "|---|---|---|---|---|---|"]
    for ms, name, calls, rd, wr in sorted(rows, reverse=True):
        lab, what = label(name)
        gb = f"{rd:.2f} + {wr:.2f}" if rd is not None else "n/a"
        tbs = f"{(rd + wr) / ms:.2f}" if rd is not None and ms else ""
        out.append(f"| {lab} | {what} | {calls:.0f} | {ms:.2f} | {gb} | {tbs} |")
    out.append(f"| **sum (one stream, nothing overlaps)** | | | **{tot_ms:.1f}** | **{tot_gb:.1f}** | |")
    return "\n".join(out)


def main():
    path = os.path.join(ROOT, "DESIGN.md")
    s = open(path).read()
    a, b = s.index("<!-- KERNEL_TABLE_BEGIN -->"), s.index("<!-- KERNEL_TABLE_END -->")
    new = s[:a] + "<!-- KERNEL_TABLE_BEGIN -->\n" + table() + "\n" + s[b:]
    if "--check" in sys.argv:
        sys.exit(0 if new == s else 1)
    open(path, "w").write(new)


if __name__ == "__main__":
    main()
```

Before: 65280.

## Fuse chroma marks and quantiser into one row walk in a dedicated tail kernel

Adds a k_chroma_tail kernel that computes only the per-row shifts of the chroma marks pass, then marks and quantises each plane row in registers in a single walk instead of writing marks into cproc, copying the LL2 block and re-reading the plane for quantisation. The quantiser symbol logic and the flush are factored into reusable helpers, and quiet rows are skipped early. The aim is to cut plane read/write traffic and barriers in the chroma tail, at the cost of more registers and LDS (two park buffers per wavefront). The old phase path is kept behind an environment flag and for debug runs.

Result: faster. 67130 (median of 6 runs) (+2.8%).

```diff
diff --git a/include/nhw_hip_debug.h b/include/nhw_hip_debug.h
--- a/include/nhw_hip_debug.h
+++ b/include/nhw_hip_debug.h
@@ -19,6 +19,7 @@
 
 int nhw_stage_chroma_loops(nhw_enc *e, int n, int comp, int form, void *stream);
 int nhw_debug_write(nhw_enc *e, int buf, int img, const void *src, size_t bytes);
+int nhw_stage_chroma_tail(nhw_enc *e, int n, int comp, int form, void *stream);
 int nhw_stage_luma_loop(nhw_enc *e, int n, int form, void *stream);
 int nhw_stage_ll2_walk(nhw_enc *e, int n, int form, void *stream);
 int nhw_stage_quant(nhw_enc *e, int n, int form, void *stream);
diff --git a/nhwcodec_amd/__init__.py b/nhwcodec_amd/__init__.py
--- a/nhwcodec_amd/__init__.py
+++ b/nhwcodec_amd/__init__.py
@@ -61,6 +61,7 @@
     L.nhw_stage_prefilter.argtypes = [P, P, ctypes.c_int, ctypes.c_int, P]
     L.nhw_stage_chroma_l1.argtypes = [P, ctypes.c_int, P]
     L.nhw_stage_chroma_loops.argtypes = [P, ctypes.c_int, ctypes.c_int, ctypes.c_int, P]
+    L.nhw_stage_chroma_tail.argtypes = [P, ctypes.c_int, ctypes.c_int, ctypes.c_int, P]
     L.nhw_stage_luma_loop.argtypes = [P, ctypes.c_int, ctypes.c_int, P]
     L.nhw_stage_ll2_walk.argtypes = [P, ctypes.c_int, ctypes.c_int, P]
     L.nhw_stage_quant.argtypes = [P, ctypes.c_int, ctypes.c_int, P]
diff --git a/nhwcodec_amd/csrc/nhw_enc.h b/nhwcodec_amd/csrc/nhw_enc.h
--- a/nhwcodec_amd/csrc/nhw_enc.h
+++ b/nhwcodec_amd/csrc/nhw_enc.h
@@ -33,6 +33,7 @@
 	int quant_join;
 	int y5_fork;
 	int ll2_once;
+	int chroma_tail_once;
 	int quant_marks;
 	int pack_fork;
 	int parts;
diff --git a/nhwcodec_amd/csrc/nhw_enc.hip b/nhwcodec_amd/csrc/nhw_enc.hip
--- a/nhwcodec_amd/csrc/nhw_enc.hip
+++ b/nhwcodec_amd/csrc/nhw_enc.hip
@@ -91,6 +91,7 @@
 	e->y5_fork = env("NHW_Y5_FORK", 1) != 0;
 	e->ll2_once = env("NHW_LL2_ONCE", 1) != 0;
 	e->quant_marks = env("NHW_QUANT_MARKS", 1) != 0;
+	e->chroma_tail_once = env("NHW_CHROMA_TAIL_ONCE", 1) != 0;
 	e->pack_fork = within(env("NHW_PACK_FORK", 2), 0, 2, 2);
 	*out = e;
 	return NHW_OK;
@@ -262,9 +263,10 @@
 	ws.defer_verbatim = fork_ll;
 	hipStream_t cs = fork ? e->part_stream[0] : s;
 	ws.split_chroma = fork;
+	const bool tail_once = e->chroma_tail_once && !e->stop_after && !ws.dbg;
 	auto chroma_head = [&](int comp) -> int { return chroma_head_launches(e, ws, comp, n, cs, stage); };
 	auto chroma_tail = [&](int comp) -> int {
-		nhw_launch_phase(PH_C5, ws, comp, cs);
+		nhw_launch_chroma_tail(ws, comp, tail_once, cs);
 		STAGE_DONE();
 		return 1;
 	};
@@ -554,6 +556,23 @@
 	return NHW_OK;
 }
 
+extern "C" int nhw_stage_chroma_tail(nhw_enc *e, int n, int comp, int form, void *stream)
+{
+	if (!e || n < 1 || n > e->max_batch || comp < 0 || comp > 1 || form < 0 || form > 1) { nhw_enc_err = "bad argument"; return NHW_E_ARG; }
+	if (!e->timed || n > e->last_n || e->stop_after) {
+		nhw_enc_err = "nhw_stage_chroma_tail: needs a completed whole batch of >= n images and no debug stop";
+		return NHW_E_ARG;
+	}
+	HIPCHK(hipSetDevice(e->device));
+	NhwWs ws = e->ws;
+	ws.n = n; ws.q = e->last_q; ws.dbg = form == 1; ws.split_chroma = e->chroma_fork;
+	hipStream_t s = stream ? (hipStream_t)stream : e->own_stream;
+	HIPCHK(hipStreamWaitEvent(s, e->ev[EV_END], 0));
+	nhw_launch_chroma_tail(ws, comp, form == 0, s);
+	HIPCHK(hipGetLastError());
+	return NHW_OK;
+}
+
 extern "C" int nhw_stage_luma_loop(nhw_enc *e, int n, int form, void *stream)
 {
 	if (!e || n < 1 || n > e->max_batch || form < 0 || form > 7) { nhw_enc_err = "bad argument"; return NHW_E_ARG; }
diff --git a/nhwcodec_amd/csrc/nhw_host.h b/nhwcodec_amd/csrc/nhw_host.h
--- a/nhwcodec_amd/csrc/nhw_host.h
+++ b/nhwcodec_amd/csrc/nhw_host.h
@@ -57,6 +57,7 @@
 enum { PH_L1, PH_L2, PH_L3, PH_L4A, PH_C0, PH_C2, PH_C3, PH_C4, PH_C5, PH_L4B = 10, PH_L4C, PH_L4D, PH_LLC, PH_L4C2 };
 enum { WV_DQ1, WV_DQ0, WV_EMIT, WV_QUANT };
 void nhw_launch_phase(int ph, const NhwWs &ws, int comp, hipStream_t s);
+void nhw_launch_chroma_tail(const NhwWs &ws, int comp, bool once, hipStream_t s);
 void nhw_launch_pack_chroma(const NhwWs &ws, hipStream_t s);
 void nhw_launch_final(const NhwWs &ws, uint8_t *out, uint32_t *sizes, int32_t *status, hipStream_t s, bool chroma_packed = false);
 void nhw_launch_wave(int ph, const NhwWs &ws, hipStream_t s, bool one_walk = false ,
diff --git a/nhwcodec_amd/csrc/nhw_tail.hip b/nhwcodec_amd/csrc/nhw_tail.hip
--- a/nhwcodec_amd/csrc/nhw_tail.hip
+++ b/nhwcodec_amd/csrc/nhw_tail.hip
@@ -81,6 +81,17 @@
 	Ctx c;
 	ctx_load(&c, ws, blockIdx.x);
 	luma_p4a_par(&c, threadIdx.x, dyn_lds);
+}
+
+#ifndef NHW_CTAIL_WAVES
+#define NHW_CTAIL_WAVES 4
+#endif
+__global__ __launch_bounds__(256) __attribute__((amdgpu_waves_per_eu(NHW_CTAIL_WAVES, NHW_CTAIL_WAVES))) void k_chroma_tail(NhwWs ws, int comp)
+{
+	extern __shared__ __attribute__((aligned(16))) int16_t dyn_lds[];
+	Ctx c;
+	ctx_load(&c, ws, blockIdx.x, comp);
+	chroma_tail_once_par(&c, comp, threadIdx.x, dyn_lds);
 }
 
 template <int PH>
@@ -427,7 +438,7 @@
 {
 #define SETATTR(fn) do { const hipError_t e_ = hipFuncSetAttribute(reinterpret_cast<const void *>(&fn), hipFuncAttributeMaxDynamicSharedMemorySize, 100 << 10); \
                          if (e_ != hipSuccess) { *where = "hipFuncSetAttribute(" #fn ", MaxDynamicSharedMemorySize)"; return (int)e_; } } while (0)
-	SETATTR(k_phase<PH_L1>); SETATTR(k_phase<PH_L2>); SETATTR(k_phase<PH_L3>); SETATTR(k_phase<PH_C5>);
+	SETATTR(k_phase<PH_L1>); SETATTR(k_phase<PH_L2>); SETATTR(k_phase<PH_L3>); SETATTR(k_phase<PH_C5>); SETATTR(k_chroma_tail);
 	for (const void *fn : { reinterpret_cast<const void *>(&k_l2_recon<false>), reinterpret_cast<const void *>(&k_l2_recon<true>), reinterpret_cast<const void *>(&k_l2_recon<true, true>) }) {
 		const hipError_t e_ = hipFuncSetAttribute(fn, hipFuncAttributeMaxDynamicSharedMemorySize, (int)(H * (H + 2) * sizeof(int16_t) + 288));
 		if (e_ != hipSuccess) { *where = "hipFuncSetAttribute(k_l2_recon, MaxDynamicSharedMemorySize)"; return (int)e_; }
@@ -450,6 +461,11 @@
 	}
 #undef PHASE
 }
+void nhw_launch_chroma_tail(const NhwWs &ws, int comp, bool once, hipStream_t s)
+{
+	if (once && !ws.dbg) k_chroma_tail<<<ws.n, 256, CT_LDS_BYTES, s>>>(ws, comp);
+	else nhw_launch_phase(PH_C5, ws, comp, s);
+}
 void nhw_launch_pack_chroma(const NhwWs &ws, hipStream_t s)
 {
 	k_pack_chroma<<<ws.n, 256, PK_LDS_BYTES, s>>>(ws);
diff --git a/nhwcodec_amd/csrc/nhw_tail_par.h b/nhwcodec_amd/csrc/nhw_tail_par.h
--- a/nhwcodec_amd/csrc/nhw_tail_par.h
+++ b/nhwcodec_amd/csrc/nhw_tail_par.h
@@ -705,12 +705,89 @@
 
 #define CQROW 264
 #define CQ_LDS_BYTES (4 * 16 * CQROW + 2 * (H + 2))
+DEV void cq_symbols(const int cur[4], int first_next, int lane, int sym[4])
+{
+	if (!__any((unsigned)(cur[0] + 6) > 12u || (unsigned)(cur[1] + 6) > 12u || (unsigned)(cur[2] + 6) > 12u || (unsigned)(cur[3] + 6) > 12u)) {
+		for (int k = 0; k < 4; k++) sym[k] = 128;
+		return;
+	}
+	unsigned P, S, T;
+	BS_PRED(P, cur, 4, (unsigned)(x + 8) < 2u); BS_PRED(S, cur, 4, x > 6 && x <= 127 && (x & 7) >= 6); BS_PRED(T, cur, 4, x == 7);
+	const unsigned inrow = lane == 63 ? 0x7u : 0xFu;
+	const unsigned pc = P & bs_dn(P, lane) & inrow, bc = S & bs_dn(T, lane) & inrow;
+	const unsigned pf = __any(pc != 0) ? bs_from4(alt_runs(bs_ballot4(pc))) : 0u;
+	const unsigned bf = __any(bc != 0) ? bs_from4(alt_runs(bs_ballot4(bc))) : 0u;
+	const unsigned pair = pf | bs_up<4>(pf, lane), raised = bs_up<4>(bf, lane);
+	for (int k = 0; k < 4; k++) {
+		const int x = cur[k], nx = right_of_dpp(cur, k, 4, lane, first_next);
+		int a = (raised >> k) & 1 ? 8 : x;
+		const bool neg = a < 0;
+		int m = neg ? -a : a;
+		const bool keep = (nx < 0 && nx > -8) ? (m & 7) >= 6 : (m & 7) == 7;
+		m = (neg && !keep) ? (m & 504) : m;
+		a = neg ? -m : m;
+		int s = (unsigned)(a + DEADZONE - 1) < (unsigned)(2 * DEADZONE - 1) ? 128 : ((a + 128) & 248);
+		s = (pair >> k) & 1 ? 120 : s;
+		if (__ballot(x > 127 || x < -127)) {
+			if (x == 12400) s = 124; else if (x == 12600) s = 126; else if (x == 12900) s = 122; else if (x == 13000) s = 130;
+			else if (x > 127) s = big_code(x, k_big_pos);
+			else if (x < -127) s = big_code(-x, k_big_neg);
+		}
+		sym[k] = s;
+	}
+}
+DEV void cq_flush(Ctx *c, int comp, uint8_t *park, int rb0, int region, unsigned &vtotal, bool dense, int lane)
+{
+	uint8_t *ubytes = c->ubytes;
+	uint8_t *scan = c->scan + 4 * Q;
+	const int strip = lane >> 1, rb = rb0 + 8 * (lane & 1);
+	uint32_t w[16];
+	for (int j = 0; j < 8; j++) {
+		const uint2 x = *reinterpret_cast<const uint2 *>(park + (8 * (lane & 1) + j) * CQROW + 8 * strip);
+		if ((rb + j) & 1) { w[2 * j] = __builtin_bswap32(x.y); w[2 * j + 1] = __builtin_bswap32(x.x); } else { w[2 * j] = x.x; w[2 * j + 1] = x.y; }
+	}
+	const int pos = strip * (8 * H) + 8 * rb;
+	if (!comp) { for (int j = 0; j < 4; j++) reinterpret_cast<uint4 *>(ubytes + pos)[j] = make_uint4(w[4 * j], w[4 * j + 1], w[4 * j + 2], w[4 * j + 3]); return; }
+	uint32_t o[32];
+	for (int j = 0; j < 4; j++) {
+		const uint4 u4 = reinterpret_cast<const uint4 *>(ubytes + pos)[j];
+		const uint32_t uu[4] = { u4.x, u4.y, u4.z, u4.w };
+		for (int e = 0; e < 4; e++) {
+			const uint32_t u = uu[e], v = w[4 * j + e];
+			o[8 * j + 2 * e] = (u & 0xFF) | ((v & 0xFF) << 8) | ((u & 0xFF00) << 8) | ((v & 0xFF00) << 16);
+			o[8 * j + 2 * e + 1] = ((u >> 16) & 0xFF) | (((v >> 16) & 0xFF) << 8) | ((u >> 24) << 16) | ((v >> 24) << 24);
+		}
+	}
+	if (dense) for (int j = 0; j < 8; j++) reinterpret_cast<uint4 *>(scan + 2 * pos)[j] = make_uint4(o[4 * j], o[4 * j + 1], o[4 * j + 2], o[4 * j + 3]);
+	const int F = rb0 >> 4;
+	const uint64_t M0 = (uint64_t)ne_mask32(o, 0x80808080u) | (uint64_t)ne_mask32(o + 8, 0x80808080u) << 32;
+	const uint64_t M1 = (uint64_t)ne_mask32(o + 16, 0x80808080u) | (uint64_t)ne_mask32(o + 24, 0x80808080u) << 32;
+	*reinterpret_cast<uint4 *>(c->cnzq + (F * 64 + lane) * 2) = make_uint4((uint32_t)M0, (uint32_t)(M0 >> 32), (uint32_t)M1, (uint32_t)(M1 >> 32));
+	const unsigned cnt = (unsigned)(__builtin_popcountll(M0) + __builtin_popcountll(M1));
+	unsigned incl = cnt;
+	for (int o_ = 1; o_ < 64; o_ <<= 1) { const unsigned t_ = (unsigned)__shfl_up((int)incl, o_); if (lane >= o_) incl += t_; }
+	if (lane == 0) { c->cfbase[F] = 32768u * region + vtotal; c->cfbase[16 + region] = vtotal + (unsigned)__builtin_amdgcn_readlane((int)incl, 63); }
+	uint8_t *vp = c->cvals + 32768u * region + vtotal + incl - cnt;
+	vtotal += (unsigned)__builtin_amdgcn_readlane((int)incl, 63);
+	uint32_t *sw = reinterpret_cast<uint32_t *>(park);
+	static_assert(16 * CQROW >= 16 * 64 * 4, "a slice of every lane fits the parked rows");
+#pragma unroll
+	for (int hs = 0; hs < 2; hs++) {
+		__builtin_amdgcn_fence(__ATOMIC_SEQ_CST, "wavefront"); __builtin_amdgcn_wave_barrier();
+#pragma unroll
+		for (int k = 0; k < 16; k++) sw[64 * k + lane] = o[16 * hs + k];
+		__builtin_amdgcn_fence(__ATOMIC_SEQ_CST, "wavefront"); __builtin_amdgcn_wave_barrier();
+		const uint8_t *sb = reinterpret_cast<const uint8_t *>(sw) + 4 * lane;
+		for (uint64_t m = hs ? M1 : M0; m; m &= m - 1) {
+			const int bit = __builtin_ctzll(m);
+			*vp++ = sb[256 * (bit >> 2) + (bit & 3)];
+		}
+	}
+}
 DEV void quantise_chroma_par(Ctx *c, int comp, int tid, int16_t *lds, bool write_plane, bool dense )
 {
 	unsigned vtotal = 0;
 	int16_t *p = c->cproc;
-	uint8_t *ubytes = c->ubytes;
-	uint8_t *scan = c->scan + 4 * Q;
 	const int lane = tid & 63, wv = tid >> 6;
 	uint8_t *park = reinterpret_cast<uint8_t *>(lds) + wv * 16 * CQROW;
 	int16_t *nf = lds + 4 * 16 * CQROW / 2;
@@ -722,79 +799,15 @@
 	for (int i = 0; i < 64; i++) {
 		const int r = r0 + i;
 		if (i + 1 < 64) for (int k = 0; k < 4; k++) nxt[k] = p[(r + 1) * H + lane + 64 * k];
-		const int first_next = nf[r + 1];
-		unsigned P, S, T;
-		BS_PRED(P, cur, 4, (unsigned)(x + 8) < 2u); BS_PRED(S, cur, 4, x > 6 && x <= 127 && (x & 7) >= 6); BS_PRED(T, cur, 4, x == 7);
-		const unsigned inrow = lane == 63 ? 0x7u : 0xFu;
-		const unsigned pc = P & bs_dn(P, lane) & inrow, bc = S & bs_dn(T, lane) & inrow;
-		const unsigned pf = __any(pc != 0) ? bs_from4(alt_runs(bs_ballot4(pc))) : 0u;
-		const unsigned bf = __any(bc != 0) ? bs_from4(alt_runs(bs_ballot4(bc))) : 0u;
-		const unsigned pair = pf | bs_up<4>(pf, lane), raised = bs_up<4>(bf, lane);
+		int sym[4];
+		cq_symbols(cur, nf[r + 1], lane, sym);
 		for (int k = 0; k < 4; k++) {
-			const int x = cur[k], nx = right_of_dpp(cur, k, 4, lane, first_next);
-			int a = (raised >> k) & 1 ? 8 : x;
-			const bool neg = a < 0;
-			int m = neg ? -a : a;
-			const bool keep = (nx < 0 && nx > -8) ? (m & 7) >= 6 : (m & 7) == 7;
-			m = (neg && !keep) ? (m & 504) : m;
-			a = neg ? -m : m;
-			int sym = (unsigned)(a + DEADZONE - 1) < (unsigned)(2 * DEADZONE - 1) ? 128 : ((a + 128) & 248);
-			sym = (pair >> k) & 1 ? 120 : sym;
-			if (__ballot(x > 127 || x < -127)) {
-				if (x == 12400) sym = 124; else if (x == 12600) sym = 126; else if (x == 12900) sym = 122; else if (x == 13000) sym = 130;
-				else if (x > 127) sym = big_code(x, k_big_pos);
-				else if (x < -127) sym = big_code(-x, k_big_neg);
-			}
-			if (write_plane) p[r * H + lane + 64 * k] = (int16_t)sym;
-			park[(i & 15) * CQROW + lane + 64 * k] = (uint8_t)sym;
+			if (write_plane) p[r * H + lane + 64 * k] = (int16_t)sym[k];
+			park[(i & 15) * CQROW + lane + 64 * k] = (uint8_t)sym[k];
 		}
 		if ((i & 15) == 15) {
 			__threadfence_block();
-			const int strip = lane >> 1, rb = r - 15 + 8 * (lane & 1);
-			uint32_t w[16];
-			for (int j = 0; j < 8; j++) {
-				const uint2 x = *reinterpret_cast<const uint2 *>(park + (8 * (lane & 1) + j) * CQROW + 8 * strip);
-				if ((rb + j) & 1) { w[2 * j] = __builtin_bswap32(x.y); w[2 * j + 1] = __builtin_bswap32(x.x); } else { w[2 * j] = x.x; w[2 * j + 1] = x.y; }
-			}
-			const int pos = strip * (8 * H) + 8 * rb;
-			if (!comp) { for (int j = 0; j < 4; j++) reinterpret_cast<uint4 *>(ubytes + pos)[j] = make_uint4(w[4 * j], w[4 * j + 1], w[4 * j + 2], w[4 * j + 3]); }
-			else {
-				uint32_t o[32];
-				for (int j = 0; j < 4; j++) {
-					const uint4 u4 = reinterpret_cast<const uint4 *>(ubytes + pos)[j];
-					const uint32_t uu[4] = { u4.x, u4.y, u4.z, u4.w };
-					for (int e = 0; e < 4; e++) {
-						const uint32_t u = uu[e], v = w[4 * j + e];
-						o[8 * j + 2 * e] = (u & 0xFF) | ((v & 0xFF) << 8) | ((u & 0xFF00) << 8) | ((v & 0xFF00) << 16);
-						o[8 * j + 2 * e + 1] = ((u >> 16) & 0xFF) | (((v >> 16) & 0xFF) << 8) | ((u >> 24) << 16) | ((v >> 24) << 24);
-					}
-				}
-				if (dense) for (int j = 0; j < 8; j++) reinterpret_cast<uint4 *>(scan + 2 * pos)[j] = make_uint4(o[4 * j], o[4 * j + 1], o[4 * j + 2], o[4 * j + 3]);
-				const int F = 4 * wv + (i >> 4);
-				const uint64_t M0 = (uint64_t)ne_mask32(o, 0x80808080u) | (uint64_t)ne_mask32(o + 8, 0x80808080u) << 32;
-				const uint64_t M1 = (uint64_t)ne_mask32(o + 16, 0x80808080u) | (uint64_t)ne_mask32(o + 24, 0x80808080u) << 32;
-				*reinterpret_cast<uint4 *>(c->cnzq + (F * 64 + lane) * 2) = make_uint4((uint32_t)M0, (uint32_t)(M0 >> 32), (uint32_t)M1, (uint32_t)(M1 >> 32));
-				const unsigned cnt = (unsigned)(__builtin_popcountll(M0) + __builtin_popcountll(M1));
-				unsigned incl = cnt;
-				for (int o_ = 1; o_ < 64; o_ <<= 1) { const unsigned t_ = (unsigned)__shfl_up((int)incl, o_); if (lane >= o_) incl += t_; }
-				if (lane == 0) { c->cfbase[F] = 32768u * wv + vtotal; c->cfbase[16 + wv] = vtotal + (unsigned)__builtin_amdgcn_readlane((int)incl, 63); }
-				uint8_t *vp = c->cvals + 32768u * wv + vtotal + incl - cnt;
-				vtotal += (unsigned)__builtin_amdgcn_readlane((int)incl, 63);
-				uint32_t *sw = reinterpret_cast<uint32_t *>(park);
-				static_assert(16 * CQROW >= 16 * 64 * 4, "a slice of every lane fits the parked rows");
-#pragma unroll
-				for (int hs = 0; hs < 2; hs++) {
-					__builtin_amdgcn_fence(__ATOMIC_SEQ_CST, "wavefront"); __builtin_amdgcn_wave_barrier();
-#pragma unroll
-					for (int k = 0; k < 16; k++) sw[64 * k + lane] = o[16 * hs + k];
-					__builtin_amdgcn_fence(__ATOMIC_SEQ_CST, "wavefront"); __builtin_amdgcn_wave_barrier();
-					const uint8_t *sb = reinterpret_cast<const uint8_t *>(sw) + 4 * lane;
-					for (uint64_t m = hs ? M1 : M0; m; m &= m - 1) {
-						const int bit = __builtin_ctzll(m);
-						*vp++ = sb[256 * (bit >> 2) + (bit & 3)];
-					}
-				}
-			}
+			cq_flush(c, comp, park, r - 15, wv, vtotal, dense, lane);
 			__threadfence_block();
 		}
 		for (int k = 0; k < 4; k++) cur[k] = nxt[k];
@@ -2177,22 +2190,62 @@
 		*reinterpret_cast<uint4 *>(jp + e0) = make_uint4(out[0], out[1], out[2], out[3]);
 	}
 }
-DEV void chroma_p5_par(Ctx *c, int comp, int tid, int16_t *lds, int *sh_misc, bool write_plane)
+DEV bool uv_pair_pos(int d, int d1) { return d > 3 && d < 7 && d1 > 2 && d1 < 7; }
+DEV bool uv_pair_neg(int d, int d1) { return d < -3 && d > -7 && d1 < -2 && d1 > -8; }
+DEV bool uv_single(int d, int d1, int res_uv) { return iabs(d) > res_uv && (d > 0 || d != -5 || d1 < 0); }
+DEV int uv_code(bool pair, bool pair_pos, int d) { return pair ? (pair_pos ? 12400 : 12600) : (d > 0 ? 12900 : 13000); }
+DEV int uv_slot(int hl, int lh, int hh) { return iabs(hl) < 8 ? 0 : iabs(lh) < 8 ? 1 : iabs(hh) < 8 ? 2 : -1; }
+struct UvRow { int pl[2], hl[2], lh[2], hh[2], o0[2], o1[2]; };
+DEV bool uv_row_marks(const UvRow &x, int res_uv, int lane, bool want_codes, int code[2])
+{
+	int d[2], d1[2];
+	for (int k = 0; k < 2; k++) d[k] = x.pl[k] - x.o0[k];
+	if (!__any(iabs(d[0]) > 3 || iabs(d[1]) > 3)) { code[0] = code[1] = 0; return false; }
+	const int hl_first = __shfl(x.hl[0], 0);
+	for (int k = 0; k < 2; k++) {
+		int pn = right_of(x.pl, k, 2, 1, lane);
+		if (k == 1 && lane == 63) pn = hl_first;
+		d1[k] = pn - x.o1[k];
+	}
+	uint64_t pp[2], pn_[2], fr[2], sg[2], fhl[2], flh[2], m5[2];
+	for (int k = 0; k < 2; k++) {
+		pp[k] = __ballot(uv_pair_pos(d[k], d1[k]));
+		pn_[k] = __ballot(uv_pair_neg(d[k], d1[k]));
+		fhl[k] = __ballot(iabs(x.hl[k]) < 8); flh[k] = __ballot(iabs(x.lh[k]) < 8);
+		fr[k] = fhl[k] | flh[k] | __ballot(iabs(x.hh[k]) < 8);
+		sg[k] = __ballot(uv_single(d[k], d1[k], res_uv));
+		m5[k] = __ballot(d[k] == -5);
+	}
+	uint64_t f[2] = { (pp[0] | pn_[0]) & fr[0], (pp[1] | pn_[1]) & fr[1] };
+	if ((fhl[0] & 1) && ((f[0] | sg[0]) & 1)) {
+		f[1] &= ~(1ull << 63);
+		if (m5[1] >> 63) sg[1] &= ~(1ull << 63);
+	}
+	const M4 fired = alt_runs(M4{ { f[0], f[1], 0, 0 } });
+	const bool ends_in_pair = (fired.w[1] >> 63) != 0;
+	if (!want_codes) return ends_in_pair;
+	const M4 vis = ~up1(fired);
+	for (int k = 0; k < 2; k++) {
+		const bool pair = (fired.w[k] >> lane) & 1;
+		const bool single = !pair && ((vis.w[k] >> lane) & 1) && ((sg[k] >> lane) & 1);
+		code[k] = pair || single ? uv_code(pair, (pp[k] >> lane) & 1, d[k]) : 0;
+	}
+	return ends_in_pair;
+}
+DEV void chroma_marks_par(Ctx *c, int comp, int tid, int *shift, bool store)
 {
 	int16_t *p = c->cproc, *o = c->cll1;
 	const int q = c->q;
-	PROF_BEGIN();
-	if (q >= 18) {
+	{
 		const int res_uv = q > 17 ? 4 : 5;
 		const int lane = tid & 63, wv = tid >> 6;
-		int *shift = reinterpret_cast<int *>(lds), *haz = shift + H / 2;
+		int *haz = shift + H / 2;
 		bool last_cand = false;
 		if (tid < H / 2) {
 			shift[tid] = 0; haz[tid] = 0;
 			const int at = tid * H + H / 2 - 1, ko = tid * (H / 2) + H / 2 - 1;
 			const int d = p[at] - o[ko], d1 = p[tid * H + H / 2] - o[ko + 1];
-			const bool pair = (d > 3 && d < 7 && d1 > 2 && d1 < 7) || (d < -3 && d > -7 && d1 < -2 && d1 > -8);
-			last_cand = pair && (iabs(p[at + H / 2]) < 8 || iabs(p[at + Q / 2]) < 8 || iabs(p[at + Q / 2 + H / 2]) < 8);
+			last_cand = (uv_pair_pos(d, d1) || uv_pair_neg(d, d1)) && uv_slot(p[at + H / 2], p[at + Q / 2], p[at + Q / 2 + H / 2]) >= 0;
 		}
 		const int first_pass = __syncthreads_or(last_cand) ? 0 : 1;
 		for (int pass = first_pass;; pass++) {
@@ -2205,6 +2258,7 @@
 				BARRIER();
 				mark = !changed;
 			}
+			if (mark && !store) break;
 			int16_t nx[12];
 			auto fetch = [&](int r) {
 				const int sh = shift[r];
@@ -2217,46 +2271,22 @@
 			};
 			fetch(wv);
 			for (int r = wv; r < H / 2; r += 4) {
-				int pl[2], hl[2], lh[2], hh[2], d[2], d1[2];
+				UvRow x;
 #pragma unroll
 				for (int k = 0; k < 2; k++) {
-					pl[k] = nx[6 * k]; hl[k] = nx[6 * k + 1]; lh[k] = nx[6 * k + 2]; hh[k] = nx[6 * k + 3];
-					d[k] = pl[k] - nx[6 * k + 4];
-					d1[k] = nx[6 * k + 5];
+					x.pl[k] = nx[6 * k]; x.hl[k] = nx[6 * k + 1]; x.lh[k] = nx[6 * k + 2]; x.hh[k] = nx[6 * k + 3];
+					x.o0[k] = nx[6 * k + 4]; x.o1[k] = nx[6 * k + 5];
 				}
 				if (r + 4 < H / 2) fetch(r + 4);
-				const int hl_first = __shfl(hl[0], 0);
+				int code[2];
+				const bool ends_in_pair = uv_row_marks(x, res_uv, lane, mark, code);
+				if (!mark) { if (lane == 0) haz[r] = (int)ends_in_pair; continue; }
 				for (int k = 0; k < 2; k++) {
-					int pn = right_of(pl, k, 2, 1, lane);
-					if (k == 1 && lane == 63) pn = hl_first;
-					d1[k] = pn - d1[k];
-				}
-				uint64_t pp[2], pn_[2], fr[2], sg[2], fhl[2], flh[2], m5[2];
-				for (int k = 0; k < 2; k++) {
-					pp[k] = __ballot(d[k] > 3 && d[k] < 7 && d1[k] > 2 && d1[k] < 7);
-					pn_[k] = __ballot(d[k] < -3 && d[k] > -7 && d1[k] < -2 && d1[k] > -8);
-					fhl[k] = __ballot(iabs(hl[k]) < 8); flh[k] = __ballot(iabs(lh[k]) < 8);
-					fr[k] = fhl[k] | flh[k] | __ballot(iabs(hh[k]) < 8);
-					sg[k] = __ballot(iabs(d[k]) > res_uv && (d[k] > 0 || d[k] != -5 || d1[k] < 0));
-					m5[k] = __ballot(d[k] == -5);
-				}
-				uint64_t f[2] = { (pp[0] | pn_[0]) & fr[0], (pp[1] | pn_[1]) & fr[1] };
-				if ((fhl[0] & 1) && ((f[0] | sg[0]) & 1)) {
-					f[1] &= ~(1ull << 63);
-					if (m5[1] >> 63) sg[1] &= ~(1ull << 63);
-				}
-				const M4 fired = alt_runs(M4{ { f[0], f[1], 0, 0 } });
-				if (!mark) { if (lane == 0) haz[r] = (int)(fired.w[1] >> 63); continue; }
-				const M4 vis = ~up1(fired);
-				for (int k = 0; k < 2; k++) {
-					const bool pair = (fired.w[k] >> lane) & 1;
-					const bool single = !pair && ((vis.w[k] >> lane) & 1) && ((sg[k] >> lane) & 1);
-					if (!pair && !single) continue;
-					const int16_t code = pair ? (((pp[k] >> lane) & 1) ? 12400 : 12600) : (d[k] > 0 ? 12900 : 13000);
-					const int at = r * H + lane + 64 * k;
-					if (iabs(hl[k]) < 8) p[at + H / 2] = code;
-					else if (iabs(lh[k]) < 8) p[at + Q / 2] = code;
-					else if (iabs(hh[k]) < 8) p[at + Q / 2 + H / 2] = code;
+					if (!code[k]) continue;
+					const int at = r * H + lane + 64 * k, slot = uv_slot(x.hl[k], x.lh[k], x.hh[k]);
+					if (slot == 0) p[at + H / 2] = (int16_t)code[k];
+					else if (slot == 1) p[at + Q / 2] = (int16_t)code[k];
+					else if (slot == 2) p[at + Q / 2 + H / 2] = (int16_t)code[k];
 				}
 			}
 			BARRIER();
@@ -2264,9 +2294,11 @@
 		}
 		if (tid == 0) { int ev = 0; for (int r = 0; r < H / 2; r++) ev += haz[r]; c->m->pad = comp ? c->m->pad + (ev << 8) : ev; }
 	}
-	BARRIER();
-	if (!tid) PROF(c, 27);
-	copy_block_par(c->cl2save, H / 2, p, H, H / 2, H / 2, tid);
+}
+DEV void chroma_ll2_emit_par(Ctx *c, int comp, int tid, int16_t *lds, int16_t *clear_plane )
+{
+	const int q = c->q;
+	PROF_BEGIN();
 	for (int idx = tid; idx < (H / 4) * (H / 4); idx += NT) lds[idx] = c->cl2save[(idx >> 6) * (H / 2) + (idx & 63)];
 	BARRIER();
 	if (q <= 11 && tid < 64) {
@@ -2318,7 +2350,7 @@
 		BARRIER();
 		if (tid == 0) { c->exw[e0] = 0; c->exw[e0 + 1] = 0; c->m->exw_len = e0 + 2 + 3 * (int)total; }
 	}
-	for (int idx = tid; idx < (H / 4) * (H / 4); idx += NT) p[(idx >> 6) * H + (idx & 63)] = 0;
+	if (clear_plane) for (int idx = tid; idx < (H / 4) * (H / 4); idx += NT) clear_plane[(idx >> 6) * H + (idx & 63)] = 0;
 	BARRIER();
 	{
 		uint8_t *dst = comp ? c->res_v64 : c->res_u64;
@@ -2330,8 +2362,97 @@
 		}
 	}
 	if (!tid) PROF(c, 21);
+}
+DEV void chroma_p5_par(Ctx *c, int comp, int tid, int16_t *lds, int *sh_misc, bool write_plane)
+{
+	PROF_BEGIN();
+	if (c->q >= 18) chroma_marks_par(c, comp, tid, reinterpret_cast<int *>(lds), true);
+	BARRIER();
+	if (!tid) PROF(c, 27);
+	copy_block_par(c->cl2save, H / 2, c->cproc, H, H / 2, H / 2, tid);
+	chroma_ll2_emit_par(c, comp, tid, lds, c->cproc);
 	BARRIER();
 	quantise_chroma_par(c, comp, tid, lds, write_plane, write_plane);
+	if (!tid) PROF(c, 22);
+}
+
+#define CT_PARKS (2 * 4 * 16 * CQROW)
+#define CT_LDS_BYTES (CT_PARKS + 2 * (H + 4) + 2 * (H / 2) * 4)
+DEV void chroma_tail_once_par(Ctx *c, int comp, int tid, int16_t *lds)
+{
+	const int16_t *p = c->cproc, *o = c->cll1, *l2 = c->cl2save;
+	const int q = c->q, lane = tid & 63, wv = tid >> 6;
+	const bool marks = q >= 18;
+	const int res_uv = q > 17 ? 4 : 5;
+	int16_t *nf = lds + CT_PARKS / 2;
+	int *shift = reinterpret_cast<int *>(nf + H + 4);
+	static_assert(CT_PARKS % 4 == 0 && CT_PARKS >= (H / 4) * (H / 4) * 2 + 4096, "tables behind the emission's LDS");
+	PROF_BEGIN();
+	if (marks) chroma_marks_par(c, comp, tid, shift, false);
+	BARRIER();
+	if (tid < H / 2) {
+		if (tid) nf[tid] = tid < H / 4 ? (int16_t)0 : l2[tid * (H / 2)];
+		const int R = tid, at = R * H;
+		int lh = p[at + Q / 2];
+		if (marks) {
+			const int ko = R * (H / 2) + shift[R];
+			const int d = p[at] - o[ko], d1 = p[at + 1] - o[ko + 1], hl = p[at + H / 2], hh = p[at + Q / 2 + H / 2];
+			const bool pair_pos = uv_pair_pos(d, d1), pair = (pair_pos || uv_pair_neg(d, d1)) && uv_slot(hl, lh, hh) >= 0;
+			if ((pair || uv_single(d, d1, res_uv)) && uv_slot(hl, lh, hh) == 1) lh = uv_code(pair, pair_pos, d);
+		}
+		nf[H / 2 + R] = (int16_t)lh;
+	}
+	if (tid == NT - 1) nf[H] = p[Q];
+	if (!tid) PROF(c, 27);
+	chroma_ll2_emit_par(c, comp, tid, lds, nullptr);
+	BARRIER();
+	uint8_t *park_t = reinterpret_cast<uint8_t *>(lds) + wv * 2 * 16 * CQROW, *park_b = park_t + 16 * CQROW;
+	unsigned vtotal = 0;
+	const int R0 = (H / 8) * wv;
+	int16_t nx[14] = { 0, 0, 0, 0, 0, 0, 0, 0, 0, 0, 0, 0, 0, 0 };
+	auto fetch = [&](int R) {
+		const int sh = marks ? shift[R] : 0;
+#pragma unroll
+		for (int k = 0; k < 2; k++) {
+			const int at = R * H + lane + 64 * k, ko = R * (H / 2) + sh + lane + 64 * k;
+			nx[7 * k + 1] = p[at + H / 2]; nx[7 * k + 2] = p[at + Q / 2]; nx[7 * k + 3] = p[at + Q / 2 + H / 2];
+			if (marks) { nx[7 * k] = p[at]; nx[7 * k + 4] = o[ko]; nx[7 * k + 5] = o[ko + 1]; }
+			nx[7 * k + 6] = l2[R * (H / 2) + lane + 64 * k];
+		}
+	};
+	fetch(R0);
+	for (int i = 0; i < H / 8; i++) {
+		const int R = R0 + i;
+		UvRow x;
+		int ll[2];
+#pragma unroll
+		for (int k = 0; k < 2; k++) {
+			x.pl[k] = nx[7 * k]; x.hl[k] = nx[7 * k + 1]; x.lh[k] = nx[7 * k + 2]; x.hh[k] = nx[7 * k + 3];
+			x.o0[k] = nx[7 * k + 4]; x.o1[k] = nx[7 * k + 5]; ll[k] = nx[7 * k + 6];
+		}
+		if (i + 1 < H / 8) fetch(R + 1);
+		if (marks) {
+			int code[2];
+			uv_row_marks(x, res_uv, lane, true, code);
+#pragma unroll
+			for (int k = 0; k < 2; k++) {
+				const int slot = code[k] ? uv_slot(x.hl[k], x.lh[k], x.hh[k]) : -1;
+				x.hl[k] = slot == 0 ? code[k] : x.hl[k]; x.lh[k] = slot == 1 ? code[k] : x.lh[k]; x.hh[k] = slot == 2 ? code[k] : x.hh[k];
+			}
+		}
+		const int top[4] = { R < H / 4 ? 0 : ll[0], ll[1], x.hl[0], x.hl[1] }, bot[4] = { x.lh[0], x.lh[1], x.hh[0], x.hh[1] };
+		int sym[4];
+		cq_symbols(top, nf[R + 1], lane, sym);
+		for (int k = 0; k < 4; k++) park_t[(i & 15) * CQROW + lane + 64 * k] = (uint8_t)sym[k];
+		cq_symbols(bot, nf[H / 2 + R + 1], lane, sym);
+		for (int k = 0; k < 4; k++) park_b[(i & 15) * CQROW + lane + 64 * k] = (uint8_t)sym[k];
+		if ((i & 15) == 15) {
+			__threadfence_block();
+			cq_flush(c, comp, park_t, R - 15, wv, vtotal, false, lane);
+			cq_flush(c, comp, park_b, H / 2 + R - 15, wv, vtotal, false, lane);
+			__threadfence_block();
+		}
+	}
 	if (!tid) PROF(c, 22);
 }
 
diff --git a/profiles/make_design_table.py b/profiles/make_design_table.py
--- a/profiles/make_design_table.py
+++ b/profiles/make_design_table.py
@@ -1,7 +1,7 @@
 import json, os, re, sys
 ROOT = os.path.dirname(os.path.dirname(os.path.abspath(__file__)))
-STATS = os.path.join(ROOT, "profiles", "l2_dead_stores_kernel_stats_1stream_after.txt")
-PMC = os.path.join(ROOT, "profiles", "l2_dead_stores_pmc_after.json")
+STATS = os.path.join(ROOT, "profiles", "chroma_tail_kernel_stats_1stream_after.txt")
+PMC = os.path.join(ROOT, "profiles", "chroma_tail_pmc_after.json")
 BATCHES = 7.0
 PH = ["L1", "L2", "L3", "L4A", "C0", "C2", "C3", "C4", "C5", "FINAL", "L4B", "L4C", "L4D", "LLC", "L4C2"]
 WV = ["DQ1", "DQ0", "EMIT", "QUANT"]
@@ -22,6 +22,7 @@
     "C0": "chroma: copy", "C2": "chroma: dequantiser simulation 1", "C3": "chroma: tags", "C4": "chroma: dequantiser simulation 2",
     "C5": "chroma: marks (running-index fixed point), LL2 emission, quantiser (wavefront per row); V leaves the merged chroma stream as a list", "LLC": "Z1 chroma LL2 coder", "FINAL": "Z2 packetiser + container",
     "k_l4a": "Y19-Y23 of q >= 17: Y21 small runs (wavefront per row, rows in which nothing fires skipped), Y22 + Y23 as ONE column sweep on registers and class tables (eight workgroups a CU)",
+    "k_chroma_tail": "chroma tail of a batch: the rows' shifts (running-index fixed point), LL2 emission, then ONE walk: a wavefront reads each plane row once, marks it in registers and quantises it (rows without a candidate and all-quiet rows skipped); cproc is not written; V leaves the merged chroma stream as a list",
     "k_y31": "Y31 rewrites on the symbol LIST (non-zero map + values), 512 threads an image; leaves map and offsets in stream order",
     "k_final": "Z2 packetiser (the luma part from its symbol list, both books) + container; a kernel of its own at six wavefronts a SIMD",
     "k_pack_chroma": "Z2's chroma part: words and ranked book entries from the chroma symbol list (on the chroma stream in the forked order)",
```
